# k-sheridan/mantis

Measured on AMD Instinct MI355X. Metric: poses/sec + p50 per-frame latency, 1280x720 4-cam batch, higher is better.
Workload: dtype f64; 1 GPU; config3: 4-cam 1280x720 rig, shared map, full mantis3 path per camera + joint rig Gauss-Newton; cams_per_rig=4, contexts_per_gpu=6, landmarks=720, parallelism=rig-data-parallel x1

## Files before the change

### mantis_amd/csrc/api.hip

```cpp
#include <hip/hip_runtime.h>
#ifndef MK_FC_THREADS
#define MK_FC_THREADS 256
#endif

#include <algorithm>
#include <atomic>
#include <cfloat>
#include <chrono>
#include <cmath>
#include <cstdio>
#include <cstdlib>
#include <cstring>
#include <mutex>
#include <sstream>
#include <string>
#include <thread>
#include <vector>

#include <rccl/rccl.h>

#include "kernels.hip"

using namespace mk;

namespace {

struct ZigTables {
  uint32_t kn[128];
  float wn[128], fn[128];
  ZigTables() {
    const double m1 = 2147483648.0;
    double dn = 3.442619855899, tn = dn, vn = 9.91256303526217e-3;
    double q = vn / std::exp(-.5 * dn * dn);
    kn[0] = (uint32_t)((dn / q) * m1);
    kn[1] = 0;
    wn[0] = (float)(q / m1);
    wn[127] = (float)(dn / m1);
    fn[0] = 1.f;
    fn[127] = (float)std::exp(-.5 * dn * dn);
    for (int i = 126; i >= 1; i--) {
      dn = std::sqrt(-2. * std::log(vn / dn + std::exp(-.5 * dn * dn)));
      kn[i + 1] = (uint32_t)((dn / tn) * m1);
      tn = dn;
      fn[i] = (float)std::exp(-.5 * dn * dn);
      wn[i] = (float)(dn / m1);
    }
  }
};
const ZigTables& zig() {
  static ZigTables t;
  return t;
}
inline uint64_t rng_step(uint64_t x) { return (uint64_t)(uint32_t)x * 4164903690ULL + (x >> 32); }
inline float rng_gauss(uint64_t& state) {
  const ZigTables& T = zig();
  const float r = 3.442620f;
  const float rng_flt = 2.3283064365386962890625e-10f;
  uint64_t temp = state;
  float x, y;
  for (;;) {
    int hz = (int)(uint32_t)temp;
    temp = rng_step(temp);
    int iz = hz & 127;
    x = hz * T.wn[iz];
    if ((unsigned)std::abs(hz) < T.kn[iz]) break;
    if (iz == 0) {
      do {
        x = (unsigned)temp * rng_flt;
        temp = rng_step(temp);
        y = (unsigned)temp * rng_flt;
        temp = rng_step(temp);
        x = (float)(-std::log(x + FLT_MIN) * 0.2904764);
        y = (float)-std::log(y + FLT_MIN);
      } while (y + y < x * x);
      x = hz > 0 ? r + x : -r - x;
      break;
    }
    y = (unsigned)temp * rng_flt;
    temp = rng_step(temp);
    if (T.fn[iz] + y * (T.fn[iz - 1] - T.fn[iz]) < std::exp(-.5 * x * x)) break;
  }
  state = temp;
  return x;
}

#define HIP_OK(expr)                                                              \
  do {                                                                            \
    hipError_t e_ = (expr);                                                       \
    if (e_ != hipSuccess) {                                                       \
      c->err = std::string(#expr) + ": " + hipGetErrorString(e_);                 \
      return MANTIS_ERR_DEVICE;                                                   \
    }                                                                             \
  } while (0)

struct Ctx {
  mantis_config cfg{};
  hipStream_t s = nullptr;
  hipStream_t s_copy = nullptr;
  hipEvent_t ev_gauss = nullptr;
  hipEvent_t ev_wait = nullptr;
  int spin_frames = 16;
  std::string err;
  uint64_t rng_state = 1;
  double* d_lm = nullptr;
  int nw = 0, nr = 0, ng = 0;
  int F = 0, Wmax = 0, Hmax = 0;
  int n_cu = 256;
  bool trace_lds_ok = false;
  size_t trace_lds_max = 0;
  int trace_lds_frames = 0;
  int fc_small_frames = 0;
  size_t plane = 0;
  int pool_cap = 0;
  uint16_t* d_lroot = nullptr;
  size_t lstride = 0;
  size_t fstride = 0;
  uint8_t *d_bgr = nullptr, *d_strong = nullptr, *d_edge = nullptr,
          *d_det = nullptr, *d_mask = nullptr;
  int32_t* d_lab = nullptr;
  uint32_t *d_eb = nullptr, *d_b1 = nullptr, *d_b2 = nullptr;
  uint32_t* d_mbits = nullptr;
  size_t bstride = 0;
  int morph_bh = 48;
  int morph_walk = 1 << 20;
  bool runs_done = false;
  int morph_walk_small = 48;
  size_t pf_mask_lds = 0;
  int hyst_epoch = 3;
  bool hyst_rec = true;
  size_t hyst_rec_lds = 0;
  bool pf_split = true;
  uint32_t* d_dbits = nullptr;
  uint32_t* d_tbits = nullptr;
  size_t tstride = 0;
  int32_t* d_rowb = nullptr;
  size_t rstride = 0;
  size_t dstride = 0;
  FrameDesc* d_frames = nullptr;
  Border* d_borders = nullptr;
  int32_t *d_bcount = nullptr, *d_boff = nullptr, *d_pool = nullptr, *d_scratch = nullptr;
  QuadRec* d_quads = nullptr;
  RppOut* d_rpp = nullptr;
  RppItem* d_items = nullptr;
  rpp::Refine* d_refine = nullptr;
  int32_t *d_jobs0 = nullptr, *d_jobs1 = nullptr;
  RppQueue* d_rq = nullptr;
  int rpp_blocks = 0;
  double* d_opool[2] = {nullptr, nullptr};
  int32_t* d_ojob[2] = {nullptr, nullptr};
  int32_t* d_octl = nullptr;
  int32_t op_cap = 0;
  int op_rounds = 6, op_spill = 32;
  int op_lanes_small = 64, op_rounds_small = 6;
  int seg_m = 64;
  int canny_strip = 2;
  int canny_small = 0;
#ifndef MK_SHIFT_SPLIT
#define MK_SHIFT_SPLIT 0
#endif
  bool shift_split = MK_SHIFT_SPLIT;
#ifndef MK_GN_FUSED_ALL
#define MK_GN_FUSED_ALL 1
#endif
  bool gn_fused_all = MK_GN_FUSED_ALL;
  bool pf_shifts = true;
  int pf_init = 1;
  bool canny_cat = true;
  bool counted = false;
  bool vec_ok = false;
  double *d_dense_c2w = nullptr, *d_dense_err = nullptr, *d_pairs = nullptr;
  int32_t* d_dense_np = nullptr;
  size_t dense_cap = 0;
  void* d_dense_jobs = nullptr;
  size_t dense_pairs_cap = 0;
  size_t dense_jobs_cap = 0;
  GnCam* d_gncam = nullptr;
  RigGnIO* d_rigio = nullptr;
  double* d_gnobs = nullptr;
  double* d_gnacc = nullptr;
  int gn_rigs = 0, gn_cpr = 0;
  int gn_last_rigs = 0, gn_last_local = 0;
  HypRec *d_gen = nullptr, *d_hyps = nullptr;
  FrameState* d_st = nullptr;
  ScoreState* d_sst = nullptr;
  FrameDebug* d_dbg = nullptr;
  mantis_cam_result* d_res = nullptr;
  float* d_gauss = nullptr;
  int32_t* d_gtotal = nullptr;
  float* h_gauss = nullptr;
  uint64_t* h_states = nullptr;
  mantis_cam_result* h_res = nullptr;
  FrameState* h_st = nullptr;
  int32_t* h_gtotal = nullptr;
  FrameDesc* h_frames = nullptr;
  bool prof = false;
  std::vector<std::string> ev_names;
  std::vector<hipEvent_t> ev;
  std::vector<float> last_ms;
  std::vector<std::string> last_names;
  std::vector<void*> user_allocs;
  void* comm = nullptr;
  int nranks = 1, rank = 0;
  double* d_gn28 = nullptr;
  int32_t *d_sh_gidx = nullptr, *d_sh_pf = nullptr, *d_sh_flags = nullptr;
  int32_t* h_sh_flags = nullptr;
  size_t sh_cap = 0;
  uint8_t *d_sh_rec = nullptr, *h_sh_rec = nullptr;
  size_t sh_rec_bytes = 0;
  int gauss_cap = 0;
  RigWJob* d_rwjobs = nullptr;
  double* d_rwout = nullptr;
  size_t rw_cap = 0;
  int rw_rigs = 0, rw_C = 0;
  std::vector<double> rw_weights, rw_c2w, rw_sums;
  std::vector<int32_t> rw_chosen;
  bool has_prior = false;
  double prior_Twb[16];
  double* d_markov = nullptr;
  MarkovOp* d_mops = nullptr;
  int markov_n = 0;
  int32_t* d_agree = nullptr;
  bool agreed_fail = false;
  struct CallGraph {
    int n = 0, W = 0, H = 0, live = 0, nw = 0, nr = 0, ng = 0;
    bool vec = false;
    const void* lm = nullptr;
    const void* gauss = nullptr;
    hipGraphExec_t pre = nullptr, post = nullptr;
  };
  std::vector<CallGraph> graphs;
  bool use_graphs = false;
  bool screen_off = false;
  std::vector<std::pair<Cam, ScreenCam>> scam_cache;
  struct Track {
    void* d_in = nullptr;
    void* h_in = nullptr;
    size_t in_cap = 0;
    void* d_state = nullptr;
    void* d_res = nullptr;
    void* h_res = nullptr;
    int rig_cap = 0;
    void *d_Twb = nullptr, *d_c2w = nullptr, *d_pf = nullptr;
    long long* d_sums = nullptr;
    int32_t* d_cnt = nullptr;
    size_t pose_cap = 0, task_cap = 0;
    int rigs = 0, C = 0, P = 0, I = 0, record = 0;
  } trk;
  struct Mcl {
    bool live = false;
    mantis_mcl_params p{};
    int N = 0, cap = 0, cur = 0;
    void* d_T[2] = {nullptr, nullptr};
    double *d_L = nullptr, *d_Lprev = nullptr;
    unsigned long long *d_q = nullptr, *d_cum = nullptr;
    int32_t* d_anc = nullptr;
    void *d_in = nullptr, *h_in = nullptr;
    void *d_c2w = nullptr, *d_pf = nullptr;
    long long* d_sums = nullptr;
    int32_t* d_cnt = nullptr;
    void *d_res = nullptr, *h_res = nullptr;
    bool has_record = false;
    int rec_C = 0, rec_pred = 0;
    void *d_modes = nullptr, *h_modes = nullptr;
    bool has_modes = false;
    struct mantis_mcl_modes modes;
    double modes_g = 0;
    mantis_mcl_color_params color{};
    long long* d_csums = nullptr;
    int32_t* d_ccnt = nullptr;
    double *d_Ec = nullptr, *d_charge = nullptr;
    int color_cap = 0;
    int rec_color = 0, rec_color_min = 0;
  } mcl;
};

mantis_status agree(Ctx* c, mantis_status local, int32_t count = -1) {
  c->agreed_fail = false;
  if (!c->comm || !c->d_agree) return local;
  int32_t v[3] = {local != MANTIS_OK ? 1 : 0, count, -count};
  if (hipMemcpyAsync(c->d_agree, v, sizeof(v), hipMemcpyHostToDevice, c->s) != hipSuccess ||
      ncclAllReduce(c->d_agree, c->d_agree, 3, ncclInt32, ncclMax, (ncclComm_t)c->comm, c->s) != ncclSuccess ||
      hipMemcpyAsync(v, c->d_agree, sizeof(v), hipMemcpyDeviceToHost, c->s) != hipSuccess ||
      hipStreamSynchronize(c->s) != hipSuccess) {
    c->err = "agreement all-reduce failed";
    return MANTIS_ERR_COMM;
  }
  const bool mismatch = v[1] != -v[2];
  c->agreed_fail = v[0] != 0 || mismatch;
  if (local != MANTIS_OK) return local;
  if (v[0]) {
    c->err = "another rank of the communicator failed before this exchange (see its mantis_last_error)";
    return MANTIS_ERR_COMM;
  }
  if (mismatch) {
    c->err = "ranks passed different frame counts to a batched exchange (every rank must pass the same n_frames)";
    return MANTIS_ERR_ARG;
  }
  return MANTIS_OK;
}

inline Landmarks lmk_of(const Ctx* c) {
  return Landmarks{c->d_lm, c->nw, c->nr, c->ng, c->d_lm ? (const float4*)(c->d_lm + kLmfOffset) : nullptr};
}

void mark(Ctx* c, const char* name) {
  if (!c->prof) return;
  if (c->ev.size() <= c->ev_names.size()) {
    hipEvent_t e;
    (void)hipEventCreate(&e);
    c->ev.push_back(e);
  }
  (void)hipEventRecord(c->ev[c->ev_names.size()], c->s);
  c->ev_names.push_back(name);
}

struct Ctx;
hipError_t wait_stream(Ctx* c, int frames);

inline void bind_device(const Ctx* c) {
  int d = -1;
  if (hipGetDevice(&d) != hipSuccess || d != c->cfg.device) (void)hipSetDevice(c->cfg.device);
}

inline size_t morph_lds(int W, int bh) { return (size_t)3 * (bh + 2 * MB_HALO) * ((W + 31) / 32) * sizeof(uint32_t); }

inline int blocks_for(size_t n, int per = 256, int cap = 4096) {
  size_t b = (n + per - 1) / per;
  return (int)std::min<size_t>(std::max<size_t>(b, 1), (size_t)cap);
}

Cam cam_from(const mantis_image& im) {
  Cam m;
  m.fx = (double)(float)im.K[0];
  m.fy = (double)(float)im.K[4];
  m.cx = (double)(float)im.K[2];
  m.cy = (double)(float)im.K[5];
  for (int k = 0; k < 4; k++) m.k[k] = im.D[k];
  return m;
}

ScreenCam screen_cam_cached(Ctx* c, const Cam& cm) {
  for (const auto& e : c->scam_cache)
    if (std::memcmp(&e.first, &cm, sizeof(Cam)) == 0) return e.second;
  ScreenCam sc = screen_cam_from(cm);
  if (c->screen_off) sc.sens = INFINITY;
  if (c->scam_cache.size() >= 64) c->scam_cache.erase(c->scam_cache.begin());
  c->scam_cache.emplace_back(cm, sc);
  return sc;
}

template <class T>
mantis_status dalloc(Ctx* c, T** p, size_t count);

mantis_status stage_frames(Ctx* c, const mantis_image* cams, int n, int& W, int& H) {
  if (n <= 0 || n > c->F) { c->err = "frame count exceeds max_cams"; return MANTIS_ERR_ARG; }
  W = cams[0].width;
  H = cams[0].height;
  if (W <= 2 || H <= 2 || W > c->Wmax || H > c->Hmax) { c->err = "image size outside [3, max]"; return MANTIS_ERR_ARG; }
  const size_t fb = (size_t)W * H * 3;
  for (int i = 0; i < n; i++) {
    const mantis_image& im = cams[i];
    if (im.width != W || im.height != H) { c->err = "all cameras of a batch must share one size"; return MANTIS_ERR_ARG; }
    if (!im.bgr || im.step_bytes < 3 * W) { c->err = "bgr8 image with step >= 3*width required"; return MANTIS_ERR_ARG; }
    FrameDesc& fd = c->h_frames[i];
    fd.w = W;
    fd.h = H;
    fd.cam = cam_from(im);
    fd.scam = screen_cam_cached(c, fd.cam);
    if (im.mem_kind == 1 && im.step_bytes == 3 * W) {
      fd.bgr = im.bgr;
    } else {
      if (!c->d_bgr) {
        if (dalloc(c, &c->d_bgr, (size_t)c->F * c->Wmax * c->Hmax * 3) != MANTIS_OK) {
          c->d_bgr = nullptr;
          c->err = "hipMalloc of the frame staging buffer failed";
          return MANTIS_ERR_OOM;
        }
      }
      uint8_t* dst = c->d_bgr + (size_t)i * fb;
      HIP_OK(hipMemcpy2DAsync(dst, 3 * W, im.bgr, im.step_bytes, 3 * W, H,
                              im.mem_kind == 1 ? hipMemcpyDeviceToDevice : hipMemcpyHostToDevice, c->s));
      fd.bgr = dst;
    }
  }
  c->vec_ok = (W % 4) == 0;
  for (int i = 0; i < n; i++) c->vec_ok = c->vec_ok && ((uintptr_t)c->h_frames[i].bgr & 3) == 0;
// ... 198 lines not shown
  k_rpp_s1b<<<(unsigned)std::min<size_t>((expected_items + 63) / 64, (size_t)c->n_cu * MK_S1B_WPC), 64, 0, c->s>>>(
      items, jobs0, jobs1, q, pr);
  mark(c, "rpp_2nd");
  run_objpose_rounds<1>(c, blocks_for(expected_items * 2), items, rf, jobs1, q, st, 0, lanes, rounds);
  mark(c, "rpp_cand");
  k_rpp_merge<<<(unsigned)((ni + 255) / 256), 256, 0, c->s>>>(items, ni, rf, out, quads,
                                                               quads ? c->cfg.quad_gn_iterations : 0);
  mark(c, "rpp_merge");
}

mantis_status run_pose(Ctx* c, int n) {
  HIP_OK(hipMemsetAsync(c->d_rq, 0, sizeof(RppQueue), c->s));
  dim3 gr((kMaxQuads * 2 + 255) / 256, n);
  k_rpp_prep<<<gr, 256, 0, c->s>>>(c->d_quads, c->d_st, c->d_items, c->d_jobs0, c->d_rq, c->cfg.grid_spacing / 2);
  const size_t ni = (size_t)n * kMaxQuads * 2;
  mark(c, "rpp_prep");
  launch_rpp_queues(c, c->d_items, c->d_refine, c->d_jobs0, c->d_jobs1, c->d_rq, c->d_rpp, c->d_st, ni, (size_t)n * 160,
                    c->d_quads, true, n <= c->fc_small_frames);
  k_frame_hyps<<<n, 256, 0, c->s>>>(c->d_rpp, c->d_st, c->d_gen, c->d_hyps, c->d_dbg, 0.5, 0.2);
  mark(c, "hyps_cluster");
  HIP_OK(hipGetLastError());
  return MANTIS_OK;
}

struct Shard {
  int n_global;
  int slots;
  const int32_t* gidx;
};

mantis_status gauss_offsets(Ctx* c, int n, const Shard* sh) {
  const int per = c->cfg.particles * c->cfg.iterations * 6;
  if (!sh) {
    k_gauss_offsets<<<1, kGaussOffThreads, 0, c->s>>>(c->d_st, n, per, c->d_gtotal);
    HIP_OK(hipGetLastError());
    return MANTIS_OK;
  }
  HIP_OK(hipMemcpyAsync(c->d_sh_gidx, sh->gidx, sizeof(int32_t) * n, hipMemcpyHostToDevice, c->s));
  int32_t* send = c->d_sh_pf;
  int32_t* recv = c->d_sh_pf + 2 * (size_t)sh->slots;
  k_shard_pf_pack<<<(sh->slots + 255) / 256, 256, 0, c->s>>>(c->d_st, c->d_sh_gidx, n, sh->slots, send);
  ncclResult_t r = ncclAllGather(send, recv, 2 * (size_t)sh->slots, ncclInt32, (ncclComm_t)c->comm, c->s);
  if (r != ncclSuccess) { c->err = std::string("ncclAllGather (PF flags): ") + ncclGetErrorString(r); return MANTIS_ERR_COMM; }
  k_gauss_offsets_global<<<1, 1024, 0, c->s>>>(recv, sh->slots * c->nranks, c->d_sh_flags, sh->n_global, c->d_st,
                                               c->d_sh_gidx, n, per, c->d_gtotal);
  mark(c, "pf_exchange");
  HIP_OK(hipGetLastError());
  return MANTIS_OK;
}

void gen_gauss(Ctx* c, int n) {
  const int per = c->cfg.particles * c->cfg.iterations * 6;
  uint64_t s = c->rng_state;
  c->h_states[0] = s;
  for (int f = 0; f < n; f++) {
    float* g = c->h_gauss + (size_t)f * per;
    for (int k = 0; k < per; k++) g[k] = rng_gauss(s);
    c->h_states[f + 1] = s;
  }
}

mantis_status run_score(Ctx* c, int n, int n_gauss, bool copy_gauss = true) {
  const int per = c->cfg.particles * c->cfg.iterations * 6;
  if (copy_gauss) {
    HIP_OK(hipMemcpyAsync(c->d_gauss, c->h_gauss, sizeof(float) * per * n_gauss, hipMemcpyHostToDevice, c->s_copy));
    HIP_OK(hipEventRecord(c->ev_gauss, c->s_copy));
    HIP_OK(hipStreamWaitEvent(c->s, c->ev_gauss, 0));
  }
  mark(c, "gauss_h2d");
  Landmarks L = lmk_of(c);
  const bool split = c->pf_split && n <= c->fc_small_frames && c->cfg.particles <= kPfMaxParticles &&
                     c->cfg.iterations > 0;
  const bool pf_shifts = !split && c->pf_shifts;
  const int pf_init = split ? 0 : c->pf_init;
  if (!pf_init) {
    k_score_init<kScoreInit><<<n, kScoreInit, 0, c->s>>>(c->d_frames, c->d_mbits, c->bstride, L, c->d_st, c->d_hyps,
                                                        c->d_res, c->d_dbg, c->d_sst);
    mark(c, "score_pf_yaw/k_score_init");
  }
  const size_t ml = c->pf_mask_lds;
  constexpr int ppb = std::max(1, kPfThreads / 64 / kPfSplit);
  if (split) {
    const int nblk = (c->cfg.particles + ppb - 1) / ppb;
    for (int it = 0; it < c->cfg.iterations; it++)
      k_score_pf_part<kPfThreads, kPfSplit><<<dim3(nblk, n), kPfThreads, 0, c->s>>>(
          c->d_frames, c->d_mbits, c->bstride, L, c->d_st, c->d_gauss, c->d_res, c->d_dbg, c->d_sst, c->cfg.particles,
          c->cfg.iterations, it, ppb, nblk);
  } else if (ml)
    k_score_pf<kPfThreads, kPfSplit, true><<<n, kPfThreads, ml, c->s>>>(
        c->d_frames, c->d_mbits, c->bstride, L, c->d_st, c->d_gauss, c->d_res, c->d_dbg, c->d_sst, c->cfg.particles,
        c->cfg.iterations, pf_shifts ? 1 : 0, c->cfg.grid_spacing, 9, pf_init, c->d_hyps,
        (unsigned char*)c->d_gen);
  else
    k_score_pf<kPfThreads, kPfSplit, false><<<n, kPfThreads, 0, c->s>>>(
        c->d_frames, c->d_mbits, c->bstride, L, c->d_st, c->d_gauss, c->d_res, c->d_dbg, c->d_sst, c->cfg.particles,
        c->cfg.iterations, pf_shifts ? 1 : 0, c->cfg.grid_spacing, 9, pf_init, c->d_hyps,
        (unsigned char*)c->d_gen);
  mark(c, "score_pf_yaw/k_score_pf");
  const bool shifts_apart = !pf_shifts && (split || c->shift_split);
  if (shifts_apart) {
    constexpr int spb = kScoreTail / 128;
    k_score_shift_part<kScoreTail><<<dim3((81 + spb - 1) / spb, n), kScoreTail, 0, c->s>>>(
        c->d_frames, c->d_mbits, c->bstride, L, c->d_st, c->d_sst, c->cfg.grid_spacing, 9, spb);
    mark(c, "score_pf_yaw/k_score_shift_part");
  }
  k_score_final<kScoreTail><<<n, kScoreTail, 0, c->s>>>(c->d_frames, c->d_mbits, c->bstride, L, c->d_st, c->d_res, c->d_dbg,
                                               c->d_sst, c->cfg.grid_spacing, 9, shifts_apart || pf_shifts);
  mark(c, "score_pf_yaw/k_score_final");
  HIP_OK(hipGetLastError());
  return MANTIS_OK;
}

void finish_profile(Ctx* c, bool append = false) {
  if (!c->prof || c->ev_names.empty()) return;
  (void)hipEventSynchronize(c->ev[c->ev_names.size() - 1]);
  if (!append) {
    c->last_names.clear();
    c->last_ms.clear();
  }
  for (size_t i = 1; i < c->ev_names.size(); i++) {
    float ms = 0;
    (void)hipEventElapsedTime(&ms, c->ev[i - 1], c->ev[i]);
    c->last_names.push_back(c->ev_names[i]);
    c->last_ms.push_back(ms);
  }
  c->ev_names.clear();
}

hipError_t wait_stream(Ctx* c, int frames) {
  if (frames <= c->spin_frames || !c->ev_wait) return hipStreamSynchronize(c->s);
  hipError_t e = hipEventRecord(c->ev_wait, c->s);
  if (e != hipSuccess) return e;
  return hipEventSynchronize(c->ev_wait);
}

using mk::shard::fuse_rig;
using mk::shard::mat4_inv_rigid;
using mk::shard::mat4_mul;
using mk::shard::quat_to_mat4;

template <class T>
mantis_status dalloc(Ctx* c, T** p, size_t count);
template <class T>
mantis_status halloc(Ctx* c, T** p, size_t count);

mantis_status ensure_gauss(Ctx* c, int n) {
  if (n <= c->gauss_cap) return MANTIS_OK;
  const int per = c->cfg.particles * c->cfg.iterations * 6;
  HIP_OK(hipStreamSynchronize(c->s));
  (void)hipFree(c->d_gauss);
  (void)hipHostFree(c->h_gauss);
  (void)hipHostFree(c->h_states);
  c->d_gauss = nullptr;
  c->h_gauss = nullptr;
  c->h_states = nullptr;
  c->gauss_cap = 0;
  if (dalloc(c, &c->d_gauss, (size_t)n * per) || halloc(c, &c->h_gauss, (size_t)n * per) ||
      halloc(c, &c->h_states, (size_t)n + 1))
    return MANTIS_ERR_OOM;
  c->gauss_cap = n;
  return MANTIS_OK;
}

template <class F>
mantis_status capture_graph(Ctx* c, hipGraphExec_t* out, F&& body) {
  HIP_OK(hipStreamBeginCapture(c->s, hipStreamCaptureModeThreadLocal));
  const mantis_status st = body();
  hipGraph_t gr = nullptr;
  const hipError_t e = hipStreamEndCapture(c->s, &gr);
  if (st != MANTIS_OK || e != hipSuccess) {
    if (gr) (void)hipGraphDestroy(gr);
    if (st != MANTIS_OK) return st;
    c->err = std::string("hipStreamEndCapture: ") + hipGetErrorString(e);
    return MANTIS_ERR_DEVICE;
  }
  const hipError_t ei = hipGraphInstantiate(out, gr, nullptr, nullptr, 0);
  (void)hipGraphDestroy(gr);
  if (ei != hipSuccess) {
    *out = nullptr;
    c->err = std::string("hipGraphInstantiate: ") + hipGetErrorString(ei);
    return MANTIS_ERR_DEVICE;
  }
  return MANTIS_OK;
}

Ctx::CallGraph* call_graph(Ctx* c, int n, int W, int H, const Shard* sh) {
  if (!c->use_graphs || sh || c->prof || n > c->fc_small_frames) return nullptr;
  const size_t hr_lds = (size_t)((H + HR_ROWS - 1) / HR_ROWS) * HR_ROWS * bits::words(W) * sizeof(uint32_t);
  if (!(c->hyst_rec && bits::words(W) <= 63 && H <= HR_ROWS * HR_MAXW && hr_lds <= c->hyst_rec_lds)) return nullptr;
  const int live = std::max(1, g_live_ctx[c->cfg.device & 63].load());
  for (auto& g : c->graphs)
    if (g.n == n && g.W == W && g.H == H && g.vec == c->vec_ok && g.live == live && g.lm == c->d_lm &&
        g.nw == c->nw && g.nr == c->nr && g.ng == c->ng && g.gauss == c->d_gauss)
      return &g;
  if (c->graphs.size() >= 8) {
    if (c->graphs.front().pre) (void)hipGraphExecDestroy(c->graphs.front().pre);
    if (c->graphs.front().post) (void)hipGraphExecDestroy(c->graphs.front().post);
    c->graphs.erase(c->graphs.begin());
  }
  Ctx::CallGraph g;
  g.n = n; g.W = W; g.H = H; g.vec = c->vec_ok; g.live = live;
  g.lm = c->d_lm; g.nw = c->nw; g.nr = c->nr; g.ng = c->ng; g.gauss = c->d_gauss;
  c->graphs.push_back(g);
  return &c->graphs.back();
}

mantis_status process_frames(Ctx* c, const mantis_image* cams, int n, const Shard* sh = nullptr) {
  if (!c->d_lm) { c->err = "map not set (mantis_set_map)"; return MANTIS_ERR_STATE; }
  if (n <= 0 || n > c->F) { c->err = "frame count exceeds max_cams"; return MANTIS_ERR_ARG; }
  const int ng = sh ? sh->n_global : n;
  if ((int64_t)c->cfg.particles * c->cfg.iterations * 6 * ng > INT32_MAX) {
    c->err = "particles x iterations x 6 x frames (all rig cameras when sharded) exceeds 2^31 gaussians per call";
    return MANTIS_ERR_ARG;
  }
  if (mantis_status e = ensure_gauss(c, ng)) return e;
  struct Joiner {
    std::thread t;
    ~Joiner() { if (t.joinable()) t.join(); }
  } gauss;
  gauss.t = std::thread([c, ng] { gen_gauss(c, ng); });
  int W, H;
  mantis_status st = stage_frames(c, cams, n, W, H);
  const auto results_d2h = [&]() -> mantis_status {
    HIP_OK(hipMemcpyAsync(c->h_res, c->d_res, sizeof(mantis_cam_result) * n, hipMemcpyDeviceToHost, c->s));
    HIP_OK(hipMemcpyAsync(c->h_st, c->d_st, sizeof(FrameState) * n, hipMemcpyDeviceToHost, c->s));
    HIP_OK(hipMemcpyAsync(c->h_gtotal, c->d_gtotal, sizeof(int32_t), hipMemcpyDeviceToHost, c->s));
    return MANTIS_OK;
  };
  Ctx::CallGraph* g = st == MANTIS_OK ? call_graph(c, n, W, H, sh) : nullptr;
  if (g) {
    if (!g->pre)
      st = capture_graph(c, &g->pre, [&]() -> mantis_status {
        mantis_status s2 = run_image_stages(c, n, W, H);
        if (s2 == MANTIS_OK) s2 = run_contours(c, n, W, H);
        if (s2 == MANTIS_OK) s2 = run_pose(c, n);
        if (s2 == MANTIS_OK) s2 = gauss_offsets(c, n, nullptr);
        return s2;
      });
    if (st != MANTIS_OK) return st;
    HIP_OK(hipGraphLaunch(g->pre, c->s));
    gauss.t.join();
    const int per = c->cfg.particles * c->cfg.iterations * 6;
    HIP_OK(hipMemcpyAsync(c->d_gauss, c->h_gauss, sizeof(float) * per * ng, hipMemcpyHostToDevice, c->s));
    if (!g->post)
      st = capture_graph(c, &g->post, [&]() -> mantis_status {
        mantis_status s2 = run_score(c, n, ng, false);
        if (s2 == MANTIS_OK) s2 = results_d2h();
        return s2;
      });
    if (st != MANTIS_OK) return st;
    HIP_OK(hipGraphLaunch(g->post, c->s));
  } else {
    if (st == MANTIS_OK) st = run_image_stages(c, n, W, H);
    if (st == MANTIS_OK) st = run_contours(c, n, W, H);
    if (st == MANTIS_OK) st = run_pose(c, n);
    if (sh) st = agree(c, st);
    if (st != MANTIS_OK) return st;
    if ((st = gauss_offsets(c, n, sh)) != MANTIS_OK) return st;
    gauss.t.join();
    if ((st = run_score(c, n, ng)) != MANTIS_OK) return st;
    if ((st = results_d2h()) != MANTIS_OK) return st;
  }
  if (sh) HIP_OK(hipMemcpyAsync(c->h_sh_flags, c->d_sh_flags, sizeof(int32_t) * ng, hipMemcpyDeviceToHost, c->s));
  HIP_OK(wait_stream(c, n));
  finish_profile(c);
  const int per = c->cfg.particles * c->cfg.iterations * 6;
  int used = 0;
  if (sh)
    for (int f = 0; f < ng; f++) used += c->h_sh_flags[f] ? 1 : 0;
  for (int f = 0; f < n; f++) {
    if (!sh && c->h_st[f].reaches_pf) used++;
    if (c->h_st[f].overflow) {
      std::ostringstream os;
      os << "frame " << f << ": workspace capacity exceeded (flags " << c->h_st[f].overflow << ", borders "
         << c->h_st[f].n_borders << ", points " << c->h_st[f].n_points << ", raw quads " << c->h_st[f].n_raw_quads
         << ")";
      c->err = os.str();
      c->h_res[f].status = MANTIS_ERR_CAPACITY;
    }
  }
  if (const char* fs = getenv("MANTIS_FRAME_STATS")) {
    if (FILE* fp = fopen(fs, "a")) {
      for (int f = 0; f < n; f++)
        fprintf(fp, "%d %d %d %d %d %d %d\n", c->h_st[f].n_runs, c->h_st[f].n_borders, c->h_st[f].n_points,
                c->h_st[f].trace_steps_max, c->h_st[f].trace_steps_sum, c->h_st[f].n_chunks, c->h_st[f].trace_ticks);
// ... 84 lines not shown
      g_create_err = "mantis_config.struct_size mismatch";
      return MANTIS_ERR_ARG;
    }
    cfg = *cfg_in;
  }
  if (cfg.max_quads == 0) cfg.max_quads = kMaxQuads;
  if ((int64_t)cfg.particles * cfg.iterations * 6 * (cfg.max_cams > 0 ? cfg.max_cams : 1) > INT32_MAX) {
    g_create_err = "particles x iterations x 6 x max_cams exceeds 2^31 gaussians per batch";
    return MANTIS_ERR_ARG;
  }
  if (cfg.particles < 1 || cfg.particles > 96 || cfg.iterations < 0 || cfg.iterations > 1000 || cfg.max_cams < 1 ||
      cfg.max_width < 3 || cfg.max_height < 3 || cfg.gn_iterations < 0 || cfg.gn_iterations > 10 ||
      cfg.quad_gn_iterations < 0 || cfg.quad_gn_iterations > 20 || cfg.rig_weighting < 0 || cfg.rig_weighting > 1) {
    g_create_err = "invalid config (particles 1..96, iterations 0..1000, gn_iterations 0..10, "
                   "quad_gn_iterations 0..20, max_cams >= 1, image >= 3x3)";
    return MANTIS_ERR_ARG;
  }
  if (cfg.max_width > 8190) {
    g_create_err = "max_width: at most 8190 (the hysteresis bands hold a row's worst-case runs in LDS)";
    return MANTIS_ERR_ARG;
  }
  if (cfg.max_height > 65533) {
    g_create_err = "max_height: at most 65533 (border walks and contour points pack y + 1 in 16 bits)";
    return MANTIS_ERR_ARG;
  }
  if ((int64_t)((cfg.max_height + HB_ROWS - 1) / HB_ROWS) * HB_ROWS * ((cfg.max_width + 1) / 2) >= (1 << 24)) {
    g_create_err = "max_width x max_height: at most 2^25 pixels (hysteresis run ids and their band row share a word)";
    return MANTIS_ERR_ARG;
  }
  if (cfg.max_quads != kMaxQuads) {
    g_create_err = "max_quads: the per-frame quad capacity is fixed at 256 in this build";
    return MANTIS_ERR_ARG;
  }
  int ndev = 0;
  if (hipGetDeviceCount(&ndev) != hipSuccess || ndev <= cfg.device) {
    g_create_err = "no HIP device available (libmantis_amd requires an MI355X / gfx950 GPU)";
    return MANTIS_ERR_DEVICE;
  }
  Ctx* c = new Ctx();
  c->cfg = cfg;
  c->rng_state = cfg.rng_seed ? cfg.rng_seed : 0xffffffffULL;
  if (hipSetDevice(cfg.device) != hipSuccess || hipStreamCreateWithFlags(&c->s, hipStreamNonBlocking) != hipSuccess ||
      hipStreamCreateWithFlags(&c->s_copy, hipStreamNonBlocking) != hipSuccess ||
      hipEventCreateWithFlags(&c->ev_gauss, hipEventDisableTiming) != hipSuccess ||
      hipEventCreateWithFlags(&c->ev_wait, hipEventDisableTiming | hipEventBlockingSync) != hipSuccess) {
    g_create_err = "hipSetDevice/hipStreamCreate failed";
    if (c->s) (void)hipStreamDestroy(c->s);
    if (c->s_copy) (void)hipStreamDestroy(c->s_copy);
    delete c;
    return MANTIS_ERR_DEVICE;
  }
  if (hipDeviceGetAttribute(&c->n_cu, hipDeviceAttributeMultiprocessorCount, cfg.device) != hipSuccess || c->n_cu < 1)
    c->n_cu = 256;
  if (const char* e = std::getenv("MANTIS_RPP_BLOCKS")) c->rpp_blocks = std::atoi(e);
  if (const char* e = std::getenv("MANTIS_OP_ROUNDS")) c->op_rounds = std::max(1, std::min(kOpMaxRounds, std::atoi(e)));
  if (const char* e = std::getenv("MANTIS_OP_SPILL")) c->op_spill = std::max(0, std::min(64, std::atoi(e)));
  if (const char* e = std::getenv("MANTIS_OP_LANES_SMALL")) c->op_lanes_small = std::max(1, std::min(64, std::atoi(e)));
  if (const char* e = std::getenv("MANTIS_OP_ROUNDS_SMALL")) c->op_rounds_small = std::max(1, std::min(kOpMaxRounds, std::atoi(e)));
  if (const char* e = std::getenv("MANTIS_SEG_M")) c->seg_m = std::max(0, std::min(4096, std::atoi(e)));
  if (const char* e = std::getenv("MANTIS_CANNY_STRIP")) c->canny_strip = c->canny_small = std::atoi(e);
  if (const char* e = std::getenv("MANTIS_CANNY_CAT")) c->canny_cat = e[0] != '0';
  if (const char* e = std::getenv("MANTIS_SHIFT_SPLIT")) c->shift_split = e[0] != '0';
  if (const char* e = std::getenv("MANTIS_PF_SHIFTS")) c->pf_shifts = e[0] != '0';
  if (const char* e = std::getenv("MANTIS_GN_FUSED")) c->gn_fused_all = e[0] != '0';
  if (const char* e = std::getenv("MANTIS_PF_INIT")) c->pf_init = std::max(0, std::min(2, std::atoi(e)));
  if (const char* e = std::getenv("MANTIS_HYST_REC")) c->hyst_rec = e[0] != '0';
  {
    const char* pc = std::getenv("DEBUG_CLR_GRAPH_PACKET_CAPTURE");
    c->use_graphs = pc && pc[0] == '0';
    if (const char* e = std::getenv("MANTIS_GRAPHS")) c->use_graphs = c->use_graphs && e[0] != '0';
  }
  if (const char* e = std::getenv("MANTIS_HYST_EPOCH0")) c->hyst_epoch = std::max(3, std::min(255, std::atoi(e)));
  c->F = cfg.max_cams;
  c->Wmax = cfg.max_width;
  c->Hmax = cfg.max_height;
  c->plane = (size_t)(c->Wmax + 2) * (c->Hmax + 2);
  c->bstride = bits::tiled_words(c->Wmax, c->Hmax);
  c->dstride = (size_t)dbits_wpw(c->Wmax + 2) * (c->Hmax + 2);
  c->pool_cap = cfg.max_contour_points;
  {
    c->trace_lds_max = 160 * 1024 - 512 * 8 - 64;
    c->trace_lds_ok = hipFuncSetAttribute((const void*)k_trace_borders_lds, hipFuncAttributeMaxDynamicSharedMemorySize,
                                          (int)c->trace_lds_max) == hipSuccess;
    const char* so = getenv("MANTIS_SCREEN");
    c->screen_off = so && so[0] == '0';
    const char* e = getenv("MANTIS_TRACE_LDS_FRAMES");
    c->trace_lds_frames = e ? atoi(e) : c->n_cu / 4;
    const char* e2 = getenv("MANTIS_FC_SMALL_FRAMES");
    c->fc_small_frames = e2 ? atoi(e2) : c->n_cu / 4;
    const char* e3 = getenv("MANTIS_PF_SPLIT");
    c->pf_split = !(e3 && e3[0] == '0');
  }
  {
    const size_t ml = bits::tiled_words(c->Wmax, c->Hmax) * 4;
    hipFuncAttributes a1;
    c->pf_mask_lds = 0;
    if (!getenv("MANTIS_PF_MASK_GLOBAL") &&
        hipFuncGetAttributes(&a1, (const void*)k_score_pf<kPfThreads, kPfSplit, true>) == hipSuccess &&
        a1.sharedSizeBytes + ml <= 160 * 1024 &&
        hipFuncSetAttribute((const void*)k_score_pf<kPfThreads, kPfSplit, true>,
                            hipFuncAttributeMaxDynamicSharedMemorySize, (int)ml) == hipSuccess)
      c->pf_mask_lds = ml;
  }
  {
    hipFuncAttributes a;
    if (hipFuncGetAttributes(&a, (const void*)k_hyst_rec) == hipSuccess) {
      const size_t budget = 160 * 1024 - a.sharedSizeBytes;
      if (hipFuncSetAttribute((const void*)k_hyst_rec, hipFuncAttributeMaxDynamicSharedMemorySize, (int)budget) ==
          hipSuccess)
        c->hyst_rec_lds = budget;
    }
  }
  if (hipFuncSetAttribute((const void*)k_hyst_band, hipFuncAttributeMaxDynamicSharedMemorySize,
                          (int)(3 * sizeof(uint32_t) * HB_ROWS * bits::words(c->Wmax))) != hipSuccess) {
    g_create_err = "max_width too large for the hysteresis band kernel";
    (void)hipStreamDestroy(c->s);
    delete c;
    return MANTIS_ERR_ARG;
  }
  c->morph_bh = morph_lds(c->Wmax, MB_BH) <= 160 * 1024 ? MB_BH : MB_BH_NARROW;
  if (const char* e = getenv("MANTIS_MORPH_WALK")) {
    c->morph_walk = std::max(0, atoi(e));
    c->morph_walk_small = std::max(1, c->morph_walk);
  }
  if (const char* e = getenv("MANTIS_MORPH_WALK_SMALL")) c->morph_walk_small = std::max(1, atoi(e));
  if (morph_lds(c->Wmax, c->morph_bh) > 160 * 1024 ||
      hipFuncSetAttribute((const void*)k_morph, hipFuncAttributeMaxDynamicSharedMemorySize,
                          (int)morph_lds(c->Wmax, c->morph_bh)) !=
          hipSuccess) {
    g_create_err = "max_width too large for the morphology band kernel";
    (void)hipStreamDestroy(c->s);
    delete c;
    return MANTIS_ERR_ARG;
  }
  const int F = c->F;
  const int per = cfg.particles * cfg.iterations * 6;
  mantis_status st = MANTIS_OK;
  auto chk = [&](mantis_status s) { if (st == MANTIS_OK) st = s; };
  c->fstride = (c->plane + 3) & ~(size_t)3;
  chk(dalloc(c, &c->d_strong, (size_t)F * c->fstride));
  c->lstride = (c->plane + 1) & ~(size_t)1;
  chk(dalloc(c, &c->d_lroot, (size_t)F * c->lstride));
  chk(dalloc(c, &c->d_edge, c->plane));
  chk(dalloc(c, &c->d_det, c->plane));
  chk(dalloc(c, &c->d_eb, (size_t)F * c->bstride));
  chk(dalloc(c, &c->d_b1, (size_t)F * c->bstride));
  chk(dalloc(c, &c->d_b2, (size_t)F * c->bstride));
  chk(dalloc(c, &c->d_dbits, (size_t)F * c->dstride));
  c->tstride = tbits_words(c->Wmax + 2, c->Hmax + 2);
  chk(dalloc(c, &c->d_tbits, (size_t)F * c->tstride));
  c->rstride = (size_t)c->Hmax + 3 + (c->Hmax + HB_ROWS - 1) / HB_ROWS;
  chk(dalloc(c, &c->d_rowb, (size_t)F * c->rstride));
  chk(dalloc(c, &c->d_mask, c->plane));
  chk(dalloc(c, &c->d_mbits, (size_t)F * c->bstride));
  chk(dalloc(c, &c->d_lab, (size_t)F * c->plane));
  chk(dalloc(c, &c->d_frames, (size_t)F));
  chk(dalloc(c, &c->d_borders, (size_t)F * kMaxBorders));
  chk(dalloc(c, &c->d_bcount, (size_t)F * kMaxBorders));
  chk(dalloc(c, &c->d_boff, (size_t)F * kMaxBorders));
  chk(dalloc(c, &c->d_pool, (size_t)F * 2 * c->pool_cap));
  chk(dalloc(c, &c->d_scratch, (size_t)F * 4 * c->pool_cap));
  chk(dalloc(c, &c->d_quads, (size_t)F * kMaxQuads));
  chk(dalloc(c, &c->d_rpp, (size_t)F * kMaxQuads * 2));
  chk(dalloc(c, &c->d_items, (size_t)F * kMaxQuads * 2));
  chk(dalloc(c, &c->d_refine, (size_t)F * kMaxQuads * 2 * rpp::kCand));
  chk(dalloc(c, &c->d_jobs0, (size_t)F * kMaxQuads * 2));
  chk(dalloc(c, &c->d_jobs1, (size_t)F * kMaxQuads * 2 * rpp::kCand));
  chk(dalloc(c, &c->d_rq, 1));
  {
    const size_t blocks = c->rpp_blocks > 0 ? (size_t)c->rpp_blocks : (size_t)std::max(64, 3 * c->n_cu / 2);
    c->op_cap = (int32_t)(blocks * 256);
    for (int k = 0; k < 2; k++) {
      chk(dalloc(c, &c->d_opool[k], (size_t)kOpFields * c->op_cap));
      chk(dalloc(c, &c->d_ojob[k], (size_t)c->op_cap));
    }
    chk(dalloc(c, &c->d_octl, 2 * 2 * kOpMaxRounds));
  }
  chk(dalloc(c, &c->d_gen, (size_t)F * kMaxHyps));
  chk(dalloc(c, &c->d_hyps, (size_t)F * kMaxHyps));
  chk(dalloc(c, &c->d_st, (size_t)F));
  chk(dalloc(c, &c->d_sst, (size_t)F));
  chk(dalloc(c, &c->d_dbg, (size_t)F));
  chk(dalloc(c, &c->d_res, (size_t)F));
  chk(dalloc(c, &c->d_gauss, (size_t)F * per));
// ... 4 lines not shown
  chk(halloc(c, &c->h_res, (size_t)F));
  chk(halloc(c, &c->h_st, (size_t)F));
  chk(halloc(c, &c->h_gtotal, 1));
  chk(halloc(c, &c->h_frames, (size_t)F));
  if (st != MANTIS_OK) {
    g_create_err = c->err;
    mantis_destroy(c);
    return st;
  }
  (void)hipGetLastError();
  if (hipMemset(c->d_dbg, 0, sizeof(FrameDebug) * F) != hipSuccess ||
      hipMemset(c->d_strong, 0, c->fstride * (size_t)F) != hipSuccess) {
    g_create_err = "hipMemset failed";
    mantis_destroy(c);
    return MANTIS_ERR_DEVICE;
  }
  g_live_ctx[cfg.device & 63].fetch_add(1);
  c->counted = true;
  *out_ctx = c;
  return MANTIS_OK;
}

mantis_status mantis_destroy(void* ctx) {
  Ctx* c = (Ctx*)ctx;
  if (c) bind_device(c);
  if (!c) return MANTIS_ERR_ARG;
  if (c->counted) g_live_ctx[c->cfg.device & 63].fetch_sub(1);
  if (c->s) (void)hipStreamSynchronize(c->s);
  if (c->comm) (void)ncclCommDestroy((ncclComm_t)c->comm);
  for (auto& g : c->graphs) {
    if (g.pre) (void)hipGraphExecDestroy(g.pre);
    if (g.post) (void)hipGraphExecDestroy(g.post);
  }
  if (c->d_rwjobs) (void)hipFree(c->d_rwjobs);
  if (c->d_markov) (void)hipFree(c->d_markov);
  if (c->d_mops) (void)hipFree(c->d_mops);
  if (c->d_rwout) (void)hipFree(c->d_rwout);
  void* dptrs[] = {c->d_opool[0], c->d_opool[1], c->d_ojob[0], c->d_ojob[1], c->d_octl, c->d_dense_jobs, c->d_agree, c->d_gn28, c->d_bgr, c->d_lroot, c->d_strong, c->d_edge, c->d_det, c->d_mask, c->d_lab, c->d_eb, c->d_b1, c->d_b2, c->d_mbits, c->d_dbits, c->d_tbits, c->d_rowb,
                   c->d_frames, c->d_borders, c->d_bcount, c->d_boff, c->d_pool, c->d_scratch, c->d_quads, c->d_rpp, c->d_items, c->d_refine, c->d_jobs0, c->d_jobs1, c->d_rq,
                   c->d_dense_c2w, c->d_dense_err, c->d_dense_np, c->d_pairs, c->d_gncam, c->d_rigio, c->d_gnobs, c->d_gnacc, c->d_sh_gidx, c->d_sh_pf, c->d_sh_flags, c->d_sh_rec, c->d_gen, c->d_hyps, c->d_st, c->d_sst, c->d_dbg, c->d_res, c->d_gauss, c->d_gtotal, c->d_lm};
  for (void* p : dptrs)
    if (p) (void)hipFree(p);
  void* tptrs[] = {c->trk.d_in, c->trk.d_state, c->trk.d_res, c->trk.d_Twb, c->trk.d_c2w, c->trk.d_pf, c->trk.d_sums, c->trk.d_cnt};
  for (void* p : tptrs)
    if (p) (void)hipFree(p);
  void* mptrs[] = {c->mcl.d_T[0], c->mcl.d_T[1], c->mcl.d_L, c->mcl.d_Lprev, c->mcl.d_q, c->mcl.d_cum, c->mcl.d_anc,
                   c->mcl.d_in, c->mcl.d_c2w, c->mcl.d_pf, c->mcl.d_sums, c->mcl.d_cnt, c->mcl.d_res, c->mcl.d_modes,
                   c->mcl.d_csums, c->mcl.d_ccnt, c->mcl.d_Ec, c->mcl.d_charge};
  for (void* p : mptrs)
    if (p) (void)hipFree(p);
  for (void* p : c->user_allocs) (void)hipFree(p);
  void* hptrs[] = {c->h_gauss, c->h_states, c->h_res, c->h_st, c->h_gtotal, c->h_frames, c->h_sh_flags, c->h_sh_rec,
                   c->trk.h_in, c->trk.h_res, c->mcl.h_in, c->mcl.h_res, c->mcl.h_modes};
  for (void* p : hptrs)
    if (p) (void)hipHostFree(p);
  for (hipEvent_t e : c->ev) (void)hipEventDestroy(e);
  if (c->ev_gauss) (void)hipEventDestroy(c->ev_gauss);
  if (c->ev_wait) (void)hipEventDestroy(c->ev_wait);
  if (c->s_copy) (void)hipStreamDestroy(c->s_copy);
  if (c->s) (void)hipStreamDestroy(c->s);
  delete c;
  return MANTIS_OK;
}

const char* mantis_last_error(void* ctx) {
  if (!ctx) return g_create_err.c_str();
  return ((Ctx*)ctx)->err.c_str();
}

mantis_status mantis_set_map(void* ctx, const double* white, int32_t nw, const double* red, int32_t nr,
                             const double* green, int32_t ng) {
  Ctx* c = (Ctx*)ctx;
  if (c) bind_device(c);
  if (!c || nw < 0 || nr < 0 || ng < 0 || nw + nr + ng > 768 || ng > 64 || (nw && !white) || (nr && !red) ||
      (ng && !green)) {
    if (c) c->err = "map: need nw+nr+ng <= 768 and ng <= 64";
    return MANTIS_ERR_ARG;
  }
  std::vector<double> all;
  all.insert(all.end(), white, white + 3 * nw);
  all.insert(all.end(), red, red + 3 * nr);
  all.insert(all.end(), green, green + 3 * ng);
  const size_t nl = (size_t)nw + nr + ng;
  std::vector<double> buf(kLmfOffset + 2 * 768, 0.0);
  std::copy(all.begin(), all.end(), buf.begin());
  float* lf = (float*)(buf.data() + kLmfOffset);
  for (size_t i = 0; i < nl; i++) screen_landmark(all.data() + 3 * i, lf + 4 * i);
  if (c->d_lm) (void)hipFree(c->d_lm);
  c->d_lm = nullptr;
  if (dalloc(c, &c->d_lm, buf.size()) != MANTIS_OK) return MANTIS_ERR_OOM;
  HIP_OK(hipMemcpy(c->d_lm, buf.data(), sizeof(double) * buf.size(), hipMemcpyHostToDevice));
  c->nw = nw;
  c->nr = nr;
  c->ng = ng;
  return MANTIS_OK;
}

int32_t mantis_parse_coordinates(const char* s, double* xyz, int32_t max_pts) {
  if (!s) return 0;
  std::vector<std::string> rows;
  std::stringstream ts(s);
  std::string tmp;
  while (std::getline(ts, tmp, ';')) {
    tmp.erase(std::remove(tmp.begin(), tmp.end(), '\n'), tmp.end());
    tmp.erase(std::remove(tmp.begin(), tmp.end(), ' '), tmp.end());
    rows.push_back(tmp);
  }
  int n = 0;
  for (auto& e : rows) {
    std::stringstream rs(e);
    std::string rt;
    double v[3] = {0, 0, 0};
    for (int k = 0; k < 3; k++) {
      std::getline(rs, rt, ',');
      v[k] = std::atof(rt.data());
    }
    if (xyz && n < max_pts) { xyz[3 * n] = v[0]; xyz[3 * n + 1] = v[1]; xyz[3 * n + 2] = v[2]; }
    n++;
  }
  return n;
}

mantis_status mantis_rng_get(void* ctx, uint64_t* state) {
  if (!ctx || !state) return MANTIS_ERR_ARG;
  *state = ((Ctx*)ctx)->rng_state;
  return MANTIS_OK;
}
mantis_status mantis_rng_set(void* ctx, uint64_t state) {
  if (!ctx) return MANTIS_ERR_ARG;
  ((Ctx*)ctx)->rng_state = state ? state : 0xffffffffULL;
  return MANTIS_OK;
}

namespace {
mantis_status run_rig_gn(Ctx* c, const double* Tbc, int n_rigs, int cams_local, mantis_result* out,
                         bool use_comm);
}

namespace {
mantis_status weight_rigs(Ctx* c, int n_rigs, int C, const mantis_cam_result* all, const double* Tall,
                          const int32_t* gidx, int n_local, bool use_comm, mantis_result* out,
                          const double* pred_Twb = nullptr) {
  const int K = C + 1;
  const size_t nslot = (size_t)n_rigs * K * C;
  std::vector<double> Twb((size_t)n_rigs * K * 16);
  std::vector<char> cand((size_t)n_rigs * K, 0);
  for (int r = 0; r < n_rigs; r++) {
    for (int k = 0; k < C; k++) {
      const mantis_cam_result& cr = all[(size_t)r * C + k];
      if (!cr.publish) continue;
      double Twc[16], Tinv[16];
      quat_to_mat4(cr.orientation_xyzw, cr.position, Twc);
      mat4_inv_rigid(Tall + 16 * ((size_t)r * C + k), Tinv);
      mat4_mul(Twc, Tinv, &Twb[16 * ((size_t)r * K + k)]);
      cand[(size_t)r * K + k] = 1;
    }
    if (pred_Twb) {
      std::memcpy(&Twb[16 * ((size_t)r * K + C)], pred_Twb + 16 * (size_t)r, sizeof(double) * 16);
      cand[(size_t)r * K + C] = 1;
    }
  }
  c->rw_c2w.assign(nslot * 12, 0.0);
  std::vector<RigWJob> jobs;
  std::vector<size_t> slot_of;
  for (int i = 0; i < n_local; i++) {
    const int g = gidx ? gidx[i] : i;
    const int r = g / C, cam = g % C;
    for (int k = 0; k < K; k++) {
      if (!cand[(size_t)r * K + k]) continue;
      double Twc[16], Tcw[16];
      mat4_mul(&Twb[16 * ((size_t)r * K + k)], Tall + 16 * (size_t)g, Twc);
      mat4_inv_rigid(Twc, Tcw);
      RigWJob J;
      std::memset(&J, 0, sizeof(J));
      for (int a = 0; a < 3; a++) {
        for (int b = 0; b < 3; b++) J.c2w[3 * a + b] = Tcw[4 * a + b];
        J.c2w[9 + a] = Tcw[4 * a + 3];
// ... 397 lines not shown
  if (c) bind_device(c);
  if (!c || !cls || !edges_out) return MANTIS_ERR_ARG;
  const int W = width, H = height;
  if (W <= 2 || H <= 2 || W > c->Wmax || H > c->Hmax) { c->err = "image size outside [3, max]"; return MANTIS_ERR_ARG; }
  for (size_t i = 0; i < (size_t)W * H; i++)
    if (cls[i] > 2) { c->err = "class plane: bytes must be 0 (none), 1 (weak) or 2 (strong)"; return MANTIS_ERR_ARG; }
  HIP_OK(hipMemcpyAsync(c->d_edge, cls, (size_t)W * H, hipMemcpyHostToDevice, c->s));
  k_cls_to_bits<<<blocks_for((size_t)bits::words(W) * H), 256, 0, c->s>>>(c->d_edge, c->d_b1, c->d_b2, W, H);
  if (mantis_status st = run_hysteresis(c, 1, W, H, true); st != MANTIS_OK) return st;
  HIP_OK(hipMemcpyAsync(edges_out, c->d_edge, (size_t)W * H, hipMemcpyDeviceToHost, c->s));
  HIP_OK(hipStreamSynchronize(c->s));
  for (size_t i = 0; i < (size_t)W * H; i++) edges_out[i] = edges_out[i] ? 255 : 0;
  return MANTIS_OK;
}

mantis_status mantis_masks(void* ctx, const mantis_image* img, uint8_t* det_out, uint8_t* mask_out) {
  Ctx* c = (Ctx*)ctx;
  if (c) bind_device(c);
  if (!c || !img) return MANTIS_ERR_ARG;
  int W, H;
  mantis_status st = stage_frames(c, img, 1, W, H);
  if (st != MANTIS_OK) return st;
  if ((st = run_image_stages(c, 1, W, H, false, det_out != nullptr)) != MANTIS_OK) return st;
  if (det_out) {
    HIP_OK(hipMemcpy2DAsync(det_out, W, c->d_det + (W + 2) + 1, W + 2, W, H, hipMemcpyDeviceToHost, c->s));
  }
  if (mask_out) {
    k_bits_to_bytes<<<blocks_for((size_t)W * H), 256, 0, c->s>>>(c->d_mbits, c->d_mask, W, H, -1);
    HIP_OK(hipMemcpyAsync(mask_out, c->d_mask, (size_t)W * H, hipMemcpyDeviceToHost, c->s));
  }
  HIP_OK(hipStreamSynchronize(c->s));
  for (size_t i = 0; det_out && i < (size_t)W * H; i++) det_out[i] = det_out[i] ? 255 : 0;
  for (size_t i = 0; mask_out && i < (size_t)W * H; i++) mask_out[i] = mask_out[i] ? 255 : 0;
  return MANTIS_OK;
}

mantis_status mantis_detect_quads(void* ctx, const mantis_image* img, int32_t* corners, int32_t max_quads,
                                  int32_t* n_quads) {
  Ctx* c = (Ctx*)ctx;
  if (c) bind_device(c);
  if (!c || !img || !n_quads) return MANTIS_ERR_ARG;
  int W, H;
  mantis_status st = stage_frames(c, img, 1, W, H);
  if (st != MANTIS_OK) return st;
  if ((st = run_image_stages(c, 1, W, H)) != MANTIS_OK) return st;
  if ((st = run_contours(c, 1, W, H)) != MANTIS_OK) return st;
  HIP_OK(hipMemcpyAsync(c->h_st, c->d_st, sizeof(FrameState), hipMemcpyDeviceToHost, c->s));
  HIP_OK(hipStreamSynchronize(c->s));
  if (c->h_st[0].overflow) { c->err = "detect_quads: workspace capacity exceeded"; return MANTIS_ERR_CAPACITY; }
  int nq = c->h_st[0].n_quads;
  *n_quads = nq;
  if (corners && max_quads > 0) {
    std::vector<QuadRec> q(nq);
    HIP_OK(hipMemcpy(q.data(), c->d_quads, sizeof(QuadRec) * nq, hipMemcpyDeviceToHost));
    for (int i = 0; i < nq && i < max_quads; i++)
      for (int k = 0; k < 8; k++) corners[8 * i + k] = q[i].c[k];
  }
  return MANTIS_OK;
}

mantis_status mantis_score_hypotheses(void* ctx, const mantis_image* img, const uint8_t* mask, const double* c2w,
                                      int32_t n, int32_t fast, double* err, int32_t* nproj) {
  Ctx* c = (Ctx*)ctx;
  if (c) bind_device(c);
  if (!c || !img || !c2w || n <= 0 || !err || !nproj) return MANTIS_ERR_ARG;
  if (!c->d_lm) { c->err = "map not set"; return MANTIS_ERR_STATE; }
  int W, H;
  mantis_status st = stage_frames(c, img, 1, W, H);
  if (st != MANTIS_OK) return st;
  double* d_c2w = nullptr;
  double* d_err = nullptr;
  int32_t* d_np = nullptr;
  if (dalloc(c, &d_c2w, (size_t)12 * n) != MANTIS_OK || dalloc(c, &d_err, (size_t)n) != MANTIS_OK ||
      dalloc(c, &d_np, (size_t)n) != MANTIS_OK)
    return MANTIS_ERR_OOM;
  const uint8_t* d_mask = nullptr;
  if (mask) {
    HIP_OK(hipMemcpyAsync(c->d_mask, mask, (size_t)W * H, hipMemcpyHostToDevice, c->s));
    d_mask = c->d_mask;
  }
  HIP_OK(hipMemcpyAsync(d_c2w, c2w, sizeof(double) * 12 * n, hipMemcpyHostToDevice, c->s));
  Landmarks L = lmk_of(c);
  mark(c, "start");
  k_score_api<<<(n + kApiHyps - 1) / kApiHyps, 64 * kApiHyps, 0, c->s>>>(c->d_frames, d_mask, L, d_c2w, n, fast, d_err, d_np);
  mark(c, "score_api");
  HIP_OK(hipGetLastError());
  HIP_OK(hipMemcpyAsync(err, d_err, sizeof(double) * n, hipMemcpyDeviceToHost, c->s));
  HIP_OK(hipMemcpyAsync(nproj, d_np, sizeof(int32_t) * n, hipMemcpyDeviceToHost, c->s));
  HIP_OK(hipStreamSynchronize(c->s));
  finish_profile(c);
  (void)hipFree(d_c2w);
  (void)hipFree(d_err);
  (void)hipFree(d_np);
  return MANTIS_OK;
}

mantis_status mantis_quad_gn(void* ctx, const double* img_pts, const double* obj_pts, int32_t n, double* R,
                             double* t, int32_t iterations, int32_t* steps, double* costs) {
  Ctx* c = (Ctx*)ctx;
  if (c) bind_device(c);
  if (!c || !img_pts || !obj_pts || n <= 0 || !R || !t || iterations < 0 || iterations > 100) return MANTIS_ERR_ARG;
  double *d_ip, *d_op, *d_R, *d_t, *d_c;
  int32_t* d_s;
  if (dalloc(c, &d_ip, (size_t)8 * n) || dalloc(c, &d_op, (size_t)12 * n) || dalloc(c, &d_R, (size_t)9 * n) ||
      dalloc(c, &d_t, (size_t)3 * n) || dalloc(c, &d_c, (size_t)2 * n) || dalloc(c, &d_s, (size_t)n))
    return MANTIS_ERR_OOM;
  HIP_OK(hipMemcpyAsync(d_ip, img_pts, sizeof(double) * 8 * n, hipMemcpyHostToDevice, c->s));
  HIP_OK(hipMemcpyAsync(d_op, obj_pts, sizeof(double) * 12 * n, hipMemcpyHostToDevice, c->s));
  HIP_OK(hipMemcpyAsync(d_R, R, sizeof(double) * 9 * n, hipMemcpyHostToDevice, c->s));
  HIP_OK(hipMemcpyAsync(d_t, t, sizeof(double) * 3 * n, hipMemcpyHostToDevice, c->s));
  k_quad_gn<<<(n + 255) / 256, 256, 0, c->s>>>(d_ip, d_op, n, d_R, d_t, iterations, d_s, d_c);
  HIP_OK(hipGetLastError());
  HIP_OK(hipMemcpyAsync(R, d_R, sizeof(double) * 9 * n, hipMemcpyDeviceToHost, c->s));
  HIP_OK(hipMemcpyAsync(t, d_t, sizeof(double) * 3 * n, hipMemcpyDeviceToHost, c->s));
  if (steps) HIP_OK(hipMemcpyAsync(steps, d_s, sizeof(int32_t) * n, hipMemcpyDeviceToHost, c->s));
  if (costs) HIP_OK(hipMemcpyAsync(costs, d_c, sizeof(double) * 2 * n, hipMemcpyDeviceToHost, c->s));
  HIP_OK(hipStreamSynchronize(c->s));
  void* ps[] = {d_ip, d_op, d_R, d_t, d_c, d_s};
  for (void* p : ps) (void)hipFree(p);
  return MANTIS_OK;
}

mantis_status mantis_rpp_batch(void* ctx, const double* img_pts, const double* obj_pts, int32_t n, double* R,
                               double* t, double* errs, int32_t* rpp_status) {
  Ctx* c = (Ctx*)ctx;
  if (c) bind_device(c);
  if (!c || !img_pts || !obj_pts || n <= 0 || !R || !t || !errs || !rpp_status) return MANTIS_ERR_ARG;
  double *d_ip, *d_op;
  RppItem* d_it;
  rpp::Refine* d_rf;
  RppOut* d_out;
  int32_t *d_j0, *d_j1;
  RppQueue* d_q;
  if (dalloc(c, &d_ip, (size_t)8 * n) || dalloc(c, &d_op, (size_t)12 * n) || dalloc(c, &d_it, (size_t)n) ||
      dalloc(c, &d_rf, (size_t)n * rpp::kCand) || dalloc(c, &d_out, (size_t)n) || dalloc(c, &d_j0, (size_t)n) ||
      dalloc(c, &d_j1, (size_t)n * rpp::kCand) || dalloc(c, &d_q, 1))
    return MANTIS_ERR_OOM;
  HIP_OK(hipMemcpyAsync(d_ip, img_pts, sizeof(double) * 8 * n, hipMemcpyHostToDevice, c->s));
  HIP_OK(hipMemcpyAsync(d_op, obj_pts, sizeof(double) * 12 * n, hipMemcpyHostToDevice, c->s));
  HIP_OK(hipMemsetAsync(d_q, 0, sizeof(RppQueue), c->s));
  mark(c, "start");
  k_rpp_prep_api<<<(n + 255) / 256, 256, 0, c->s>>>(d_ip, d_op, n, d_it, d_j0, d_q);
  mark(c, "rpp_prep");
  launch_rpp_queues(c, d_it, d_rf, d_j0, d_j1, d_q, d_out, nullptr, (size_t)n, (size_t)n, nullptr, false);
  HIP_OK(hipGetLastError());
  std::vector<RppOut> h(n);
  HIP_OK(hipMemcpyAsync(h.data(), d_out, sizeof(RppOut) * n, hipMemcpyDeviceToHost, c->s));
  HIP_OK(hipStreamSynchronize(c->s));
  finish_profile(c);
  for (int i = 0; i < n; i++) {
    for (int k = 0; k < 9; k++) R[9 * i + k] = h[i].R[k];
    for (int k = 0; k < 3; k++) t[3 * i + k] = h[i].t[k];
    errs[2 * i] = h[i].obj_err;
    errs[2 * i + 1] = h[i].img_err;
    rpp_status[i] = h[i].error == 1 ? -1 : h[i].status;
  }
  void* ps[] = {d_ip, d_op, d_it, d_rf, d_out, d_j0, d_j1, d_q};
  for (void* p : ps) (void)hipFree(p);
  return MANTIS_OK;
}

mantis_status mantis_rpp_solve(void* ctx, const double* img_pts, const double* obj_pts, int32_t n_points,
                               int32_t n, double* R, double* t, double* errs, int32_t* rpp_status,
                               int32_t* iterations) {
  Ctx* c = (Ctx*)ctx;
  if (c) bind_device(c);
  if (!c || !img_pts || !obj_pts || n <= 0 || !R || !t || !errs || !rpp_status) return MANTIS_ERR_ARG;
// ... 130 lines not shown
```

### mantis_amd/csrc/dense_impl.hip

```cpp

namespace mk {

__global__ __launch_bounds__(1024) void k_argmin(const double* __restrict__ err, int n, int64_t base,
                                                 double* __restrict__ out2) {
  __shared__ double se[1024];
  __shared__ int si[1024];
  const int t = threadIdx.x;
  double be = DBL_MAX;
  int bi = 0x7fffffff;
  for (int i = t; i < n; i += 1024) {
    const double e = err[i];
    if (e < be) { be = e; bi = i; }
  }
  se[t] = be;
  si[t] = bi;
  __syncthreads();
  for (int s = 512; s > 0; s >>= 1) {
    if (t < s) {
      const double e2 = se[t + s];
      const int i2 = si[t + s];
      if (e2 < se[t] || (e2 == se[t] && i2 < si[t])) { se[t] = e2; si[t] = i2; }
    }
    __syncthreads();
  }
  if (t == 0) {
    out2[0] = se[0];
    out2[1] = si[0] == 0x7fffffff ? -1.0 : (double)(base + si[0]);
  }
}

struct DenseJob {
  const uint8_t* mask;
  const double* c2w;
  int32_t n, err_off;
  int64_t index_base;
};
__global__ __launch_bounds__(64 * kApiHyps) void k_score_api_batch(const FrameDesc* __restrict__ frames,
                                                                   const DenseJob* __restrict__ jobs, Landmarks lmk,
                                                                   double* __restrict__ err, int32_t* __restrict__ nproj) {
  const int f = blockIdx.y;
  const DenseJob J = jobs[f];
  if ((int)blockIdx.x * kDenseHyps >= J.n) return;
  const FrameDesc fd = frames[f];
  if (J.mask)
    score_api_fast<kDenseHyps>(fd, &frames[f].cam, MaskBytes{J.mask}, lmk, J.c2w, J.n, err + J.err_off,
                               nproj + J.err_off);
  else
    score_api_fast<kDenseHyps>(fd, &frames[f].cam, MaskNone{}, lmk, J.c2w, J.n, err + J.err_off, nproj + J.err_off);
}
__global__ __launch_bounds__(1024) void k_argmin_batch(const DenseJob* __restrict__ jobs, const double* __restrict__ err,
                                                       double* __restrict__ out2) {
  const DenseJob J = jobs[blockIdx.x];
  __shared__ double se[1024];
  __shared__ int si[1024];
  const int t = threadIdx.x;
  double be = DBL_MAX;
  int bi = 0x7fffffff;
  for (int i = t; i < J.n; i += 1024) {
    const double e = err[J.err_off + i];
    if (e < be) { be = e; bi = i; }
  }
  se[t] = be;
  si[t] = bi;
  __syncthreads();
  for (int s = 512; s > 0; s >>= 1) {
    if (t < s) {
      const double e2 = se[t + s];
      const int i2 = si[t + s];
      if (e2 < se[t] || (e2 == se[t] && i2 < si[t])) { se[t] = e2; si[t] = i2; }
    }
    __syncthreads();
  }
  if (t == 0) {
    out2[2 * blockIdx.x] = se[0];
    out2[2 * blockIdx.x + 1] = si[0] == 0x7fffffff ? -1.0 : (double)(J.index_base + si[0]);
  }
}

}

extern "C" {

mantis_status mantis_argmin_pick(const double* pairs, int32_t nranks, double* best_err, int64_t* best_idx) {
  if (!pairs || nranks <= 0 || !best_err || !best_idx) return MANTIS_ERR_ARG;
  double be = DBL_MAX;
  int64_t bi = -1;
  for (int r = 0; r < nranks; r++) {
    const double e = pairs[2 * r];
    const int64_t i = (int64_t)pairs[2 * r + 1];
    if (i < 0) continue;
    if (bi < 0 || e < be || (e == be && i < bi)) { be = e; bi = i; }
  }
  *best_err = be;
  *best_idx = bi;
  return MANTIS_OK;
}

}

namespace {
mantis_status score_argmin_impl(void* ctx, const mantis_image* img, const uint8_t* mask, const double* c2w,
                                int32_t n, int64_t index_base, int32_t use_comm, double* best_err,
                                int64_t* best_idx, bool dev) {
  Ctx* c = (Ctx*)ctx;
  if (c) bind_device(c);
  if (!c || !img || !c2w || n < 0 || !best_err || !best_idx) return MANTIS_ERR_ARG;
  if (use_comm && !c->comm) { c->err = "comm not initialised (mantis_comm_init)"; return MANTIS_ERR_STATE; }
  const auto prepare = [&]() -> mantis_status {
    if (!c->d_lm) { c->err = "map not set"; return MANTIS_ERR_STATE; }
    if (use_comm && (c->nranks < 1 || c->nranks > 63)) { c->err = "argmin exchange supports 1..63 ranks"; return MANTIS_ERR_ARG; }
    int W, H;
    mantis_status st = stage_frames(c, img, 1, W, H);
    if (st != MANTIS_OK) return st;
    const size_t cap = (size_t)(n > 0 ? n : 1);
    if (cap > c->dense_cap) {
      (void)hipFree(c->d_dense_c2w);
      (void)hipFree(c->d_dense_err);
      (void)hipFree(c->d_dense_np);
      c->d_dense_c2w = nullptr;
      c->d_dense_err = nullptr;
      c->d_dense_np = nullptr;
      c->dense_cap = 0;
      if (dalloc(c, &c->d_dense_c2w, 12 * cap) != MANTIS_OK || dalloc(c, &c->d_dense_err, cap) != MANTIS_OK ||
          dalloc(c, &c->d_dense_np, cap) != MANTIS_OK)
        return MANTIS_ERR_OOM;
      c->dense_cap = cap;
    }
    if (!c->d_pairs) {
      if (dalloc(c, &c->d_pairs, (size_t)2 * 64) != MANTIS_OK) return MANTIS_ERR_OOM;
      c->dense_pairs_cap = 128;
    }
    return MANTIS_OK;
  };
  mantis_status st = prepare();
  if (use_comm) st = agree(c, st, 1);
  if (st != MANTIS_OK) return st;
  const int W = img->width, H = img->height;
  const uint8_t* d_mask = nullptr;
  const double* d_c2w = c->d_dense_c2w;
  if (dev) {
    d_mask = mask;
    d_c2w = c2w;
  } else {
    if (mask) {
      HIP_OK(hipMemcpyAsync(c->d_mask, mask, (size_t)W * H, hipMemcpyHostToDevice, c->s));
      d_mask = c->d_mask;
    }
    if (n > 0) HIP_OK(hipMemcpyAsync(c->d_dense_c2w, c2w, sizeof(double) * 12 * n, hipMemcpyHostToDevice, c->s));
  }
  Landmarks L = lmk_of(c);
  mark(c, "start");
  if (n > 0) {
    k_score_api<<<(n + kApiHyps - 1) / kApiHyps, 64 * kApiHyps, 0, c->s>>>(c->d_frames, d_mask, L, d_c2w, n, 1, c->d_dense_err,
                                               c->d_dense_np);
    mark(c, "score_dense");
  }
  k_argmin<<<1, 1024, 0, c->s>>>(c->d_dense_err, n, index_base, c->d_pairs);
  mark(c, "argmin");
  HIP_OK(hipGetLastError());
  int nr = 1;
  if (use_comm) {
    nr = c->nranks;
    ncclResult_t r = ncclAllGather(c->d_pairs, c->d_pairs + 2, 2, ncclFloat64, (ncclComm_t)c->comm, c->s);
    if (r != ncclSuccess) { c->err = std::string("ncclAllGather: ") + ncclGetErrorString(r); return MANTIS_ERR_COMM; }
    mark(c, "allgather");
  }
  double h[2 * 64];
  HIP_OK(hipMemcpyAsync(h, c->d_pairs + (use_comm ? 2 : 0), sizeof(double) * 2 * nr, hipMemcpyDeviceToHost, c->s));
  HIP_OK(hipStreamSynchronize(c->s));
  finish_profile(c);
  return mantis_argmin_pick(h, nr, best_err, best_idx);
}
}

extern "C" {

mantis_status mantis_score_argmin_batch(void* ctx, const mantis_image* imgs, int32_t n_frames,
                                        const uint8_t* const* masks_dev, const double* const* c2w_dev,
                                        const int32_t* n_hyps, const int64_t* index_base, int32_t use_comm,
                                        double* best_err, int64_t* best_idx) {
  Ctx* c = (Ctx*)ctx;
  if (c) bind_device(c);
  if (!c || !imgs || n_frames <= 0 || !c2w_dev || !n_hyps || !index_base || !best_err || !best_idx)
    return MANTIS_ERR_ARG;
  if (use_comm && !c->comm) { c->err = "comm not initialised (mantis_comm_init)"; return MANTIS_ERR_STATE; }
  std::vector<DenseJob> jobs(n_frames);
  int maxn = 0;
  const auto prepare = [&]() -> mantis_status {
    if (!c->d_lm) { c->err = "map not set"; return MANTIS_ERR_STATE; }
    if (use_comm && (c->nranks < 1 || c->nranks > 63)) { c->err = "argmin exchange supports 1..63 ranks"; return MANTIS_ERR_ARG; }
    int W, H;
    mantis_status st = stage_frames(c, imgs, n_frames, W, H);
    if (st != MANTIS_OK) return st;
    size_t tot = 0;
    for (int f = 0; f < n_frames; f++) {
      if (n_hyps[f] < 0 || (n_hyps[f] > 0 && !c2w_dev[f])) { c->err = "bad hypothesis block"; return MANTIS_ERR_ARG; }
      jobs[f] = DenseJob{masks_dev ? masks_dev[f] : nullptr, c2w_dev[f], n_hyps[f], (int32_t)tot, index_base[f]};
      tot += (size_t)n_hyps[f];
      maxn = std::max(maxn, n_hyps[f]);
    }
    if (tot > (size_t)INT32_MAX) { c->err = "too many hypotheses in one batch"; return MANTIS_ERR_ARG; }
    const size_t cap = std::max<size_t>(tot, 1);
    if (cap > c->dense_cap) {
      (void)hipFree(c->d_dense_err);
      (void)hipFree(c->d_dense_np);
      (void)hipFree(c->d_dense_c2w);
      c->d_dense_err = c->d_dense_c2w = nullptr;
      c->d_dense_np = nullptr;
      c->dense_cap = 0;
      if (dalloc(c, &c->d_dense_c2w, 12 * cap) != MANTIS_OK || dalloc(c, &c->d_dense_err, cap) != MANTIS_OK ||
          dalloc(c, &c->d_dense_np, cap) != MANTIS_OK)
        return MANTIS_ERR_OOM;
      c->dense_cap = cap;
    }
    const size_t pair_cap = std::max<size_t>((size_t)2 * n_frames * (use_comm ? c->nranks + 1 : 1), 128);
    if (pair_cap > c->dense_pairs_cap) {
      (void)hipFree(c->d_pairs);
      c->d_pairs = nullptr;
      c->dense_pairs_cap = 0;
      if (dalloc(c, &c->d_pairs, pair_cap) != MANTIS_OK) return MANTIS_ERR_OOM;
      c->dense_pairs_cap = pair_cap;
    }
    if ((size_t)n_frames > c->dense_jobs_cap) {
      (void)hipFree(c->d_dense_jobs);
      c->d_dense_jobs = nullptr;
      c->dense_jobs_cap = 0;
      if (dalloc(c, (DenseJob**)&c->d_dense_jobs, (size_t)n_frames) != MANTIS_OK) return MANTIS_ERR_OOM;
      c->dense_jobs_cap = (size_t)n_frames;
    }
    return MANTIS_OK;
  };
  mantis_status st = prepare();
  if (use_comm) st = agree(c, st, n_frames);
  if (st != MANTIS_OK) return st;
  DenseJob* d_jobs = (DenseJob*)c->d_dense_jobs;
  HIP_OK(hipMemcpyAsync(d_jobs, jobs.data(), sizeof(DenseJob) * n_frames, hipMemcpyHostToDevice, c->s));
  Landmarks L = lmk_of(c);
  mark(c, "start");
  if (maxn > 0)
    k_score_api_batch<<<dim3((maxn + kDenseHyps - 1) / kDenseHyps, n_frames), 64 * kApiHyps, 0, c->s>>>(
        c->d_frames, d_jobs, L, c->d_dense_err, c->d_dense_np);
  mark(c, "score_dense");
  k_argmin_batch<<<n_frames, 1024, 0, c->s>>>(d_jobs, c->d_dense_err, c->d_pairs);
  mark(c, "argmin");
  HIP_OK(hipGetLastError());
  int nr = 1;
  if (use_comm) {
    nr = c->nranks;
    ncclResult_t r = ncclAllGather(c->d_pairs, c->d_pairs + 2 * n_frames, 2 * (size_t)n_frames, ncclFloat64,
                                   (ncclComm_t)c->comm, c->s);
    if (r != ncclSuccess) { c->err = std::string("ncclAllGather: ") + ncclGetErrorString(r); return MANTIS_ERR_COMM; }
    mark(c, "allgather");
  }
  std::vector<double> h((size_t)2 * n_frames * nr);
  HIP_OK(hipMemcpyAsync(h.data(), c->d_pairs + (use_comm ? 2 * n_frames : 0), sizeof(double) * h.size(),
                        hipMemcpyDeviceToHost, c->s));
  HIP_OK(hipStreamSynchronize(c->s));
  finish_profile(c);
  std::vector<double> pr((size_t)2 * nr);
  for (int f = 0; f < n_frames; f++) {
    for (int r = 0; r < nr; r++) {
      pr[2 * r] = h[(size_t)r * 2 * n_frames + 2 * f];
      pr[2 * r + 1] = h[(size_t)r * 2 * n_frames + 2 * f + 1];
    }
    mantis_argmin_pick(pr.data(), nr, &best_err[f], &best_idx[f]);
  }
  return MANTIS_OK;
}

mantis_status mantis_score_argmin(void* ctx, const mantis_image* img, const uint8_t* mask, const double* c2w,
                                  int32_t n, int64_t index_base, int32_t use_comm, double* best_err,
                                  int64_t* best_idx) {
  return score_argmin_impl(ctx, img, mask, c2w, n, index_base, use_comm, best_err, best_idx, false);
}

mantis_status mantis_score_argmin_dev(void* ctx, const mantis_image* img, const uint8_t* mask_dev,
                                      const double* c2w_dev, int32_t n, int64_t index_base, int32_t use_comm,
                                      double* best_err, int64_t* best_idx) {
  return score_argmin_impl(ctx, img, mask_dev, c2w_dev, n, index_base, use_comm, best_err, best_idx, true);
}

}
```

### mantis_amd/csrc/hostcheck.cpp

```cpp
#include <algorithm>
#include <cstdint>
#include <cstring>
#include <vector>

static int g_jacobi_ff = 1;
#define MK_JACOBI_FF g_jacobi_ff
#include "mk_bits.h"
#include "mk_contour.h"
#include "mk_gn.h"
#include "mk_math.h"
#include "mk_mcl.h"
#include "mk_mcl_color.h"
#include "mk_mcl_modes.h"
#include "mk_rpp.h"
#include "mk_screen.h"
#include "mk_shard.h"
#include "mk_sort.h"
#include "mk_track.h"

extern "C" {

void hc_set_jacobi_ff(int on) { g_jacobi_ff = on; }

int hc_rpp(const double* model, const double* iprts, double* R, double* t, double* errs, int* err_code) {
  mk::rpp::Result r = mk::rpp::solve(model, iprts);
  std::memcpy(R, r.R, sizeof(r.R));
  std::memcpy(t, r.t, sizeof(r.t));
  errs[0] = r.obj_err;
  errs[1] = r.img_err;
  errs[2] = r.iterations;
  *err_code = r.error;
  return r.status;
}

int hc_rpp_n(const double* model, const double* iprts, int n, double* R, double* t, double* errs, int* err_code) {
  mk::rpp::Result r;
  switch (n) {
    case 4: r = mk::rpp::solve(model, iprts); break;
#define MK_HC_RPP(k) \
    case k: r = mk::rpp::n##k::solve(model, iprts); break;
    MK_RPP_INSTANCES(MK_HC_RPP)
#undef MK_HC_RPP
    default: return -100;
  }
  std::memcpy(R, r.R, sizeof(r.R));
  std::memcpy(t, r.t, sizeof(r.t));
  errs[0] = r.obj_err;
  errs[1] = r.img_err;
  errs[2] = r.iterations;
  *err_code = r.error;
  return r.status;
}

void hc_first_objpose(const double* model, const double* iprts, double* R, double* t, double* errs, int32_t* it,
                      double* Qout) {
  mk::rpp::Stage1 s;
  mk::rpp::stage1a(model, iprts, s);
  std::memcpy(R, s.R, sizeof(s.R));
  std::memcpy(t, s.t, sizeof(s.t));
  errs[0] = s.obj_err;
  errs[1] = s.img_err;
  *it = s.iterations;
  std::memcpy(Qout, s.Q, sizeof(s.Q));
}

int hc_stage1_cands(const double* model, const double* iprts, double* sR, double* R, double* t, double* errs,
                    int32_t* its, int32_t* error) {
  mk::rpp::Stage1 s;
  mk::rpp::stage1(model, iprts, s);
  *error = s.error;
  std::memcpy(sR, s.sR, sizeof(s.sR));
  for (int j = 0; j < mk::rpp::kCand; j++) {
    its[j] = -1;
    if (s.error != 1 && ((s.keep_mask >> j) & 1)) {
      mk::rpp::Refine r;
      mk::rpp::refine(model, s.Q, s.sR[j], r);
      std::memcpy(R + 9 * j, r.R, sizeof(r.R));
      std::memcpy(t + 3 * j, r.t, sizeof(r.t));
      errs[2 * j] = r.obj_err;
      errs[2 * j + 1] = r.img_err;
      its[j] = r.iterations;
    }
  }
  return s.keep_mask;
}

void hc_rpp_iters(const double* model, const double* iprts, int32_t* it) {
  mk::rpp::Stage1 s;
  mk::rpp::stage1(model, iprts, s);
  it[0] = s.iterations;
  for (int j = 0; j < mk::rpp::kCand; j++) {
    it[1 + j] = -1;
// ... 310 lines not shown
        const int j = r0 + w * 64 + l;
        if (j < N) cum[j] += pre;
      }
      pre += wt[w];
    }
    carry = pre;
  }
}
void hc_mcl_ancestors(const uint64_t* cum, const uint64_t* q, int N, uint32_t U, int32_t* anc) {
  int last = 0;
  for (int j = 0; j < N; j++)
    if (q[j] > 0) last = j;
  for (int i = 0; i < N; i++) anc[i] = mk::mcl::ancestor(cum, N, U, i, last);
}
int hc_mcl_past(uint64_t c, int N, uint32_t U, int i, uint64_t S) { return mk::mcl::past(c, N, U, i, S) ? 1 : 0; }
uint64_t hc_mcl_rng_next(uint64_t s) { return mk::mcl::rng_next(s); }

void hc_mcl_step(const int64_t* sums, const int32_t* counts, int N, int C, double* T, double* L, double tau,
                 double resample_frac, int32_t min_projections, uint32_t U, uint64_t* q, uint64_t* cum, int32_t* anc,
                 int32_t* flags4, uint64_t* S, double* ess_err2, double* T_mean16, double* cov36, double* E,
                 double* Lnew) {
  std::vector<mk::Xf> X(N);
  std::vector<long long> s((size_t)N * C);
  for (size_t k = 0; k < s.size(); k++) s[k] = sums[k];
  for (int j = 0; j < N; j++) X[j] = mk::track::xf_from_mat4(T + 16 * (size_t)j);
  const mk::mcl::Outcome o = mk::mcl::step_seq(s.data(), counts, N, C, X.data(), L, tau, resample_frac, min_projections,
                                               U, q, cum, anc, E, Lnew);
  for (int j = 0; j < N; j++) mk::track::xf_to_mat4(X[j], T + 16 * (size_t)j);
  flags4[0] = o.lost; flags4[1] = o.resampled; flags4[2] = o.n_valid; flags4[3] = o.best;
  *S = o.S;
  ess_err2[0] = o.ess;
  ess_err2[1] = o.best_error;
  if (o.lost) {
    std::memset(T_mean16, 0, sizeof(double) * 16);
    std::memset(cov36, 0, sizeof(double) * 36);
  } else {
    mk::track::xf_to_mat4(o.mean, T_mean16);
    std::memcpy(cov36, o.cov, sizeof(double) * 36);
  }
}

void hc_mcl_cell_key(const double* T, const double* A, double g, int32_t* key4) {
  key4[3] = mk::mcl::cell_key(mk::track::xf_from_mat4(T), mk::track::xf_from_mat4(A), g, key4, key4 + 1, key4 + 2);
}
void hc_mcl_lattice_site(int s, int cx, int cy, int32_t* ixy2) { mk::mcl::lattice_site(s, cx, cy, ixy2, ixy2 + 1); }
void hc_mcl_modes(const double* T, const uint64_t* q, const int64_t* sums, const int32_t* counts, int N, int C, int best,
                  double g, int max_modes, void* out) {
  std::vector<mk::Xf> X(N);
  std::vector<long long> s((size_t)N * C);
  for (size_t k = 0; k < s.size(); k++) s[k] = sums[k];
  for (int j = 0; j < N; j++) X[j] = mk::track::xf_from_mat4(T + 16 * (size_t)j);
  mk::mcl::modes_seq(X.data(), q, s.data(), counts, N, C, best, g, max_modes, (mk::mcl::Modes*)out);
}

int32_t hc_mcl_color_window(const uint8_t* bgr, int W, int H, double u, double v) {
  return mk::mcl::color_window_sum(bgr, W, H, u, v);
}
void hc_mcl_color_sums(const double* c2w, int n, const double* green, int ng, const double* K, const double* D,
                       const uint8_t* bgr, int W, int H, int64_t* csum, int32_t* cn) {
  mk::Cam cm{(double)(float)K[0], (double)(float)K[4], (double)(float)K[2], (double)(float)K[5], {D[0], D[1], D[2], D[3]}};
  for (int i = 0; i < n; i++) {
    mk::Xf T;
    for (int k = 0; k < 12; k++) (k < 9 ? T.R[k] : T.t[k - 9]) = c2w[12 * i + k];
    long long s;
    mk::mcl::color_sums(T, green, ng, cm, bgr, W, H, &s, &cn[i]);
    csum[i] = s;
  }
}
void hc_mcl_color_charge(const int64_t* csums, const int32_t* cns, int N, int C, int32_t min_color_projections,
                         double color_miss, double color_tau, double* Ec, int32_t* n_out, double* charge) {
  std::vector<long long> s(C > 0 ? C : 1);
  for (int j = 0; j < N; j++) {
    for (int c = 0; c < C; c++) s[c] = csums[(size_t)j * C + c];
    Ec[j] = mk::mcl::color_pool(s.data(), cns + (size_t)j * C, C, min_color_projections, &n_out[j]);
    charge[j] = mk::mcl::color_charge(Ec[j], color_miss, color_tau);
  }
}
void hc_mcl_color_fold(const double* L, const double* E, const int32_t* n_proj, const double* charge, int N, double tau,
                       int32_t min_projections, double* L_out) {
  for (int j = 0; j < N; j++)
    L_out[j] = mk::mcl::log_weight_color(L[j], E[j], n_proj[j], min_projections, tau, charge[j]);
}

}
```

### mantis_amd/csrc/kernels.hip

```cpp
#include <hip/hip_runtime.h>

#include <cfloat>
#include <cstdint>

#include "mk_bits.h"
#include "mk_contour.h"
#include "mk_gn.h"
#include "mk_math.h"
#include "mk_rpp.h"
#include "mk_shard.h"
#include "mk_sort.h"
#include "mk_types.h"
#include "synth.h"

namespace mk {

#ifndef MK_DPP_SCAN
#define MK_DPP_SCAN 1
#endif
__device__ inline int wave_incl_scan(int v, int lane) {
#if MK_DPP_SCAN
  (void)lane;
  v += __builtin_amdgcn_update_dpp(0, v, 0x111, 0xf, 0xf, true);
  v += __builtin_amdgcn_update_dpp(0, v, 0x112, 0xf, 0xf, true);
  v += __builtin_amdgcn_update_dpp(0, v, 0x114, 0xf, 0xf, true);
  v += __builtin_amdgcn_update_dpp(0, v, 0x118, 0xf, 0xf, true);
  v += __builtin_amdgcn_update_dpp(0, v, 0x142, 0xa, 0xf, false);
  v += __builtin_amdgcn_update_dpp(0, v, 0x143, 0xc, 0xf, false);
#else
  for (int o = 1; o < 64; o <<= 1) {
    const int u = __shfl_up(v, o);
    if (lane >= o) v += u;
  }
#endif
  return v;
}
__device__ inline int wave_sum(int v) {
#if MK_DPP_SCAN
  return __builtin_amdgcn_readlane(wave_incl_scan(v, 0), 63);
#else
  for (int o = 32; o > 0; o >>= 1) v += __shfl_xor(v, o);
  return v;
#endif
}

typedef __attribute__((address_space(1))) const uint8_t gu8;
typedef __attribute__((address_space(1))) const uint32_t gu32;
__device__ inline gu8* gbytes(const uint8_t* p) { return (gu8*)p; }
__device__ inline gu32* gwords(const void* p) { return (gu32*)p; }

__device__ inline int uf_find_c(int32_t* lab, int x) {
  while (true) {
    int p = lab[x];
    if (p == x) return x;
    int g = lab[p];
    if (g == p) return p;
    lab[x] = g;
    x = g;
  }
}
__device__ inline void uf_union_c(int32_t* lab, int a, int b) {
  while (true) {
    a = uf_find_c(lab, a);
    b = uf_find_c(lab, b);
    if (a == b) return;
    if (a < b) { int t = a; a = b; b = t; }
    int old = atomicCAS(&lab[a], a, b);
    if (old == a) return;
    a = old;
  }
}
__device__ inline int lds_find(const int* L, int x) {
  int p;
  while ((p = L[x]) != x) x = p;
  return x;
}
__device__ inline void lds_union(int* L, int a, int b) {
  while (true) {
    a = lds_find(L, a);
    b = lds_find(L, b);
    if (a == b) return;
    if (a < b) { int t = a; a = b; b = t; }
    int old = atomicCAS(&L[a], a, b);
    if (old == a) return;
    a = old;
  }
}

#ifndef MK_FTH
#define MK_FTH 16
// ... 3376 lines not shown
  HypRec* Hh = hyps + (size_t)f * kMaxHyps;
  for (int j = tid; j < n; j += blockDim.x)
    if (flag[j] >= 0) Hh[flag[j]] = G[j];
}

constexpr int kGaussOffThreads = 256;
__global__ __launch_bounds__(kGaussOffThreads) void k_gauss_offsets(FrameState* st, int nf, int per_frame, int32_t* total) {
  constexpr int NT = kGaussOffThreads;
  __shared__ int wsum[NT / 64];
  const int t = threadIdx.x, lane = t & 63, wave = t >> 6;
  const int chunk = (nf + NT - 1) / NT;
  const int f0 = min(nf, t * chunk), f1 = min(nf, f0 + chunk);
  int mine = 0;
  for (int f = f0; f < f1; f++) mine += st[f].reaches_pf ? per_frame : 0;
  int incl = mine;
  for (int o = 1; o < 64; o <<= 1) {
    const int v = __shfl_up(incl, o);
    if (lane >= o) incl += v;
  }
  if (lane == 63) wsum[wave] = incl;
  __syncthreads();
  int base = 0;
  for (int w = 0; w < wave; w++) base += wsum[w];
  int acc = base + incl - mine;
  for (int f = f0; f < f1; f++) {
    st[f].gauss_offset = acc;
    if (st[f].reaches_pf) acc += per_frame;
  }
  if (t == NT - 1) *total = base + incl;
}

__global__ __launch_bounds__(256) void k_shard_pf_pack(const FrameState* __restrict__ st,
                                                       const int32_t* __restrict__ gidx, int n_local, int slots,
                                                       int32_t* __restrict__ pairs) {
  const int s = blockIdx.x * 256 + threadIdx.x;
  if (s >= slots) return;
  pairs[2 * s] = s < n_local ? gidx[s] : -1;
  pairs[2 * s + 1] = s < n_local ? (st[s].reaches_pf ? 1 : 0) : 0;
}

__global__ __launch_bounds__(1024) void k_gauss_offsets_global(const int32_t* __restrict__ pairs, int npairs,
                                                               int32_t* flags, int ng, FrameState* st,
                                                               const int32_t* __restrict__ gidx, int n_local,
                                                               int per_frame, int32_t* total) {
  __shared__ int wsum[16];
  __shared__ int bad;
  const int t = threadIdx.x, lane = t & 63, wave = t >> 6;
  if (t == 0) bad = 0;
  for (int i = t; i < ng; i += 1024) flags[i] = 0;
  __syncthreads();
  for (int i = t; i < npairs; i += 1024) {
    const int g = pairs[2 * i];
    if (g >= ng) bad = 1;
    else if (g >= 0) flags[g] = pairs[2 * i + 1];
  }
  __syncthreads();
  const int chunk = (ng + 1023) / 1024;
  const int f0 = min(ng, t * chunk), f1 = min(ng, f0 + chunk);
  int mine = 0;
  for (int f = f0; f < f1; f++) mine += flags[f] ? per_frame : 0;
  int incl = mine;
  for (int o = 1; o < 64; o <<= 1) {
    const int v = __shfl_up(incl, o);
    if (lane >= o) incl += v;
  }
  if (lane == 63) wsum[wave] = incl;
  __syncthreads();
  int base = 0;
  for (int w = 0; w < wave; w++) base += wsum[w];
  int acc = base + incl - mine;
  for (int f = f0; f < f1; f++) {
    flags[ng + f] = acc;
    if (flags[f]) acc += per_frame;
  }
  if (t == 1023) *total = bad ? -1 : base + incl;
  __syncthreads();
  for (int f = t; f < n_local; f += 1024) st[f].gauss_offset = flags[ng + gidx[f]];
}

struct Landmarks {
  const double* xyz;
  int32_t nw, nr, ng;
  const float4* xyzf;
};
constexpr int kLmfOffset = 3 * 768;

struct MaskNone {
  __device__ uint32_t word(int, int, int) const { return 1u; }
  __device__ bool test(uint32_t, int) const { return true; }
};
struct MaskBytes {
  const uint8_t* m;
  __device__ uint32_t word(int lin, int, int) const { return m[lin]; }
  __device__ bool test(uint32_t w, int) const { return w != 0; }
};
typedef __attribute__((address_space(3))) const uint32_t lds_cu32;
struct MaskLds {
  lds_cu32* m;
  int Hp;
  __device__ uint32_t word(int, int x, int y) const { return m[__umul24((uint32_t)(x >> 5), (uint32_t)Hp) + y]; }
  __device__ bool test(uint32_t w, int x) const { return (w >> (x & 31)) & 1u; }
};
struct MaskBits {
  const uint32_t* m;
  int Hp, W;
  __device__ uint32_t word(int, int x, int y) const { return m[__umul24((uint32_t)(x >> 5), (uint32_t)Hp) + y]; }
  __device__ bool test(uint32_t w, int x) const { return (w >> (x & 31)) & 1u; }
};
__device__ inline uint32_t load_bgr(const uint8_t* bgr, int lin, int npx) {
  const bool last = lin == npx - 1;
  typedef __attribute__((address_space(1), aligned(1))) const uint32_t gu32u;
  const uint32_t v = *(gu32u*)(bgr + (3 * lin - (last ? 1 : 0)));
  return last ? (v >> 8) : v;
}

struct ColorLds {
  double u[64], v[64];
  int32_t acc[64], ok[64];
  int32_t x0[64], run[64];
};
typedef unsigned int cu32x4 __attribute__((ext_vector_type(4)));
__device__ inline int color_row_words(cu32x4 q0, cu32x4 q1, uint32_t d8, uint32_t m) {
  const uint32_t d[9] = {q0.x, q0.y, q0.z, q0.w, q1.x, q1.y, q1.z, q1.w, d8};
  uint32_t w[8];
#pragma unroll
  for (int j = 0; j < 8; j++) w[j] = __builtin_amdgcn_alignbyte(d[j + 1], d[j], m);
  w[7] &= 0xffffu;
  constexpr uint32_t T0 = 50u | 255u << 8 | 85u << 16 | 50u << 24;
  constexpr uint32_t T1 = 255u | 85u << 8 | 50u << 16 | 255u << 24;
  constexpr uint32_t T2 = 85u | 50u << 8 | 255u << 16 | 85u << 24;
  uint32_t sq = 0, ct = 0;
#pragma unroll
  for (int j = 0; j < 8; j++) {
    sq = __builtin_amdgcn_udot4(w[j], w[j], sq, false);
    ct = __builtin_amdgcn_udot4(w[j], j % 3 == 0 ? T0 : (j % 3 == 1 ? T1 : T2), ct, false);
  }
  return (int)sq - 2 * (int)ct + 10 * (50 * 50 + 255 * 255 + 85 * 85);
}
__device__ inline int color_row_run(const uint8_t* bgr, long lin0) {
  const long b = 3 * lin0;
  const uint32_t m = (uint32_t)(b & 3);
  typedef __attribute__((address_space(1), aligned(4))) const cu32x4 gu4a;
  const uint8_t* a = bgr + (b - m);
  uint32_t d8 = 0u;
  if (m == 3u) d8 = *(gu32*)(a + 32);
  return color_row_words(*(gu4a*)a, *(gu4a*)(a + 16), d8, m);
}
__device__ inline void wave_score_color(const Xf& c2w, const double* green, int ngr, const Cam& cm,
                                        const uint8_t* bgr, int W, int H, ColorLds* cl, double* err_out,
                                        int* n_out) {
  const int lane = threadIdx.x & 63;
  const long npx = (long)W * H;
  double total = 0;
  int n = 0;
  for (int base = 0; base < ngr; base += 64) {
    const int nb = min(64, ngr - base);
    {
      const int l = base + lane;
      int ok = 0;
      double u = 0, v = 0;
      if (lane < nb) {
        double rp[3];
        xf_apply(c2w, green + 3 * l, rp);
        distort(cm, rp[0], rp[1], rp[2], &u, &v);
        ok = rp[2] > 0 && in_frame(u, v, H, W);
      }
      const int x0 = cv_round(u + (-5.0 + 0.0));
      int run = 1;
// ... 130 lines not shown
      } else if ((yf & 6) == 6) {
        int rs = 0;
        for (int ox = 0; ox < 10; ox++) {
          const long lin = lin0 + ox;
          int b = 0, g = 0, rr = 0;
          if (lin >= 0 && lin < npx) {
            const uint32_t pv = load_bgr(bgr, lin, npx);
            b = (int)(pv & 0xffu);
            g = (int)((pv >> 8) & 0xffu);
            rr = (int)((pv >> 16) & 0xffu);
          }
          const int e0 = b - 50, e1 = g - 255, e2 = rr - 85;
          rs += e0 * e0 + e1 * e1 + e2 * e2;
        }
        rsum[k] = rs;
      } else {
        const int h = i / ngr;
        rsum[k] = color_row_exact(pose_of(h), green + 3 * (i - h * ngr), cm, bgr, W, H, r);
      }
    }
#pragma unroll
    for (int k = 0; k < kU; k++)
      if (slot[k] >= 0) atomicAdd(&cp->acc[slot[k]], rsum[k]);
  }
  __syncthreads();
  MK_CTICK(1);
  for (int h = tid; h < nh; h += NT) {
    double total = 0;
    int n = 0;
    for (int l = 0; l < ngr; l++) {
      const int i = h * ngr + l;
      if (cp->yf[i] & 1) {
        total += (double)cp->acc[i] / (double)(10 * 10);
        n++;
      }
    }
    err[h] = n <= 0 ? DBL_MAX : total / ((double)n * 1.1);
  }
  __syncthreads();
}

#ifndef MK_SCR_UNROLL
#define MK_SCR_UNROLL 6
#endif
constexpr int kScrUnroll = MK_SCR_UNROLL;
struct UQueue {
  uint32_t* e;
  int32_t* n;
  int cap;
};
template <class MK>
__device__ __attribute__((noinline)) bool exact_term(const Xf& T, const double* X, const Cam& cm, int W, int H, const uint8_t* bgr,
                                  const MK& mask, int& e) {
  double rp[3], u, v;
  xf_apply(T, X, rp);
  distort(cm, rp[0], rp[1], rp[2], &u, &v);
  if (!(rp[2] > 0 && in_frame(u, v, H, W))) return false;
  const int npx = W * H;
  int x = cv_round(u), y = cv_round(v);
  const int li = y * W + x;
  const bool ok = li >= 0 && li < npx;
  if (x >= W) { x -= W; y += 1; }
  e = 3 * 255 * 255;
  if (ok && mask.test(mask.word(li, x, y), x)) {
    const uint32_t pv = load_bgr(bgr, li, npx);
    const int b = (int)(pv & 0xffu) - 255, g = (int)((pv >> 8) & 0xffu) - 255, r = (int)((pv >> 16) & 0xffu) - 255;
    e = b * b + g * g + r * r;
  }
  return true;
}
__device__ inline float rfl(float v) {
  return __builtin_bit_cast(float, __builtin_amdgcn_readfirstlane(__builtin_bit_cast(int, v)));
}
__device__ inline PoseF rfl(const PoseF& P) {
  PoseF u;
#pragma unroll
  for (int k = 0; k < 9; k++) u.R[k] = rfl(P.R[k]);
#pragma unroll
  for (int k = 0; k < 3; k++) u.t[k] = rfl(P.t[k]);
  u.tn = rfl(P.tn);
  u.pad[0] = u.pad[1] = u.pad[2] = 0.f;
  return u;
}
template <int U, class MK, class LM>
__device__ inline void wave_sums_screen_t(const PoseF& P, const LM& lm_at, int lb, int le, const ScreenCam& sc, int W,
                                          int H, const uint8_t* bgr, const MK& mask, UQueue q, int tag, const Xf* Tx,
                                          const double* lmd, const Cam* cmp, long long& s_out, int& n_out) {
  const int lane = threadIdx.x & 63;
  int s = 0, n = 0;
  for (int b0 = lb; b0 < le; b0 += 64 * U) {
    int st[U], lin[U], px[U], py[U];
#pragma unroll
    for (int k = 0; k < U; k++) {
      const int l = b0 + lane + 64 * k;
      const float4 L = lm_at(k, l < le ? l : le - 1);
      int x, y;
      const int t = screen_project(P, L.x, L.y, L.z, L.w, sc, W, H, &x, &y);
      st[k] = l < le ? t : SCR_OUT;
      const bool in = st[k] == SCR_IN;
      px[k] = in ? x : 0;
      py[k] = in ? y : 0;
      lin[k] = in ? (int)__umul24((uint32_t)y, (uint32_t)W) + x : 0;
    }
    uint32_t mw[U];
#pragma unroll
    for (int k = 0; k < U; k++) mw[k] = mask.word(lin[k], px[k], py[k]);
    uint32_t pv[U];
    int hm[U];
#pragma unroll
    for (int k = 0; k < U; k++) {
      const bool hit = st[k] == SCR_IN && mask.test(mw[k], px[k]);
      hm[k] = hit ? -1 : 0;
      uint32_t l3;
      asm("v_lshl_add_u32 %0, %1, 1, %1" : "=v"(l3) : "v"(lin[k]));
      const uint32_t off = hit ? l3 - 1u : 0u;
      typedef __attribute__((address_space(1), aligned(1))) const uint32_t gu32u;
      pv[k] = *(gu32u*)(gbytes(bgr) + off);
    }
#pragma unroll
    for (int k = 0; k < U; k++) asm volatile("" : "+v"(pv[k]));
    int cu = 0;
#pragma unroll
    for (int k = 0; k < U; k++) {
      cu += st[k] == SCR_UNSURE;
      const uint32_t d = ~(pv[k] >> 8) & 0xffffffu;
      const int term = (int)__builtin_amdgcn_udot4(d, d, 0u, false);
      constexpr int kBlack = 3 * 255 * 255;
      const int e = kBlack ^ ((term ^ kBlack) & hm[k]);
      const int im = st[k] == SCR_IN ? -1 : 0;
      n -= im;
      s += e & im;
    }
    if (__ballot(cu > 0)) {
      const int incl = wave_incl_scan(cu, lane);
      int base = 0;
      if (lane == 63) base = atomicAdd(q.n, incl);
      base = __builtin_amdgcn_readlane(base, 63);
      int idx = base + incl - cu;
#pragma unroll
      for (int k = 0; k < U; k++) {
        if (st[k] != SCR_UNSURE) continue;
        const int l = b0 + lane + 64 * k;
        if (idx < q.cap) {
          q.e[idx] = ((uint32_t)tag << 16) | (uint32_t)l;
        } else {
          int e;
          if (exact_term(*Tx, lmd + 3 * l, *cmp, W, H, bgr, mask, e)) { n++; s += e; }
        }
        idx++;
      }
    }
  }
  s_out = wave_sum(s);
  n_out = wave_sum(n);
}
template <int U, class MK>
__device__ inline void wave_sums_screen(const PoseF& P, const float4* lmf, int lb, int le, const ScreenCam& sc, int W,
                                        int H, const uint8_t* bgr, const MK& mask, UQueue q, int tag, const Xf* Tx,
                                        const double* lmd, const Cam* cmp, long long& s_out, int& n_out) {
  wave_sums_screen_t<U>(P, [&](int, int l) { return lmf[l]; }, lb, le, sc, W, H, bgr, mask, q, tag, Tx, lmd, cmp,
                        s_out, n_out);
}
template <int U>
struct WaveLms {
  float4 L[U];
  int lb, le;
  __device__ void load(const float4* lmf, int lb_, int le_) {
    lb = lb_;
    le = le_;
    const int lane = threadIdx.x & 63;
#pragma unroll
    for (int k = 0; k < U; k++) {
      const int l = lb + lane + 64 * k;
      L[k] = lmf[l < le ? l : le - 1];
    }
  }
  template <class MK>
  __device__ void sums(const PoseF& P, const ScreenCam& sc, int W, int H, const uint8_t* bgr, const MK& mask, UQueue q,
                       int tag, const Xf* Tx, const double* lmd, const Cam* cmp, long long& s_out, int& n_out) const {
    wave_sums_screen_t<U>(P, [&](int k, int) { return L[k]; }, lb, le, sc, W, H, bgr, mask, q, tag, Tx, lmd, cmp, s_out,
                          n_out);
  }
};
template <class MK, class PoseOf, class Add>
__device__ inline void block_drain(UQueue q, const double* lmd, const Cam* cmp, int W, int H, const uint8_t* bgr,
                                   const MK& mask, const PoseOf& pose_of, const Add& add) {
  const int n = min(*q.n, q.cap);
  for (int i = threadIdx.x; i < n; i += blockDim.x) {
    const uint32_t en = q.e[i];
    const int tag = (int)(en >> 16), l = (int)(en & 0xffffu);
    int e;
    if (exact_term(pose_of(tag), lmd + 3 * l, *cmp, W, H, bgr, mask, e)) add(tag, e);
  }
}

#ifndef MK_PF_THREADS
#define MK_PF_THREADS 1024
#endif
constexpr int kPfThreads = MK_PF_THREADS;
#ifndef MK_PF_SPLIT
#define MK_PF_SPLIT 2
#endif
constexpr int kPfSplit = MK_PF_SPLIT;
#ifndef MK_SCORE_TAIL_THREADS
#define MK_SCORE_TAIL_THREADS 1024
#endif
constexpr int kScoreTail = MK_SCORE_TAIL_THREADS;
#ifndef MK_SCORE_INIT_THREADS
#define MK_SCORE_INIT_THREADS 1024
#endif
constexpr int kScoreInit = MK_SCORE_INIT_THREADS;
constexpr int kInitQueue = 1024, kPfQueue = 1024, kTailQueue = 512;
static_assert(kScoreTail >= 128 && kScoreTail % 64 == 0, "score tail block");

struct PoseLds {
  Xf c2w, w2c;
  Quat q;
  double err;
};
constexpr int kPfMaxParticles = 96;
struct ScoreState {
  PoseLds cur;
  int32_t nsc, ctr;
  long long psum[kPfMaxParticles];
  int32_t pcnt[kPfMaxParticles];
};

__device__ inline double rfl(double v) {
  const unsigned long long b = (unsigned long long)__double_as_longlong(v);
  const unsigned lo = (unsigned)__builtin_amdgcn_readfirstlane((int)(unsigned)b);
  const unsigned hi = (unsigned)__builtin_amdgcn_readfirstlane((int)(unsigned)(b >> 32));
  return __longlong_as_double((long long)(((unsigned long long)hi << 32) | lo));
}
__device__ inline Xf rfl(const Xf& T) {
  Xf u;
#pragma unroll
  for (int k = 0; k < 9; k++) u.R[k] = rfl(T.R[k]);
#pragma unroll
  for (int k = 0; k < 3; k++) u.t[k] = rfl(T.t[k]);
  return u;
}

__device__ inline void score_early_result(const FrameState& s, mantis_cam_result& R, FrameDebug& D) {
  R.status = 0;
  R.reason = s.n_quads == 0 ? MANTIS_NO_QUADS : MANTIS_NO_HYPS;
  R.publish = 0;
  R.n_quads = s.n_quads;
  R.n_hyps = s.n_hyps;
  R.n_scored = 0;
  D.reason = R.reason;
  D.publish = 0;
}

template <int NT, class MK>
__device__ inline void block_score_init(const FrameDesc& fd, const Cam* cmp, const MK& mask, const Landmarks& lmk,
                                        const WaveLms<kScrUnroll>& wl, HypRec* Hh, int C, FrameDebug& D, ErrIdx* ei,
                                        unsigned long long* hs, int32_t* hn, PoseF* pfi, int npfi, UQueue q,
                                        int32_t* uqn, PoseLds& cur, int32_t& nsc, int32_t& uniq_bi, ScoreState& S) {
  const int tid = threadIdx.x, wave = tid >> 6, lane = tid & 63;
  const int W = fd.w, H = fd.h;
  if (tid == 0) *uqn = 0;
  for (int h = tid; h < C; h += NT) {
    hs[h] = 0;
    hn[h] = 0;
    if (h < npfi) pfi[h] = posef_from(Hh[h].c2w);
  }
  __syncthreads();
  for (int t = __builtin_amdgcn_readfirstlane(wave); t < 2 * C; t += (NT / 64)) {
    const int h = t >> 1;
    long long s;
    int n;
    const PoseF P = h < npfi ? pfi[h] : posef_from(Hh[h].c2w);
    wl.sums(P, fd.scam, W, H, fd.bgr, mask, q, h, &Hh[h].c2w, lmk.xyz, cmp, s, n);
    if (lane == 0) {
      atomicAdd(&hs[h], (unsigned long long)s);
      atomicAdd(&hn[h], n);
    }
  }
  __syncthreads();
  block_drain(q, lmk.xyz, cmp, W, H, fd.bgr, mask, [&](int t) -> const Xf& { return Hh[t].c2w; },
              [&](int t, int e) {
                atomicAdd(&hs[t], (unsigned long long)e);
                atomicAdd(&hn[t], 1);
              });
  __syncthreads();
  for (int h = tid; h < C; h += NT) {
    const int n = hn[h];
    const double e = n <= 0 ? DBL_MAX : (double)(long long)hs[h] / ((double)n * 1.1);
    Hh[h].error = e;
    Hh[h].nproj = n;
    ei[h].e = e;
    ei[h].i = h;
    for (int k = 0; k < 9; k++) D.hyp_c2w[h][k] = Hh[h].c2w.R[k];
    for (int k = 0; k < 3; k++) D.hyp_c2w[h][9 + k] = Hh[h].c2w.t[k];
    D.hyp_err[h] = e;
    D.hyp_n[h] = n;
  }
  __syncthreads();
  if (wave == 0) {
    double be = DBL_MAX;
    int bj = 0x7fffffff, cnt = 0;
    for (int h = lane; h < C; h += 64) {
      const double e = ei[h].e;
      if (e < be || bj == 0x7fffffff) { be = e; bj = h; cnt = 1; }
      else if (e == be) cnt++;
    }
    for (int o = 32; o > 0; o >>= 1) {
      const double oe = __shfl_xor(be, o);
      const int oj = __shfl_xor(bj, o), oc = __shfl_xor(cnt, o);
      if (oe < be) { be = oe; bj = oj; cnt = oc; }
      else if (oe == be) { cnt += oc; if (oj < bj) bj = oj; }
    }
    if (lane == 0) uniq_bi = cnt == 1 ? bj : -1;
  }
  __syncthreads();
  if (tid == 0) {
    int bi = 0;
    if (C > 1) {
      if (uniq_bi >= 0) {
        bi = uniq_bi;
      } else {
        std_sort_desc(ei, ei + C);
        bi = ei[C - 1].i;
      }
    }
    cur.c2w = Hh[bi].c2w; cur.w2c = Hh[bi].w2c; cur.q = Hh[bi].q; cur.err = Hh[bi].error;
    for (int k = 0; k < 9; k++) D.best1_c2w[k] = cur.c2w.R[k];
    for (int k = 0; k < 3; k++) D.best1_c2w[9 + k] = cur.c2w.t[k];
    D.best1_err = cur.err;
    D.pf_iter_err[0] = cur.err;
    nsc = C + 1;
    S.cur = cur;
    S.nsc = nsc;
    S.ctr = 0;
  }
  __syncthreads();
}

template <int NT>
__global__ __launch_bounds__(NT) void k_score_init(
    const FrameDesc* __restrict__ frames, const uint32_t* __restrict__ mbits, size_t bstride, Landmarks lmk,
    FrameState* st, HypRec* __restrict__ hyps, mantis_cam_result* __restrict__ res, FrameDebug* dbg,
    ScoreState* __restrict__ sst) {
  const int f = blockIdx.x;
  const int tid = threadIdx.x, wave = tid >> 6;
  const FrameDesc fd = frames[f];
  const MaskBits mask{mbits + (size_t)f * bstride, bits::tiled_rows(fd.h), fd.w};
  FrameDebug& D = dbg[f];
  const int nl = lmk.nw + lmk.nr + lmk.ng;
  __shared__ float4 lmf[768];
  __shared__ ErrIdx ei[kMaxHyps];
  __shared__ unsigned long long hs[kMaxHyps];
  __shared__ int32_t hn[kMaxHyps];
  __shared__ uint32_t uqe[kInitQueue];
  __shared__ int32_t uqn;
  __shared__ PoseLds cur;
  __shared__ int32_t nsc, uniq_bi;
  constexpr int kInitPoses = 128;
  __shared__ PoseF pfi[kInitPoses];
  if (!st[f].reaches_pf) {
    if (tid == 0) score_early_result(st[f], res[f], D);
    return;
  }
  for (int i = tid; i < nl; i += blockDim.x) lmf[i] = lmk.xyzf[i];
  __syncthreads();
  static_assert((NT / 64) % 2 == 0 && 64 * kScrUnroll * 2 >= 768, "one register trip per half");
  WaveLms<kScrUnroll> wl;
  wl.load(lmf, nl * (wave & 1) / 2, nl * ((wave & 1) + 1) / 2);
  block_score_init<NT>(fd, &frames[f].cam, mask, lmk, wl, hyps + (size_t)f * kMaxHyps, st[f].n_hyps, D, ei, hs, hn,
                       pfi, kInitPoses, UQueue{uqe, &uqn, kInitQueue}, &uqn, cur, nsc, uniq_bi, sst[f]);
}

__device__ inline void shift_values(int grid_size, double grid_spacing, double* shv) {
  double x = -((double)grid_size / 2.0) * grid_spacing + ((double)grid_spacing / 2.0);
  int k = 0;
  for (; x < ((double)grid_size / 2.0) * grid_spacing && k < 9; x += grid_spacing) shv[k++] = x;
}
__device__ inline void shift_pose(const Xf& w2c, const double* shv, int j, PoseLds& o) {
  Xf nw = w2c;
  nw.t[0] += shv[j / 9];
  nw.t[1] += shv[j % 9];
  nw.t[2] += 0.0;
  Hyp h;
  hyp_set_w2c(h, nw);
  o.c2w = h.c2w; o.w2c = h.w2c; o.q = h.q;
}

__device__ inline void pf_particle(const Xf& cur_w2c, const float* g6, Xf& w2c, Xf& c2w) {
  double yaw = (double)g6[0] * 0.03, pitch = (double)g6[1] * 0.03, roll = (double)g6[2] * 0.03;
  double tz = (double)g6[3] * 0.01, ty = (double)g6[4] * 0.01, tx = (double)g6[5] * 0.01;
  Xf rnd;
  basis_from_rpy_small(roll, pitch, yaw, rnd.R);
  rnd.t[0] = tx; rnd.t[1] = ty; rnd.t[2] = tz;
  w2c = xf_mul(cur_w2c, rnd);
  c2w = xf_inverse(w2c);
}

template <int NT, int SPLIT, bool LM>
__global__ __launch_bounds__(NT) void k_score_pf(
    const FrameDesc* __restrict__ frames, const uint32_t* __restrict__ mbits, size_t bstride, Landmarks lmk,
    const FrameState* __restrict__ st, const float* __restrict__ gauss, mantis_cam_result* __restrict__ res,
    FrameDebug* dbg, ScoreState* __restrict__ sst, int particles, int iterations, int shifts, double grid_spacing,
    int grid_size, int init, HypRec* __restrict__ hyps, unsigned char* __restrict__ init_scratch) {
  const int f = blockIdx.x;
  const int tid = threadIdx.x, wave = tid >> 6, lane = tid & 63;
  if (!st[f].reaches_pf) {
    if (init && tid == 0) score_early_result(st[f], res[f], dbg[f]);
    return;
  }
  const FrameDesc fd = frames[f];
  const int W = fd.w, H = fd.h;
  const uint32_t* fm = mbits + (size_t)f * bstride;
  extern __shared__ __align__(16) uint32_t pf_mask[];
  if (LM) {
    typedef unsigned int u32x4 __attribute__((ext_vector_type(4)));
    const int n4 = (int)(bits::tiled_words(W, H) / 4);
    const u32x4* src = (const u32x4*)fm;
    u32x4* dst = (u32x4*)pf_mask;
    for (int i = tid; i < n4; i += NT) dst[i] = src[i];
  }
  FrameDebug& D = dbg[f];
  const int nl = lmk.nw + lmk.nr + lmk.ng;
  __shared__ float4 lmf[768];
  constexpr int kPfBuf = 96 * (2 * (int)sizeof(Xf) + (int)sizeof(PoseF) + 8 + SPLIT * 12);
  __shared__ __align__(16) unsigned char pbuf[kPfBuf];
  Xf* Pc = (Xf*)pbuf;
  Xf* Pw = Pc + 96;
  PoseF* Pf = (PoseF*)(Pw + 96);
  double* Pe = (double*)(Pf + 96);
  unsigned long long* Ps = (unsigned long long*)(Pe + 96);
  int32_t* Pn = (int32_t*)(Ps + 96 * SPLIT);
  __shared__ uint32_t uqe[kPfQueue];
  __shared__ int32_t uqn;
  constexpr int kW = NT / 64;
  __shared__ Xf cur_c2w, cur_w2c;
  __shared__ double cur_err;
  for (int i = tid; i < nl; i += blockDim.x) lmf[i] = lmk.xyzf[i];
  if (tid == 0 && !init) {
    cur_c2w = sst[f].cur.c2w;
    cur_w2c = sst[f].cur.w2c;
    cur_err = sst[f].cur.err;
  }
  __syncthreads();
#if defined(MK_SCORE_TICKS) && MK_SCORE_TICKS == 2
  uint64_t tkp = wall_clock64();
  int32_t tka[6] = {0, 0, 0, 0, 0, 0};
#define MK_PTICK(k)                                \
  if (tid == 0) {                                  \
    const uint64_t nw = wall_clock64();            \
    tka[k] += (int32_t)(nw - tkp);                 \
    tkp = nw;                                      \
  }
#else
#define MK_PTICK(k)
#endif
  MK_PTICK(0);
  const float* gs = gauss + st[f].gauss_offset;
  const UQueue q{uqe, &uqn, kPfQueue};
  const MaskLds mlds{(lds_cu32*)pf_mask, bits::tiled_rows(H)};
  const MaskBits mglb{fm, bits::tiled_rows(H), W};
  static_assert(kW % SPLIT == 0 && 64 * kScrUnroll * SPLIT >= 768, "one register trip per slice");
  WaveLms<kScrUnroll> wl;
  {
    const int h = wave % SPLIT;
    wl.load(lmf, nl * h / SPLIT, nl * (h + 1) / SPLIT);
  }
  if (init) {
    static_assert(SPLIT == 2, "the init tasks use landmark halves");
    __shared__ PoseLds icur;
    __shared__ int32_t insc, iuniq;
    const int C = st[f].n_hyps;
    HypRec* Hh = hyps + (size_t)f * kMaxHyps;
    constexpr int kPer = (int)(sizeof(ErrIdx) + sizeof(unsigned long long) + sizeof(int32_t));
    const auto run = [&](unsigned char* buf) {
      ErrIdx* ei = (ErrIdx*)buf;
      unsigned long long* hs = (unsigned long long*)(ei + C);
      int32_t* hn = (int32_t*)(hs + C);
      const UQueue qi{uqe, &uqn, kPfQueue};
      if (LM) block_score_init<NT>(fd, &frames[f].cam, mlds, lmk, wl, Hh, C, D, ei, hs, hn, nullptr, 0, qi, &uqn,
                                   icur, insc, iuniq, sst[f]);
      else block_score_init<NT>(fd, &frames[f].cam, mglb, lmk, wl, Hh, C, D, ei, hs, hn, nullptr, 0, qi, &uqn, icur,
                                insc, iuniq, sst[f]);
    };
    if (C * kPer <= kPfBuf && init != 2) run(pbuf);
    else run(init_scratch + (size_t)f * kMaxHyps * kPer);
    if (tid == 0) {
      cur_c2w = icur.c2w;
      cur_w2c = icur.w2c;
      cur_err = icur.err;
    }
    __syncthreads();
  }
  const int ngs = particles * iterations * 6;
  const bool gl = ngs <= (int)(sizeof(lmf) / sizeof(float));
  float* glds = (float*)lmf;
  __syncthreads();
  if (gl)
    for (int i = tid; i < ngs; i += NT) glds[i] = gs[i];
  const float* gsrc = gl ? (const float*)glds : gs;
  const auto particle = [&](int it, int j, const Xf& w2c_cur) {
    Xf w2c, c2w;
    pf_particle(w2c_cur, gsrc + (size_t)(it * particles + j) * 6, w2c, c2w);
    Pw[j] = w2c;
    Pc[j] = c2w;
    Pf[j] = posef_from(c2w);
  };
  __syncthreads();
  if (iterations > 0)
    for (int j = tid; j < particles; j += NT) particle(0, j, cur_w2c);
  if (tid == 0) uqn = 0;
  __syncthreads();
  MK_PTICK(1);
  for (int it = 0; it < iterations; it++) {
    for (int task = __builtin_amdgcn_readfirstlane(wave); task < particles * SPLIT; task += kW) {
      const int j = task / SPLIT;
      long long sum;
      int cnt;
      if (LM) wl.sums(Pf[j], fd.scam, W, H, fd.bgr, mlds, q, j, &Pc[j], lmk.xyz, &frames[f].cam, sum, cnt);
      else wl.sums(Pf[j], fd.scam, W, H, fd.bgr, mglb, q, j, &Pc[j], lmk.xyz, &frames[f].cam, sum, cnt);
      if (lane == 0) {
        Ps[task] = (unsigned long long)sum;
        Pn[task] = cnt;
      }
    }
    __syncthreads();
    MK_PTICK(2);
    const auto pose_of = [&](int t) -> const Xf& { return Pc[t]; };
    const auto add = [&](int t, int e) {
      atomicAdd(&Ps[t * SPLIT], (unsigned long long)e);
      atomicAdd(&Pn[t * SPLIT], 1);
    };
    if (LM) block_drain(q, lmk.xyz, &frames[f].cam, W, H, fd.bgr, mlds, pose_of, add);
    else block_drain(q, lmk.xyz, &frames[f].cam, W, H, fd.bgr, mglb, pose_of, add);
    __syncthreads();
    MK_PTICK(3);
    if (wave == 0) {
      double be = DBL_MAX;
      int bj = 0x7fffffff;
      for (int j = lane; j < particles; j += 64) {
        long long sum = 0;
        int cnt = 0;
        for (int h = 0; h < SPLIT; h++) {
          sum += (long long)Ps[j * SPLIT + h];
          cnt += Pn[j * SPLIT + h];
        }
        const double e = cnt <= 0 ? DBL_MAX : (double)sum / ((double)cnt * 1.1);
        if (e < be || bj == 0x7fffffff) { be = e; bj = j; }
      }
      for (int o = 32; o > 0; o >>= 1) {
        const double oe = __shfl_xor(be, o);
        const int oj = __shfl_xor(bj, o);
        if (oe < be || (oe == be && oj < bj)) { be = oe; bj = oj; }
      }
      MK_PTICK(4);
      const bool upd = bj < particles && be < cur_err;
      const Xf nw = upd ? Pw[bj] : cur_w2c;
      if (lane == 0) {
        if (upd) {
          cur_err = be;
          cur_c2w = Pc[bj];
          cur_w2c = nw;
        }
        if (it + 1 < (int)(sizeof(D.pf_iter_err) / sizeof(double))) D.pf_iter_err[it + 1] = upd ? be : cur_err;
        uqn = 0;
      }
      if (it + 1 < iterations)
        for (int j = lane; j < particles; j += 64) particle(it + 1, j, nw);
    }
    __syncthreads();
    MK_PTICK(5);
  }
#if defined(MK_SCORE_TICKS) && MK_SCORE_TICKS == 2
  if (tid == 0)
    for (int k = 0; k < 6; k++) const_cast<FrameState*>(st)[f].ticks[k] = tka[k];
#endif
#undef MK_PTICK
  if (tid == 0) {
    ScoreState& S = sst[f];
    S.cur.c2w = cur_c2w;
    S.cur.w2c = cur_w2c;
    S.cur.q = basis_to_quat(cur_w2c.R);
    S.cur.err = cur_err;
    S.nsc += iterations * particles;
    for (int k = 0; k < 9; k++) D.pf_c2w[k] = cur_c2w.R[k];
    for (int k = 0; k < 3; k++) D.pf_c2w[9 + k] = cur_c2w.t[k];
    D.pf_err = cur_err;
    res[f].pf_error = cur_err;
  }
  if (!shifts) return;
  constexpr int NS = 81;
  static_assert(NS <= 96, "shift poses in the particle arrays");
  __shared__ double shv[9];
  if (tid == 0) {
    uqn = 0;
    shift_values(grid_size, grid_spacing, shv);
  }
  __syncthreads();
  if (tid < NS) {
    PoseLds o;
    shift_pose(cur_w2c, shv, tid, o);
    Pc[tid] = o.c2w;
    Pf[tid] = posef_from(o.c2w);
  }
  for (int i = tid; i < NS * SPLIT; i += NT) {
    Ps[i] = 0;
    Pn[i] = 0;
  }
  __syncthreads();
  for (int task = __builtin_amdgcn_readfirstlane(wave); task < NS * SPLIT; task += kW) {
    const int j = task / SPLIT;
    long long sum;
    int cnt;
    if (LM) wl.sums(Pf[j], fd.scam, W, H, fd.bgr, mlds, q, j, &Pc[j], lmk.xyz, &frames[f].cam, sum, cnt);
    else wl.sums(Pf[j], fd.scam, W, H, fd.bgr, mglb, q, j, &Pc[j], lmk.xyz, &frames[f].cam, sum, cnt);
    if (lane == 0) {
      Ps[task] = (unsigned long long)sum;
      Pn[task] = cnt;
    }
  }
  __syncthreads();
  {
    const auto pose_of = [&](int t) -> const Xf& { return Pc[t]; };
    const auto add = [&](int t, int e) {
      atomicAdd(&Ps[t * SPLIT], (unsigned long long)e);
      atomicAdd(&Pn[t * SPLIT], 1);
    };
    if (LM) block_drain(q, lmk.xyz, &frames[f].cam, W, H, fd.bgr, mlds, pose_of, add);
    else block_drain(q, lmk.xyz, &frames[f].cam, W, H, fd.bgr, mglb, pose_of, add);
  }
  __syncthreads();
  if (tid < NS) {
    long long sum = 0;
    int cnt = 0;
    for (int h = 0; h < SPLIT; h++) {
      sum += (long long)Ps[tid * SPLIT + h];
      cnt += Pn[tid * SPLIT + h];
    }
    sst[f].psum[tid] = sum;
    sst[f].pcnt[tid] = cnt;
  }
}

template <int NT, int SPLIT>
__global__ __launch_bounds__(NT) void k_score_pf_part(
    const FrameDesc* __restrict__ frames, const uint32_t* __restrict__ mbits, size_t bstride, Landmarks lmk,
    const FrameState* __restrict__ st, const float* __restrict__ gauss, mantis_cam_result* __restrict__ res,
    FrameDebug* dbg, ScoreState* __restrict__ sst, int particles, int iterations, int it, int ppb, int nblk) {
  const int f = blockIdx.y, b = blockIdx.x;
  const int tid = threadIdx.x, wave = tid >> 6, lane = tid & 63;
  if (!st[f].reaches_pf) return;
  const FrameDesc fd = frames[f];
  const int W = fd.w, H = fd.h;
  const int nl = lmk.nw + lmk.nr + lmk.ng;
  constexpr int kW = NT / 64, kPP = kW / SPLIT > 0 ? kW / SPLIT : 1;
  __shared__ float4 lmf[768];
  __shared__ Xf Pc[kPP];
  __shared__ PoseF Pf[kPP];
  __shared__ unsigned long long Ps[kPP];
  __shared__ int32_t Pn[kPP];
  __shared__ uint32_t uqe[kPfQueue];
  __shared__ int32_t uqn, last;
  ScoreState& S = sst[f];
  const int p0 = b * ppb, np = max(0, min(ppb, particles - p0));
  const float* gs = gauss + st[f].gauss_offset + (size_t)it * particles * 6;
  for (int i = tid; i < nl; i += NT) lmf[i] = lmk.xyzf[i];
  if (tid < np) {
    Xf w2c, c2w;
    pf_particle(S.cur.w2c, gs + (size_t)(p0 + tid) * 6, w2c, c2w);
    Pc[tid] = c2w;
    Pf[tid] = posef_from(c2w);
    Ps[tid] = 0;
    Pn[tid] = 0;
  }
  if (tid == 0) uqn = 0;
  __syncthreads();
  const UQueue q{uqe, &uqn, kPfQueue};
  const MaskBits mglb{mbits + (size_t)f * bstride, bits::tiled_rows(H), W};
  static_assert(kW % SPLIT == 0 && 64 * kScrUnroll * SPLIT >= 768, "one register trip per slice");
  WaveLms<kScrUnroll> wl;
  {
    const int h = wave % SPLIT;
    wl.load(lmf, nl * h / SPLIT, nl * (h + 1) / SPLIT);
  }
  for (int task = __builtin_amdgcn_readfirstlane(wave); task < np * SPLIT; task += kW) {
    const int j = task / SPLIT;
    long long sum;
    int cnt;
    wl.sums(Pf[j], fd.scam, W, H, fd.bgr, mglb, q, j, &Pc[j], lmk.xyz, &frames[f].cam, sum, cnt);
    if (lane == 0) {
      atomicAdd(&Ps[j], (unsigned long long)sum);
      atomicAdd(&Pn[j], cnt);
    }
  }
  __syncthreads();
  block_drain(q, lmk.xyz, &frames[f].cam, W, H, fd.bgr, mglb, [&](int t) -> const Xf& { return Pc[t]; },
              [&](int t, int e) {
                atomicAdd(&Ps[t], (unsigned long long)e);
                atomicAdd(&Pn[t], 1);
              });
  __syncthreads();
  if (tid < np) {
    S.psum[p0 + tid] = (long long)Ps[tid];
    S.pcnt[p0 + tid] = Pn[tid];
  }
  __threadfence();
  __syncthreads();
  if (tid == 0) last = atomicAdd(&S.ctr, 1) == nblk - 1;
  __syncthreads();
  if (!last || wave != 0) return;
  __threadfence();
  const volatile long long* vs = S.psum;
  const volatile int32_t* vc = S.pcnt;
  double be = DBL_MAX;
  int bj = 0x7fffffff;
  for (int j = lane; j < particles; j += 64) {
    const int cnt = vc[j];
    const double e = cnt <= 0 ? DBL_MAX : (double)vs[j] / ((double)cnt * 1.1);
    if (e < be || bj == 0x7fffffff) { be = e; bj = j; }
  }
  for (int o = 32; o > 0; o >>= 1) {
    const double oe = __shfl_xor(be, o);
    const int oj = __shfl_xor(bj, o);
    if (oe < be || (oe == be && oj < bj)) { be = oe; bj = oj; }
  }
  if (lane == 0) {
    FrameDebug& D = dbg[f];
    if (bj < particles && be < S.cur.err) {
      Xf w2c, c2w;
      pf_particle(S.cur.w2c, gs + (size_t)bj * 6, w2c, c2w);
      S.cur.c2w = c2w;
      S.cur.w2c = w2c;
      S.cur.err = be;
    }
    if (it + 1 < (int)(sizeof(D.pf_iter_err) / sizeof(double))) D.pf_iter_err[it + 1] = S.cur.err;
    S.ctr = 0;
    if (it == iterations - 1) {
      S.cur.q = basis_to_quat(S.cur.w2c.R);
      S.nsc += iterations * particles;
      for (int k = 0; k < 9; k++) D.pf_c2w[k] = S.cur.c2w.R[k];
      for (int k = 0; k < 3; k++) D.pf_c2w[9 + k] = S.cur.c2w.t[k];
      D.pf_err = S.cur.err;
      res[f].pf_error = S.cur.err;
    }
  }
}

template <int NT>
__global__ __launch_bounds__(NT) void k_score_shift_part(
    const FrameDesc* __restrict__ frames, const uint32_t* __restrict__ mbits, size_t bstride, Landmarks lmk,
    const FrameState* __restrict__ st, ScoreState* __restrict__ sst, double grid_spacing, int grid_size, int spb) {
  const int f = blockIdx.y, b = blockIdx.x;
  const int tid = threadIdx.x, wave = tid >> 6, lane = tid & 63;
  if (!st[f].reaches_pf) return;
  const FrameDesc fd = frames[f];
  const int W = fd.w, H = fd.h;
  const MaskBits mask{mbits + (size_t)f * bstride, bits::tiled_rows(H), W};
  const int nl = lmk.nw + lmk.nr + lmk.ng;
  constexpr int NS = 81, kMaxSpb = NT / 128 > 0 ? NT / 128 : 1;
  __shared__ float4 lmf[768];
  __shared__ PoseLds P[kMaxSpb];
  __shared__ double shv[9];
  __shared__ unsigned long long hs[kMaxSpb];
  __shared__ int32_t hn[kMaxSpb];
  __shared__ uint32_t uqe[kTailQueue];
  __shared__ int32_t uqn;
  const int j0 = b * spb, ns = max(0, min(min(spb, kMaxSpb), NS - j0));
  for (int i = tid; i < nl; i += NT) lmf[i] = lmk.xyzf[i];
  if (tid == 0) {
    uqn = 0;
    shift_values(grid_size, grid_spacing, shv);
  }
  __syncthreads();
  if (tid < ns) {
    shift_pose(sst[f].cur.w2c, shv, j0 + tid, P[tid]);
    hs[tid] = 0;
    hn[tid] = 0;
  }
  __syncthreads();
  const UQueue q{uqe, &uqn, kTailQueue};
  static_assert((NT / 64) % 2 == 0 && 64 * kScrUnroll * 2 >= 768, "one register trip per half");
  WaveLms<kScrUnroll> wl;
  wl.load(lmf, nl * (wave & 1) / 2, nl * ((wave & 1) + 1) / 2);
  for (int t = __builtin_amdgcn_readfirstlane(wave); t < 2 * ns; t += NT / 64) {
    const int j = t >> 1;
    long long sum;
    int n;
    wl.sums(posef_from(P[j].c2w), fd.scam, W, H, fd.bgr, mask, q, j, &P[j].c2w, lmk.xyz, &frames[f].cam, sum, n);
    if (lane == 0) {
      atomicAdd(&hs[j], (unsigned long long)sum);
      atomicAdd(&hn[j], n);
    }
  }
  __syncthreads();
  block_drain(q, lmk.xyz, &frames[f].cam, W, H, fd.bgr, mask, [&](int t) -> const Xf& { return P[t].c2w; },
              [&](int t, int e) {
                atomicAdd(&hs[t], (unsigned long long)e);
                atomicAdd(&hn[t], 1);
              });
  __syncthreads();
  if (tid < ns) {
    sst[f].psum[j0 + tid] = (long long)hs[tid];
    sst[f].pcnt[j0 + tid] = hn[tid];
  }
}

template <int NT>
__global__ __launch_bounds__(NT) void k_score_final(
    const FrameDesc* __restrict__ frames, const uint32_t* __restrict__ mbits, size_t bstride, Landmarks lmk,
    const FrameState* __restrict__ st, mantis_cam_result* __restrict__ res, FrameDebug* dbg,
    const ScoreState* __restrict__ sst, double grid_spacing, int grid_size, bool pre) {
  const int f = blockIdx.x;
  const int tid = threadIdx.x, wave = tid >> 6, lane = tid & 63;
  if (!st[f].reaches_pf) return;
  const FrameDesc fd = frames[f];
  const int W = fd.w, H = fd.h;
  const MaskBits mask{mbits + (size_t)f * bstride, bits::tiled_rows(H), W};
  mantis_cam_result& R = res[f];
  FrameDebug& D = dbg[f];
  const int nl = lmk.nw + lmk.nr + lmk.ng;
  __shared__ float4 lmf[768];
  __shared__ PoseLds P[96];
  __shared__ ErrIdx ei[96];
  static_assert(sizeof(ColorPairs) >= sizeof(ColorLds) * (NT / 64), "color scratch");
  __shared__ ColorPairs cpairs;
  __shared__ PoseLds cur;
  __shared__ double shv[9];
  __shared__ double yerr[4];
  __shared__ int32_t nsc;
  __shared__ unsigned long long hs[96];
  __shared__ int32_t hn[96];
  __shared__ uint32_t uqe[kTailQueue];
  __shared__ int32_t uqn;
#if defined(MK_SCORE_TICKS) && MK_SCORE_TICKS != 2
  const uint64_t tk0 = wall_clock64();
  int32_t* tk = const_cast<FrameState*>(st)[f].ticks;
#define MK_STICK(k) \
  if (tid == 0 && (MK_SCORE_TICKS != 3 || ((k) != 1 && (k) != 2))) tk[k] = (int32_t)(wall_clock64() - tk0);
#else
#define MK_STICK(k)
#endif
  for (int i = tid; i < nl; i += blockDim.x) lmf[i] = lmk.xyzf[i];
  if (tid == 0) {
    uqn = 0;
    cur = sst[f].cur;
    nsc = sst[f].nsc;
    shift_values(grid_size, grid_spacing, shv);
  }
  __syncthreads();
  const int NS = 81;
  if (tid < NS) shift_pose(cur.w2c, shv, tid, P[tid]);
  __syncthreads();
  const UQueue q{uqe, &uqn, kTailQueue};
  if (tid < NS) {
    hs[tid] = pre ? (unsigned long long)sst[f].psum[tid] : 0ull;
    hn[tid] = pre ? sst[f].pcnt[tid] : 0;
  }
  __syncthreads();
  if (!pre) {
  static_assert((NT / 64) % 2 == 0 && 64 * kScrUnroll * 2 >= 768, "one register trip per half");
  WaveLms<kScrUnroll> wl;
  wl.load(lmf, nl * (wave & 1) / 2, nl * ((wave & 1) + 1) / 2);
  for (int t = __builtin_amdgcn_readfirstlane(wave); t < 2 * NS; t += (NT / 64)) {
    const int j = t >> 1;
    long long sum;
    int n;
    wl.sums(posef_from(P[j].c2w), fd.scam, W, H, fd.bgr, mask, q, j, &P[j].c2w, lmk.xyz, &frames[f].cam, sum, n);
    if (lane == 0) {
      atomicAdd(&hs[j], (unsigned long long)sum);
      atomicAdd(&hn[j], n);
    }
  }
  __syncthreads();
  MK_STICK(0);
  block_drain(q, lmk.xyz, &frames[f].cam, W, H, fd.bgr, mask, [&](int t) -> const Xf& { return P[t].c2w; },
              [&](int t, int e) {
                atomicAdd(&hs[t], (unsigned long long)e);
                atomicAdd(&hn[t], 1);
              });
  __syncthreads();
  }
  if (tid < NS) {
    const int n = hn[tid];
    const double e = n <= 0 ? DBL_MAX : (double)(long long)hs[tid] / ((double)n * 1.1);
    P[tid].err = e;
    ei[tid].e = e;
    ei[tid].i = tid;
    D.shift_err[tid] = e;
  }
  __syncthreads();
  MK_STICK(1);
  __shared__ int32_t top[20];
  __shared__ int32_t tie20;
  if (tid == 0) tie20 = 0;
  __syncthreads();
  if (tid < NS) {
    const double e = ei[tid].e;
    int lt = 0, eq = 0;
    for (int j = 0; j < NS; j++) {
      const double o = ei[j].e;
      lt += o < e;
      eq += o == e;
    }
    if (lt < 20) {
      if (eq != 1) tie20 = 1;
      else top[19 - lt] = tid;
    }
  }
  __syncthreads();
  if (tid == 0) {
    if (tie20) {
      std_sort_desc(ei, ei + NS);
      for (int k = 0; k < 20; k++) top[k] = ei[NS - 20 + k].i;
    }
    for (int k = 0; k < 20; k++) D.top20_err[k] = P[top[k]].err;
    nsc += NS;
  }
  __syncthreads();
  MK_STICK(2);
  static_assert(sizeof(ColorPairs) >= 20 * sizeof(PoseLds), "top-20 staging");
  PoseLds* Y = (PoseLds*)&cpairs;
  if (tid < 20) {
    const PoseLds& s = P[top[tid]];
    Y[tid] = s;
  }
  __syncthreads();
  const Xf rz = make_rot_z90();
  if (tid < 20) {
    P[tid] = Y[tid];
    for (int k = 1; k < 4; k++) {
      Hyp h;
      hyp_set_w2c(h, xf_mul(rz, P[20 * (k - 1) + tid].w2c));
      PoseLds& d = P[20 * k + tid];
      d.c2w = h.c2w; d.w2c = h.w2c; d.q = h.q;
    }
  }
  __syncthreads();
  MK_STICK(3);
  const double* green = lmk.xyz + 3 * (lmk.nw + lmk.nr);
  __shared__ double yset_err[80];
  if (80 * lmk.ng <= kColorPairs) {
    block_score_color<NT>([&](int h) -> const Xf& { return P[h].c2w; }, 80, green, lmk.ng, fd.cam, fd.bgr, W, H,
                          &cpairs, yset_err
#if defined(MK_SCORE_TICKS) && MK_SCORE_TICKS == 3
                          , tk, tk0
#endif
                          );
  } else {
    ColorLds* cls = (ColorLds*)&cpairs;
    for (int j = wave; j < 80; j += (NT / 64)) {
      double e;
      int n;
      wave_score_color(P[j].c2w, green, lmk.ng, fd.cam, fd.bgr, W, H, &cls[wave], &e, &n);
      if (lane == 0) yset_err[j] = e;
    }
    __syncthreads();
  }
  MK_STICK(4);
  if (tid == 0) {
    double best_error = DBL_MAX;
    int best_k = -1;
// ... 36 lines not shown
    } else {
      for (int k = 0; k < 3; k++) { R.position[k] = pb.w2c.t[k]; D.position[k] = pb.w2c.t[k]; }
      R.orientation_xyzw[0] = pb.q.x; R.orientation_xyzw[1] = pb.q.y;
      R.orientation_xyzw[2] = pb.q.z; R.orientation_xyzw[3] = pb.q.w;
      for (int k = 0; k < 4; k++) D.orientation_xyzw[k] = R.orientation_xyzw[k];
      for (int k = 0; k < 9; k++) { R.c2w[k] = pb.c2w.R[k]; D.pub_c2w[k] = pb.c2w.R[k]; }
      for (int k = 0; k < 3; k++) { R.c2w[9 + k] = pb.c2w.t[k]; D.pub_c2w[9 + k] = pb.c2w.t[k]; }
      R.error = pb.err;
      D.pub_error = pb.err;
      if (min2 > 4000) {
        double var = pb.err * (1.0 / 600.0);
        for (int i = 0; i < 6; i++) R.covariance[i * 6 + i] = var;
        R.publish = 1;
        R.reason = MANTIS_PUBLISHED;
      } else {
        R.publish = 0;
        R.reason = MANTIS_YAW_AMBIGUOUS;
      }
      for (int i = 0; i < 36; i++) D.covariance[i] = R.covariance[i];
      D.reason = R.reason;
      D.publish = R.publish;
    }
  }
  MK_STICK(5);
#undef MK_STICK
}

struct RigWJob {
  double c2w[12];
  int32_t frame, pad;
};
struct RigWColors {
  int32_t c[9];
};
__global__ __launch_bounds__(256) void k_rig_weight(const FrameDesc* __restrict__ frames, Landmarks lmk,
                                                    const RigWJob* __restrict__ jobs, int n, RigWColors col,
                                                    double* __restrict__ out2) {
  const int lane = threadIdx.x & 63;
  const int j = blockIdx.x * 4 + (threadIdx.x >> 6);
  if (j >= n) return;
  const RigWJob& J = jobs[j];
  const FrameDesc fd = frames[J.frame];
  Xf T;
  for (int k = 0; k < 9; k++) T.R[k] = J.c2w[k];
  for (int k = 0; k < 3; k++) T.t[k] = J.c2w[9 + k];
  const int nl = lmk.nw + lmk.nr + lmk.ng;
  const long npx = (long)fd.w * fd.h;
  long long s = 0;
  int cnt = 0;
  for (int l = lane; l < nl; l += 64) {
    double rp[3], u, v;
    xf_apply(T, lmk.xyz + 3 * l, rp);
    distort(fd.cam, rp[0], rp[1], rp[2], &u, &v);
    const float fu = (float)u, fv = (float)v;
    if (!(fu > 0 && fu < (float)fd.w && fv > 0 && fv < (float)fd.h)) continue;
    cnt++;
    const int x = (int)rintf(fu), y = (int)rintf(fv);
    const long lin = (long)y * fd.w + x;
    const int set = l < lmk.nw ? 0 : (l < lmk.nw + lmk.nr ? 1 : 2);
    int b = 0, g = 0, r = 0;
    if (lin >= 0 && lin < npx) {
      const uint32_t pv = load_bgr(fd.bgr, lin, npx);
      b = (int)(pv & 0xffu);
      g = (int)((pv >> 8) & 0xffu);
      r = (int)((pv >> 16) & 0xffu);
    }
    const int e0 = b - col.c[3 * set], e1 = g - col.c[3 * set + 1], e2 = r - col.c[3 * set + 2];
    s += e0 * e0 + e1 * e1 + e2 * e2;
  }
  for (int o = 32; o > 0; o >>= 1) {
    s += __shfl_xor(s, o);
    cnt += __shfl_xor(cnt, o);
  }
  if (lane == 0) {
    out2[2 * j] = (double)s;
    out2[2 * j + 1] = (double)cnt;
  }
}

#ifndef MK_DENSE_HYPS
#define MK_DENSE_HYPS 64
#endif
constexpr int kApiHyps = 16, kApiQueue = 1024, kDenseHyps = MK_DENSE_HYPS;
template <int HPB, class MK>
__device__ inline void score_api_fast(const FrameDesc& fd, const Cam* cmp, const MK& mask, Landmarks lmk,
                                      const double* c2w, int n, double* err, int32_t* nproj) {
  constexpr int NW = kApiHyps;
  static_assert(NW % 2 == 0 && 64 * kScrUnroll * 2 >= 768, "one register trip per half");
  const int tid = threadIdx.x, wave = tid >> 6, lane = tid & 63;
  const int h0 = blockIdx.x * HPB, nh = min(HPB, n - h0);
  const int nl = lmk.nw + lmk.nr + lmk.ng;
  __shared__ float4 lmf[768];
  __shared__ unsigned long long hs[HPB];
  __shared__ int32_t hn[HPB];
  __shared__ uint32_t uqe[kApiQueue];
  __shared__ int32_t uqn;
  __shared__ PoseF pf[HPB];
  for (int i = tid; i < nl; i += blockDim.x) lmf[i] = lmk.xyzf[i];
  for (int i = tid; i < HPB; i += blockDim.x) {
    hs[i] = 0;
    hn[i] = 0;
    if (i < nh) pf[i] = posef_from(*(const Xf*)(c2w + 12 * (size_t)(h0 + i)));
  }
  if (tid == 0) uqn = 0;
  __syncthreads();
  const UQueue q{uqe, &uqn, kApiQueue};
  WaveLms<kScrUnroll> wl;
  wl.load(lmf, nl * (wave & 1) / 2, nl * ((wave & 1) + 1) / 2);
  for (int t = __builtin_amdgcn_readfirstlane(wave); t < 2 * nh; t += NW) {
    const int j = t >> 1;
    const Xf* T = (const Xf*)(c2w + 12 * (size_t)(h0 + j));
    long long s;
    int c;
    wl.sums(pf[j], fd.scam, fd.w, fd.h, fd.bgr, mask, q, j, T, lmk.xyz, cmp, s, c);
    if (lane == 0) {
      atomicAdd(&hs[j], (unsigned long long)s);
      atomicAdd(&hn[j], c);
    }
  }
  __syncthreads();
  block_drain(q, lmk.xyz, cmp, fd.w, fd.h, fd.bgr, mask,
              [&](int t) -> const Xf& { return *(const Xf*)(c2w + 12 * (size_t)(h0 + t)); },
              [&](int t, int e) {
                atomicAdd(&hs[t], (unsigned long long)e);
                atomicAdd(&hn[t], 1);
              });
  __syncthreads();
  for (int i = tid; i < nh; i += blockDim.x) {
    const int c = hn[i];
    err[h0 + i] = c <= 0 ? DBL_MAX : (double)(long long)hs[i] / ((double)c * 1.1);
    nproj[h0 + i] = c;
  }
}
__global__ __launch_bounds__(64 * kApiHyps) void k_score_api(const FrameDesc* __restrict__ frames, const uint8_t* mask,
                                                             Landmarks lmk, const double* __restrict__ c2w, int n,
                                                             int fast, double* __restrict__ err,
                                                             int32_t* __restrict__ nproj) {
  const FrameDesc fd = frames[0];
  if (fast) {
    if (mask) score_api_fast<kApiHyps>(fd, &frames[0].cam, MaskBytes{mask}, lmk, c2w, n, err, nproj);
    else score_api_fast<kApiHyps>(fd, &frames[0].cam, MaskNone{}, lmk, c2w, n, err, nproj);
    return;
  }
  const int wave = threadIdx.x >> 6, lane = threadIdx.x & 63;
  const int h = blockIdx.x * kApiHyps + wave;
  __shared__ ColorLds cls[kApiHyps];
  if (h >= n) return;
  Xf T;
  for (int k = 0; k < 9; k++) T.R[k] = c2w[12 * h + k];
  for (int k = 0; k < 3; k++) T.t[k] = c2w[12 * h + 9 + k];
  double e;
  int np;
  wave_score_color(T, lmk.xyz + 3 * (lmk.nw + lmk.nr), lmk.ng, fd.cam, fd.bgr, fd.w, fd.h, &cls[wave], &e, &np);
  if (lane == 0) {
    err[h] = e;
    nproj[h] = np;
  }
}

__global__ __launch_bounds__(256) void k_synth(const mantis_synth::Cam* __restrict__ cams, const uint64_t* seeds,
                                               uint8_t* out, size_t plane) {
  const int f = blockIdx.y;
  const mantis_synth::Cam c = cams[f];
  const size_t n = (size_t)c.w * c.h;
  for (size_t p = (size_t)blockIdx.x * blockDim.x + threadIdx.x; p < n; p += (size_t)gridDim.x * blockDim.x)
    mantis_synth::render_pixel(c, (int)(p % c.w), (int)(p / c.w), seeds[f], out + (size_t)f * plane + 3 * p);
}

}
```

### mantis_amd/csrc/track_impl.hip

```cpp
#include "mk_track.h"

namespace mk {

struct TrackState {
  Xf cur;
  double err;
  int32_t n, pad;
};

struct TrackArgs {
  const Xf* pred;
  const Xf* ext;
  const float* gauss;
  TrackState* st;
  mantis_track_result* res;
  Xf* Twb;
  Xf* c2w;
  PoseF* pf;
  long long* sums;
  int32_t* cnt;
  size_t pass_poses, pass_tasks;
  int32_t C, P, iterations, min_projections;
  double sigma_rot, sigma_t, max_error;
};
// ... 4 lines not shown
  TrackState& S = a.st[rig];
  mantis_track_result& R = a.res[rig];
  Xf cur;
  double cur_err = DBL_MAX;
  int32_t cur_n = 0;
  if (call == 0) {
    cur = a.pred[rig];
  } else {
    const int pass = call - 1, np = pass == 0 ? 1 : P;
    const size_t t0 = (size_t)pass * a.pass_tasks + (size_t)rig * P * C;
    double be = DBL_MAX;
    int bj = 0x7fffffff;
    int32_t bn = 0;
    for (int j = lane; j < np; j += 64) {
      int32_t n;
      const double e = track::pool(a.sums + t0 + (size_t)j * C, a.cnt + t0 + (size_t)j * C, C, &n);
      if (track::before(e, j, be, bj)) { be = e; bj = j; bn = n; }
    }
    for (int o = 32; o > 0; o >>= 1) {
      const double oe = __shfl_xor(be, o);
      const int oj = __shfl_xor(bj, o);
      const int32_t on = __shfl_xor(bn, o);
      if (track::before(oe, oj, be, bj)) { be = oe; bj = oj; bn = on; }
    }
    if (pass == 0) {
      cur = S.cur;
      cur_err = be;
      cur_n = bn;
      if (lane == 0) R.seed_error = R.iter_err[0] = be;
    } else {
      cur_err = S.err;
      cur_n = S.n;
      const bool take = bj < np && be < cur_err;
      cur = take ? a.Twb[(size_t)pass * a.pass_poses + (size_t)rig * P + bj] : S.cur;
      if (take) { cur_err = be; cur_n = bn; }
      if (lane == 0) {
        R.iter_pick[pass - 1] = take ? bj : -1;
        R.iter_err[pass] = cur_err;
      }
    }
  }
  if (call <= a.iterations) {
    const int np = call == 0 ? 1 : P;
    const float* g = a.gauss + ((size_t)rig * a.iterations + (call > 0 ? call - 1 : 0)) * P * 6;
    const size_t p0 = (size_t)call * a.pass_poses + (size_t)rig * P;
    const size_t t0 = (size_t)call * a.pass_tasks + (size_t)rig * P * C;
    for (int j = lane; j < np; j += 64) {
      const Xf T = call == 0 ? cur : track::particle(cur, g + (size_t)j * 6, a.sigma_rot, a.sigma_t);
      a.Twb[p0 + j] = T;
      for (int c = 0; c < C; c++) {
        const Xf v = track::cam_c2w(T, a.ext[(size_t)rig * C + c]);
        a.c2w[t0 + (size_t)j * C + c] = v;
        a.pf[t0 + (size_t)j * C + c] = posef_from(v);
      }
    }
  }
  if (lane == 0) {
    S.cur = cur;
    S.err = cur_err;
    S.n = cur_n;
    if (call == a.iterations + 1) {
      R.status = MANTIS_OK;
      R.n_proj = cur_n;
      R.n_scored = 1 + P * a.iterations;
      R.error = cur_err;
      R.tracked = track::gate(cur_err, cur_n, a.min_projections, a.max_error);
      track::xf_to_mat4(cur, R.T_w_b);
    }
  }
}

template <int NT, int SPLIT>
__device__ __forceinline__ void track_score_block(const FrameDesc* __restrict__ frames,
                                                  const uint32_t* __restrict__ mbits, size_t bstride,
                                                  const Landmarks& lmk, const Xf* __restrict__ c2w,
                                                  const PoseF* __restrict__ pf, long long* __restrict__ sums,
                                                  int32_t* __restrict__ cnt, size_t t0, int C, int f, int cam,
                                                  int chunk, int np) {
  const int tid = threadIdx.x, wave = tid >> 6, lane = tid & 63;
  constexpr int kW = NT / 64, kPP = kW / SPLIT;
  static_assert(kW % SPLIT == 0 && kPP >= 1 && 64 * kScrUnroll * SPLIT >= 768, "one register trip per slice");
  const FrameDesc fd = frames[f];
  const int W = fd.w, H = fd.h;
  const int nl = lmk.nw + lmk.nr + lmk.ng;
  __shared__ float4 lmf[768];
  __shared__ Xf Pc[kPP];
  __shared__ PoseF Pf[kPP];
  __shared__ unsigned long long Ps[kPP];
  __shared__ int32_t Pn[kPP];
  __shared__ uint32_t uqe[kPfQueue];
  __shared__ int32_t uqn;
  const int j0 = chunk * kPP, nj = max(0, min(kPP, np - j0));
  for (int i = tid; i < nl; i += NT) lmf[i] = lmk.xyzf[i];
  if (tid < nj) {
    const size_t t = t0 + (size_t)(j0 + tid) * C + cam;
    Pc[tid] = c2w[t];
    Pf[tid] = pf[t];
    Ps[tid] = 0;
    Pn[tid] = 0;
  }
  if (tid == 0) uqn = 0;
  __syncthreads();
  const UQueue q{uqe, &uqn, kPfQueue};
  const MaskBits mask{mbits + (size_t)f * bstride, bits::tiled_rows(H), W};
  WaveLms<kScrUnroll> wl;
  {
    const int h = wave % SPLIT;
    wl.load(lmf, nl * h / SPLIT, nl * (h + 1) / SPLIT);
  }
  for (int task = __builtin_amdgcn_readfirstlane(wave); task < nj * SPLIT; task += kW) {
    const int j = task / SPLIT;
    long long sum;
    int cnt;
    wl.sums(Pf[j], fd.scam, W, H, fd.bgr, mask, q, j, &Pc[j], lmk.xyz, &frames[f].cam, sum, cnt);
    if (lane == 0) {
      atomicAdd(&Ps[j], (unsigned long long)sum);
      atomicAdd(&Pn[j], cnt);
    }
  }
  __syncthreads();
  block_drain(q, lmk.xyz, &frames[f].cam, W, H, fd.bgr, mask, [&](int t) -> const Xf& { return Pc[t]; },
              [&](int t, int e) {
                atomicAdd(&Ps[t], (unsigned long long)e);
                atomicAdd(&Pn[t], 1);
              });
  __syncthreads();
  if (tid < nj) {
    const size_t t = t0 + (size_t)(j0 + tid) * C + cam;
    sums[t] = (long long)Ps[tid];
    cnt[t] = Pn[tid];
  }
}
template <int NT, int SPLIT>
__global__ __launch_bounds__(NT) void k_track_score(const FrameDesc* __restrict__ frames,
                                                    const uint32_t* __restrict__ mbits, size_t bstride, Landmarks lmk,
                                                    TrackArgs a, int pass, int np) {
  const int chunk = blockIdx.x, cam = blockIdx.y, rig = blockIdx.z;
  track_score_block<NT, SPLIT>(frames, mbits, bstride, lmk, a.c2w, a.pf, a.sums, a.cnt,
                               (size_t)pass * a.pass_tasks + (size_t)rig * a.P * a.C, a.C, rig * a.C + cam, cam, chunk,
                               np);
}
constexpr int kTrackPP = (kPfThreads / 64) / kPfSplit;

}

namespace {

namespace trk = mk::track;

template <class T>
mantis_status track_grow(Ctx* c, T** p, size_t count) {
  if (*p) (void)hipFree(*p);
  *p = nullptr;
  return dalloc(c, p, count);
}

mantis_status track_workspace(Ctx* c, int R, int C, int P, int I, bool record) {
  Ctx::Track& t = c->trk;
  const size_t in_bytes = sizeof(Xf) * ((size_t)R + (size_t)R * C) + sizeof(float) * (size_t)R * I * P * 6;
  const size_t passes = record ? (size_t)I + 1 : 1;
  const size_t poses = passes * R * P, tasks = poses * C;
  if (in_bytes > t.in_cap || R > t.rig_cap || poses > t.pose_cap || tasks > t.task_cap)
    HIP_OK(hipStreamSynchronize(c->s));
  if (in_bytes > t.in_cap) {
    t.in_cap = 0;
    if (t.h_in) (void)hipHostFree(t.h_in);
    t.h_in = nullptr;
    if (track_grow(c, (uint8_t**)&t.d_in, in_bytes) || halloc(c, (uint8_t**)&t.h_in, in_bytes)) return MANTIS_ERR_OOM;
    t.in_cap = in_bytes;
  }
  if (R > t.rig_cap) {
    t.rig_cap = 0;
    if (t.h_res) (void)hipHostFree(t.h_res);
    t.h_res = nullptr;
    if (track_grow(c, (TrackState**)&t.d_state, (size_t)R) || track_grow(c, (mantis_track_result**)&t.d_res, (size_t)R) ||
        halloc(c, (mantis_track_result**)&t.h_res, (size_t)R))
      return MANTIS_ERR_OOM;
    t.rig_cap = R;
  }
  if (poses > t.pose_cap) {
    t.pose_cap = 0;
    if (track_grow(c, (Xf**)&t.d_Twb, poses)) return MANTIS_ERR_OOM;
    t.pose_cap = poses;
  }
  if (tasks > t.task_cap) {
    t.task_cap = 0;
    if (track_grow(c, (Xf**)&t.d_c2w, tasks) || track_grow(c, (PoseF**)&t.d_pf, tasks) ||
        track_grow(c, &t.d_sums, tasks) || track_grow(c, &t.d_cnt, tasks))
      return MANTIS_ERR_OOM;
    t.task_cap = tasks;
  }
  return MANTIS_OK;
}

mantis_status track_fail(Ctx* c, const char* what) {
  c->err = std::string("track: ") + what;
  return MANTIS_ERR_ARG;
}

mantis_status track_impl(Ctx* c, const mantis_image* cams, int32_t n_rigs, int32_t C, const double* pred,
                         const mantis_track_params* p, mantis_track_result* out) {
  if (!cams || !pred || !p || !out) return track_fail(c, "null argument");
  if (p->struct_size != (int32_t)sizeof(mantis_track_params)) return track_fail(c, "params.struct_size mismatch");
  if (!c->d_lm || c->nw + c->nr + c->ng <= 0) return track_fail(c, "map not set (mantis_set_map)");
  if (n_rigs <= 0 || C <= 0) return track_fail(c, "n_rigs and cams_per_rig must be positive");
  if (C > trk::kMaxCams) return track_fail(c, "cams_per_rig exceeds 8");
  if ((int64_t)n_rigs * C > c->F) return track_fail(c, "n_rigs x cams_per_rig exceeds max_cams");
// ... 202 lines not shown
```

Measured before the change: 30480 rig poses/s.

## Deduplicate identical landmarks with multiplicity weights and narrow unroll when few remain

Identical landmark coordinates are merged on the host at upload into a unique set with per-landmark counts. All screen-scoring kernels (particle filter, shift, tracking, dense API) iterate over the unique set and weight errors and projection counts by multiplicity. When the unique count fits in fewer register slots, a narrower-unroll kernel variant is chosen. This reduces projection work only if the map contains duplicates, and adds a weight multiply per landmark plus more kernel instantiations.

```diff
diff --git a/mantis_amd/csrc/api.hip b/mantis_amd/csrc/api.hip
--- a/mantis_amd/csrc/api.hip
+++ b/mantis_amd/csrc/api.hip
@@ -104,6 +104,8 @@
   uint64_t rng_state = 1;
   double* d_lm = nullptr;
   int nw = 0, nr = 0, ng = 0;
+  int nd = 0;
+  bool lm_dedupe = true;
   int F = 0, Wmax = 0, Hmax = 0;
   int n_cu = 256;
   bool trace_lds_ok = false;
@@ -222,7 +224,7 @@
   int32_t* d_agree = nullptr;
   bool agreed_fail = false;
   struct CallGraph {
-    int n = 0, W = 0, H = 0, live = 0, nw = 0, nr = 0, ng = 0;
+    int n = 0, W = 0, H = 0, live = 0, nw = 0, nr = 0, ng = 0, nd = 0;
     bool vec = false;
     const void* lm = nullptr;
     const void* gauss = nullptr;
@@ -300,8 +302,11 @@
 }
 
 inline Landmarks lmk_of(const Ctx* c) {
-  return Landmarks{c->d_lm, c->nw, c->nr, c->ng, c->d_lm ? (const float4*)(c->d_lm + kLmfOffset) : nullptr};
-}
+  if (!c->d_lm) return Landmarks{nullptr, c->nw, c->nr, c->ng, nullptr, nullptr, nullptr, nullptr, 0};
+  return Landmarks{c->d_lm, c->nw, c->nr, c->ng, (const float4*)(c->d_lm + kLmfOffset), c->d_lm + kLmdOffset,
+                   (const float4*)(c->d_lm + kLmdfOffset), (const int32_t*)(c->d_lm + kLmwOffset), c->nd};
+}
+inline bool lm_narrow(const Ctx* c, int split) { return lm_trip_slots(c->nd, split, kScrUnroll) < kScrUnroll; }
 
 void mark(Ctx* c, const char* name) {
   if (!c->prof) return;
@@ -666,26 +671,30 @@
   constexpr int ppb = std::max(1, kPfThreads / 64 / kPfSplit);
   if (split) {
     const int nblk = (c->cfg.particles + ppb - 1) / ppb;
+    const auto kpart = lm_narrow(c, kPfSplit) ? k_score_pf_part<kPfThreads, kPfSplit, kScrUnroll - 1>
+                                              : k_score_pf_part<kPfThreads, kPfSplit, kScrUnroll>;
     for (int it = 0; it < c->cfg.iterations; it++)
-      k_score_pf_part<kPfThreads, kPfSplit><<<dim3(nblk, n), kPfThreads, 0, c->s>>>(
-          c->d_frames, c->d_mbits, c->bstride, L, c->d_st, c->d_gauss, c->d_res, c->d_dbg, c->d_sst, c->cfg.particles,
-          c->cfg.iterations, it, ppb, nblk);
-  } else if (ml)
-    k_score_pf<kPfThreads, kPfSplit, true><<<n, kPfThreads, ml, c->s>>>(
-        c->d_frames, c->d_mbits, c->bstride, L, c->d_st, c->d_gauss, c->d_res, c->d_dbg, c->d_sst, c->cfg.particles,
-        c->cfg.iterations, pf_shifts ? 1 : 0, c->cfg.grid_spacing, 9, pf_init, c->d_hyps,
-        (unsigned char*)c->d_gen);
-  else
-    k_score_pf<kPfThreads, kPfSplit, false><<<n, kPfThreads, 0, c->s>>>(
-        c->d_frames, c->d_mbits, c->bstride, L, c->d_st, c->d_gauss, c->d_res, c->d_dbg, c->d_sst, c->cfg.particles,
-        c->cfg.iterations, pf_shifts ? 1 : 0, c->cfg.grid_spacing, 9, pf_init, c->d_hyps,
-        (unsigned char*)c->d_gen);
+      kpart<<<dim3(nblk, n), kPfThreads, 0, c->s>>>(c->d_frames, c->d_mbits, c->bstride, L, c->d_st, c->d_gauss, c->d_res,
+                                                    c->d_dbg, c->d_sst, c->cfg.particles, c->cfg.iterations, it, ppb,
+                                                    nblk);
+  } else {
+    const bool narrow = lm_narrow(c, kPfSplit);
+    const auto kpf = ml ? (narrow ? k_score_pf<kPfThreads, kPfSplit, true, kScrUnroll - 1>
+                                  : k_score_pf<kPfThreads, kPfSplit, true, kScrUnroll>)
+                        : (narrow ? k_score_pf<kPfThreads, kPfSplit, false, kScrUnroll - 1>
+                                  : k_score_pf<kPfThreads, kPfSplit, false, kScrUnroll>);
+    kpf<<<n, kPfThreads, ml, c->s>>>(c->d_frames, c->d_mbits, c->bstride, L, c->d_st, c->d_gauss, c->d_res, c->d_dbg,
+                                     c->d_sst, c->cfg.particles, c->cfg.iterations, pf_shifts ? 1 : 0,
+                                     c->cfg.grid_spacing, 9, pf_init, c->d_hyps, (unsigned char*)c->d_gen);
+  }
   mark(c, "score_pf_yaw/k_score_pf");
   const bool shifts_apart = !pf_shifts && (split || c->shift_split);
   if (shifts_apart) {
     constexpr int spb = kScoreTail / 128;
-    k_score_shift_part<kScoreTail><<<dim3((81 + spb - 1) / spb, n), kScoreTail, 0, c->s>>>(
-        c->d_frames, c->d_mbits, c->bstride, L, c->d_st, c->d_sst, c->cfg.grid_spacing, 9, spb);
+    const auto kshift = lm_narrow(c, 2) ? k_score_shift_part<kScoreTail, kScrUnroll - 1>
+                                        : k_score_shift_part<kScoreTail, kScrUnroll>;
+    kshift<<<dim3((81 + spb - 1) / spb, n), kScoreTail, 0, c->s>>>(c->d_frames, c->d_mbits, c->bstride, L, c->d_st,
+                                                                   c->d_sst, c->cfg.grid_spacing, 9, spb);
     mark(c, "score_pf_yaw/k_score_shift_part");
   }
   k_score_final<kScoreTail><<<n, kScoreTail, 0, c->s>>>(c->d_frames, c->d_mbits, c->bstride, L, c->d_st, c->d_res, c->d_dbg,
@@ -775,7 +784,7 @@
   const int live = std::max(1, g_live_ctx[c->cfg.device & 63].load());
   for (auto& g : c->graphs)
     if (g.n == n && g.W == W && g.H == H && g.vec == c->vec_ok && g.live == live && g.lm == c->d_lm &&
-        g.nw == c->nw && g.nr == c->nr && g.ng == c->ng && g.gauss == c->d_gauss)
+        g.nw == c->nw && g.nr == c->nr && g.ng == c->ng && g.nd == c->nd && g.gauss == c->d_gauss)
       return &g;
   if (c->graphs.size() >= 8) {
     if (c->graphs.front().pre) (void)hipGraphExecDestroy(c->graphs.front().pre);
@@ -784,7 +793,7 @@
   }
   Ctx::CallGraph g;
   g.n = n; g.W = W; g.H = H; g.vec = c->vec_ok; g.live = live;
-  g.lm = c->d_lm; g.nw = c->nw; g.nr = c->nr; g.ng = c->ng; g.gauss = c->d_gauss;
+  g.lm = c->d_lm; g.nw = c->nw; g.nr = c->nr; g.ng = c->ng; g.nd = c->nd; g.gauss = c->d_gauss;
   c->graphs.push_back(g);
   return &c->graphs.back();
 }
@@ -1035,6 +1044,8 @@
     c->trace_lds_max = 160 * 1024 - 512 * 8 - 64;
     c->trace_lds_ok = hipFuncSetAttribute((const void*)k_trace_borders_lds, hipFuncAttributeMaxDynamicSharedMemorySize,
                                           (int)c->trace_lds_max) == hipSuccess;
+    const char* ld = getenv("MANTIS_LM_DEDUPE");
+    c->lm_dedupe = !(ld && ld[0] == '0');
     const char* so = getenv("MANTIS_SCREEN");
     c->screen_off = so && so[0] == '0';
     const char* e = getenv("MANTIS_TRACE_LDS_FRAMES");
@@ -1048,11 +1059,14 @@
     const size_t ml = bits::tiled_words(c->Wmax, c->Hmax) * 4;
     hipFuncAttributes a1;
     c->pf_mask_lds = 0;
-    if (!getenv("MANTIS_PF_MASK_GLOBAL") &&
-        hipFuncGetAttributes(&a1, (const void*)k_score_pf<kPfThreads, kPfSplit, true>) == hipSuccess &&
-        a1.sharedSizeBytes + ml <= 160 * 1024 &&
-        hipFuncSetAttribute((const void*)k_score_pf<kPfThreads, kPfSplit, true>,
-                            hipFuncAttributeMaxDynamicSharedMemorySize, (int)ml) == hipSuccess)
+    const void* kn = (const void*)k_score_pf<kPfThreads, kPfSplit, true, kScrUnroll - 1>;
+    const void* kw = (const void*)k_score_pf<kPfThreads, kPfSplit, true, kScrUnroll>;
+    hipFuncAttributes a2;
+    if (!getenv("MANTIS_PF_MASK_GLOBAL") && hipFuncGetAttributes(&a1, kn) == hipSuccess &&
+        hipFuncGetAttributes(&a2, kw) == hipSuccess &&
+        std::max(a1.sharedSizeBytes, a2.sharedSizeBytes) + ml <= 160 * 1024 &&
+        hipFuncSetAttribute(kn, hipFuncAttributeMaxDynamicSharedMemorySize, (int)ml) == hipSuccess &&
+        hipFuncSetAttribute(kw, hipFuncAttributeMaxDynamicSharedMemorySize, (int)ml) == hipSuccess)
       c->pf_mask_lds = ml;
   }
   {
@@ -1223,10 +1237,14 @@
   all.insert(all.end(), red, red + 3 * nr);
   all.insert(all.end(), green, green + 3 * ng);
   const size_t nl = (size_t)nw + nr + ng;
-  std::vector<double> buf(kLmfOffset + 2 * 768, 0.0);
+  std::vector<double> buf(kLmBufDoubles, 0.0);
   std::copy(all.begin(), all.end(), buf.begin());
   float* lf = (float*)(buf.data() + kLmfOffset);
   for (size_t i = 0; i < nl; i++) screen_landmark(all.data() + 3 * i, lf + 4 * i);
+  const int nd = lm_dedupe(all.data(), (int)nl, c->lm_dedupe, buf.data() + kLmdOffset,
+                           (int32_t*)(buf.data() + kLmwOffset), nullptr);
+  float* ldf = (float*)(buf.data() + kLmdfOffset);
+  for (int i = 0; i < nd; i++) screen_landmark(buf.data() + kLmdOffset + 3 * i, ldf + 4 * i);
   if (c->d_lm) (void)hipFree(c->d_lm);
   c->d_lm = nullptr;
   if (dalloc(c, &c->d_lm, buf.size()) != MANTIS_OK) return MANTIS_ERR_OOM;
@@ -1234,6 +1252,7 @@
   c->nw = nw;
   c->nr = nr;
   c->ng = ng;
+  c->nd = nd;
   return MANTIS_OK;
 }
 
@@ -1797,7 +1816,8 @@
   HIP_OK(hipMemcpyAsync(d_c2w, c2w, sizeof(double) * 12 * n, hipMemcpyHostToDevice, c->s));
   Landmarks L = lmk_of(c);
   mark(c, "start");
-  k_score_api<<<(n + kApiHyps - 1) / kApiHyps, 64 * kApiHyps, 0, c->s>>>(c->d_frames, d_mask, L, d_c2w, n, fast, d_err, d_np);
+  const auto kapi = lm_narrow(c, 2) ? k_score_api<kScrUnroll - 1> : k_score_api<kScrUnroll>;
+  kapi<<<(n + kApiHyps - 1) / kApiHyps, 64 * kApiHyps, 0, c->s>>>(c->d_frames, d_mask, L, d_c2w, n, fast, d_err, d_np);
   mark(c, "score_api");
   HIP_OK(hipGetLastError());
   HIP_OK(hipMemcpyAsync(err, d_err, sizeof(double) * n, hipMemcpyDeviceToHost, c->s));
diff --git a/mantis_amd/csrc/dense_impl.hip b/mantis_amd/csrc/dense_impl.hip
--- a/mantis_amd/csrc/dense_impl.hip
+++ b/mantis_amd/csrc/dense_impl.hip
@@ -35,6 +35,7 @@
   int32_t n, err_off;
   int64_t index_base;
 };
+template <int U>
 __global__ __launch_bounds__(64 * kApiHyps) void k_score_api_batch(const FrameDesc* __restrict__ frames,
                                                                    const DenseJob* __restrict__ jobs, Landmarks lmk,
                                                                    double* __restrict__ err, int32_t* __restrict__ nproj) {
@@ -43,10 +44,11 @@
   if ((int)blockIdx.x * kDenseHyps >= J.n) return;
   const FrameDesc fd = frames[f];
   if (J.mask)
-    score_api_fast<kDenseHyps>(fd, &frames[f].cam, MaskBytes{J.mask}, lmk, J.c2w, J.n, err + J.err_off,
-                               nproj + J.err_off);
+    score_api_fast<kDenseHyps, U>(fd, &frames[f].cam, MaskBytes{J.mask}, lmk, J.c2w, J.n, err + J.err_off,
+                                  nproj + J.err_off);
   else
-    score_api_fast<kDenseHyps>(fd, &frames[f].cam, MaskNone{}, lmk, J.c2w, J.n, err + J.err_off, nproj + J.err_off);
+    score_api_fast<kDenseHyps, U>(fd, &frames[f].cam, MaskNone{}, lmk, J.c2w, J.n, err + J.err_off,
+                                  nproj + J.err_off);
 }
 __global__ __launch_bounds__(1024) void k_argmin_batch(const DenseJob* __restrict__ jobs, const double* __restrict__ err,
                                                        double* __restrict__ out2) {
@@ -151,8 +153,9 @@
   Landmarks L = lmk_of(c);
   mark(c, "start");
   if (n > 0) {
-    k_score_api<<<(n + kApiHyps - 1) / kApiHyps, 64 * kApiHyps, 0, c->s>>>(c->d_frames, d_mask, L, d_c2w, n, 1, c->d_dense_err,
-                                               c->d_dense_np);
+    const auto kapi = lm_narrow(c, 2) ? k_score_api<kScrUnroll - 1> : k_score_api<kScrUnroll>;
+    kapi<<<(n + kApiHyps - 1) / kApiHyps, 64 * kApiHyps, 0, c->s>>>(c->d_frames, d_mask, L, d_c2w, n, 1, c->d_dense_err,
+                                                                   c->d_dense_np);
     mark(c, "score_dense");
   }
   k_argmin<<<1, 1024, 0, c->s>>>(c->d_dense_err, n, index_base, c->d_pairs);
@@ -237,9 +240,11 @@
   HIP_OK(hipMemcpyAsync(d_jobs, jobs.data(), sizeof(DenseJob) * n_frames, hipMemcpyHostToDevice, c->s));
   Landmarks L = lmk_of(c);
   mark(c, "start");
-  if (maxn > 0)
-    k_score_api_batch<<<dim3((maxn + kDenseHyps - 1) / kDenseHyps, n_frames), 64 * kApiHyps, 0, c->s>>>(
+  if (maxn > 0) {
+    const auto kbatch = lm_narrow(c, 2) ? k_score_api_batch<kScrUnroll - 1> : k_score_api_batch<kScrUnroll>;
+    kbatch<<<dim3((maxn + kDenseHyps - 1) / kDenseHyps, n_frames), 64 * kApiHyps, 0, c->s>>>(
         c->d_frames, d_jobs, L, c->d_dense_err, c->d_dense_np);
+  }
   mark(c, "score_dense");
   k_argmin_batch<<<n_frames, 1024, 0, c->s>>>(d_jobs, c->d_dense_err, c->d_pairs);
   mark(c, "argmin");
diff --git a/mantis_amd/csrc/hostcheck.cpp b/mantis_amd/csrc/hostcheck.cpp
--- a/mantis_amd/csrc/hostcheck.cpp
+++ b/mantis_amd/csrc/hostcheck.cpp
@@ -8,6 +8,7 @@
 #include "mk_bits.h"
 #include "mk_contour.h"
 #include "mk_gn.h"
+#include "mk_lmdedupe.h"
 #include "mk_math.h"
 #include "mk_mcl.h"
 #include "mk_mcl_color.h"
@@ -484,4 +485,9 @@
     L_out[j] = mk::mcl::log_weight_color(L[j], E[j], n_proj[j], min_projections, tau, charge[j]);
 }
 
-}
+int hc_lm_dedupe(const double* xyz, int n, int merge, double* out_xyz, int32_t* out_w, int32_t* out_first) {
+  return mk::lm_dedupe(xyz, n, merge != 0, out_xyz, out_w, out_first);
+}
+int hc_lm_trip_slots(int nd, int split, int wide) { return mk::lm_trip_slots(nd, split, wide); }
+
+}
diff --git a/mantis_amd/csrc/kernels.hip b/mantis_amd/csrc/kernels.hip
--- a/mantis_amd/csrc/kernels.hip
+++ b/mantis_amd/csrc/kernels.hip
@@ -6,6 +6,7 @@
 #include "mk_bits.h"
 #include "mk_contour.h"
 #include "mk_gn.h"
+#include "mk_lmdedupe.h"
 #include "mk_math.h"
 #include "mk_rpp.h"
 #include "mk_shard.h"
@@ -3548,8 +3549,13 @@
   const double* xyz;
   int32_t nw, nr, ng;
   const float4* xyzf;
+  const double* dxyz;
+  const float4* dxyzf;
+  const int32_t* dw;
+  int32_t nd;
 };
-constexpr int kLmfOffset = 3 * 768;
+constexpr int kLmfOffset = 3 * 768, kLmdOffset = kLmfOffset + 2 * 768, kLmdfOffset = kLmdOffset + 3 * 768,
+              kLmwOffset = kLmdfOffset + 2 * 768, kLmBufDoubles = kLmwOffset + 768 / 2;
 
 struct MaskNone {
   __device__ uint32_t word(int, int, int) const { return 1u; }
@@ -3846,10 +3852,11 @@
   u.pad[0] = u.pad[1] = u.pad[2] = 0.f;
   return u;
 }
-template <int U, class MK, class LM>
-__device__ inline void wave_sums_screen_t(const PoseF& P, const LM& lm_at, int lb, int le, const ScreenCam& sc, int W,
-                                          int H, const uint8_t* bgr, const MK& mask, UQueue q, int tag, const Xf* Tx,
-                                          const double* lmd, const Cam* cmp, long long& s_out, int& n_out) {
+template <int U, class MK, class LM, class WT>
+__device__ inline void wave_sums_screen_t(const PoseF& P, const LM& lm_at, const WT& wt_at, int lb, int le,
+                                          const ScreenCam& sc, int W, int H, const uint8_t* bgr, const MK& mask,
+                                          UQueue q, int tag, const Xf* Tx, const double* lmd, const Cam* cmp,
+                                          long long& s_out, int& n_out) {
   const int lane = threadIdx.x & 63;
   int s = 0, n = 0;
   for (int b0 = lb; b0 < le; b0 += 64 * U) {
@@ -3891,9 +3898,9 @@
       const int term = (int)__builtin_amdgcn_udot4(d, d, 0u, false);
       constexpr int kBlack = 3 * 255 * 255;
       const int e = kBlack ^ ((term ^ kBlack) & hm[k]);
-      const int im = st[k] == SCR_IN ? -1 : 0;
-      n -= im;
-      s += e & im;
+      const int wm = st[k] == SCR_IN ? wt_at(k) : 0;
+      n += wm;
+      s += (int)__umul24((uint32_t)e, (uint32_t)wm);
     }
     if (__ballot(cu > 0)) {
       const int incl = wave_incl_scan(cu, lane);
@@ -3909,7 +3916,10 @@
           q.e[idx] = ((uint32_t)tag << 16) | (uint32_t)l;
         } else {
           int e;
-          if (exact_term(*Tx, lmd + 3 * l, *cmp, W, H, bgr, mask, e)) { n++; s += e; }
+          if (exact_term(*Tx, lmd + 3 * l, *cmp, W, H, bgr, mask, e)) {
+            n += wt_at(k);
+            s += e * wt_at(k);
+          }
         }
         idx++;
       }
@@ -3917,44 +3927,42 @@
   }
   s_out = wave_sum(s);
   n_out = wave_sum(n);
-}
-template <int U, class MK>
-__device__ inline void wave_sums_screen(const PoseF& P, const float4* lmf, int lb, int le, const ScreenCam& sc, int W,
-                                        int H, const uint8_t* bgr, const MK& mask, UQueue q, int tag, const Xf* Tx,
-                                        const double* lmd, const Cam* cmp, long long& s_out, int& n_out) {
-  wave_sums_screen_t<U>(P, [&](int, int l) { return lmf[l]; }, lb, le, sc, W, H, bgr, mask, q, tag, Tx, lmd, cmp,
-                        s_out, n_out);
 }
 template <int U>
 struct WaveLms {
   float4 L[U];
+  int w[U];
   int lb, le;
-  __device__ void load(const float4* lmf, int lb_, int le_) {
+  __device__ void load(const float4* lmf, const int32_t* wt, int lb_, int le_) {
     lb = lb_;
     le = le_;
     const int lane = threadIdx.x & 63;
 #pragma unroll
     for (int k = 0; k < U; k++) {
       const int l = lb + lane + 64 * k;
-      L[k] = lmf[l < le ? l : le - 1];
+      L[k] = lmf[l < le ? l : max(le - 1, 0)];
+      w[k] = l < le ? wt[l] : 0;
     }
   }
   template <class MK>
   __device__ void sums(const PoseF& P, const ScreenCam& sc, int W, int H, const uint8_t* bgr, const MK& mask, UQueue q,
                        int tag, const Xf* Tx, const double* lmd, const Cam* cmp, long long& s_out, int& n_out) const {
-    wave_sums_screen_t<U>(P, [&](int k, int) { return L[k]; }, lb, le, sc, W, H, bgr, mask, q, tag, Tx, lmd, cmp, s_out,
-                          n_out);
+    wave_sums_screen_t<U>(P, [&](int k, int) { return L[k]; }, [&](int k) { return w[k]; }, lb, le, sc, W, H, bgr, mask,
+                          q, tag, Tx, lmd, cmp, s_out, n_out);
   }
 };
 template <class MK, class PoseOf, class Add>
-__device__ inline void block_drain(UQueue q, const double* lmd, const Cam* cmp, int W, int H, const uint8_t* bgr,
-                                   const MK& mask, const PoseOf& pose_of, const Add& add) {
+__device__ inline void block_drain(UQueue q, const double* lmd, const int32_t* wt, const Cam* cmp, int W, int H,
+                                   const uint8_t* bgr, const MK& mask, const PoseOf& pose_of, const Add& add) {
   const int n = min(*q.n, q.cap);
   for (int i = threadIdx.x; i < n; i += blockDim.x) {
     const uint32_t en = q.e[i];
     const int tag = (int)(en >> 16), l = (int)(en & 0xffffu);
     int e;
-    if (exact_term(pose_of(tag), lmd + 3 * l, *cmp, W, H, bgr, mask, e)) add(tag, e);
+    if (exact_term(pose_of(tag), lmd + 3 * l, *cmp, W, H, bgr, mask, e)) {
+      const int w = wt[l];
+      add(tag, e * w, w);
+    }
   }
 }
 
@@ -4016,9 +4024,9 @@
   D.publish = 0;
 }
 
-template <int NT, class MK>
+template <int NT, int U, class MK>
 __device__ inline void block_score_init(const FrameDesc& fd, const Cam* cmp, const MK& mask, const Landmarks& lmk,
-                                        const WaveLms<kScrUnroll>& wl, HypRec* Hh, int C, FrameDebug& D, ErrIdx* ei,
+                                        const WaveLms<U>& wl, HypRec* Hh, int C, FrameDebug& D, ErrIdx* ei,
                                         unsigned long long* hs, int32_t* hn, PoseF* pfi, int npfi, UQueue q,
                                         int32_t* uqn, PoseLds& cur, int32_t& nsc, int32_t& uniq_bi, ScoreState& S) {
   const int tid = threadIdx.x, wave = tid >> 6, lane = tid & 63;
@@ -4035,17 +4043,17 @@
     long long s;
     int n;
     const PoseF P = h < npfi ? pfi[h] : posef_from(Hh[h].c2w);
-    wl.sums(P, fd.scam, W, H, fd.bgr, mask, q, h, &Hh[h].c2w, lmk.xyz, cmp, s, n);
+    wl.sums(P, fd.scam, W, H, fd.bgr, mask, q, h, &Hh[h].c2w, lmk.dxyz, cmp, s, n);
     if (lane == 0) {
       atomicAdd(&hs[h], (unsigned long long)s);
       atomicAdd(&hn[h], n);
     }
   }
   __syncthreads();
-  block_drain(q, lmk.xyz, cmp, W, H, fd.bgr, mask, [&](int t) -> const Xf& { return Hh[t].c2w; },
-              [&](int t, int e) {
+  block_drain(q, lmk.dxyz, lmk.dw, cmp, W, H, fd.bgr, mask, [&](int t) -> const Xf& { return Hh[t].c2w; },
+              [&](int t, int e, int w) {
                 atomicAdd(&hs[t], (unsigned long long)e);
-                atomicAdd(&hn[t], 1);
+                atomicAdd(&hn[t], w);
               });
   __syncthreads();
   for (int h = tid; h < C; h += NT) {
@@ -4111,7 +4119,7 @@
   const FrameDesc fd = frames[f];
   const MaskBits mask{mbits + (size_t)f * bstride, bits::tiled_rows(fd.h), fd.w};
   FrameDebug& D = dbg[f];
-  const int nl = lmk.nw + lmk.nr + lmk.ng;
+  const int nl = lmk.nd;
   __shared__ float4 lmf[768];
   __shared__ ErrIdx ei[kMaxHyps];
   __shared__ unsigned long long hs[kMaxHyps];
@@ -4126,11 +4134,11 @@
     if (tid == 0) score_early_result(st[f], res[f], D);
     return;
   }
-  for (int i = tid; i < nl; i += blockDim.x) lmf[i] = lmk.xyzf[i];
+  for (int i = tid; i < nl; i += blockDim.x) lmf[i] = lmk.dxyzf[i];
   __syncthreads();
   static_assert((NT / 64) % 2 == 0 && 64 * kScrUnroll * 2 >= 768, "one register trip per half");
   WaveLms<kScrUnroll> wl;
-  wl.load(lmf, nl * (wave & 1) / 2, nl * ((wave & 1) + 1) / 2);
+  wl.load(lmf, lmk.dw, nl * (wave & 1) / 2, nl * ((wave & 1) + 1) / 2);
   block_score_init<NT>(fd, &frames[f].cam, mask, lmk, wl, hyps + (size_t)f * kMaxHyps, st[f].n_hyps, D, ei, hs, hn,
                        pfi, kInitPoses, UQueue{uqe, &uqn, kInitQueue}, &uqn, cur, nsc, uniq_bi, sst[f]);
 }
@@ -4160,7 +4168,7 @@
   c2w = xf_inverse(w2c);
 }
 
-template <int NT, int SPLIT, bool LM>
+template <int NT, int SPLIT, bool LM, int U>
 __global__ __launch_bounds__(NT) void k_score_pf(
     const FrameDesc* __restrict__ frames, const uint32_t* __restrict__ mbits, size_t bstride, Landmarks lmk,
     const FrameState* __restrict__ st, const float* __restrict__ gauss, mantis_cam_result* __restrict__ res,
@@ -4184,7 +4192,7 @@
     for (int i = tid; i < n4; i += NT) dst[i] = src[i];
   }
   FrameDebug& D = dbg[f];
-  const int nl = lmk.nw + lmk.nr + lmk.ng;
+  const int nl = lmk.nd;
   __shared__ float4 lmf[768];
   constexpr int kPfBuf = 96 * (2 * (int)sizeof(Xf) + (int)sizeof(PoseF) + 8 + SPLIT * 12);
   __shared__ __align__(16) unsigned char pbuf[kPfBuf];
@@ -4199,7 +4207,7 @@
   constexpr int kW = NT / 64;
   __shared__ Xf cur_c2w, cur_w2c;
   __shared__ double cur_err;
-  for (int i = tid; i < nl; i += blockDim.x) lmf[i] = lmk.xyzf[i];
+  for (int i = tid; i < nl; i += blockDim.x) lmf[i] = lmk.dxyzf[i];
   if (tid == 0 && !init) {
     cur_c2w = sst[f].cur.c2w;
     cur_w2c = sst[f].cur.w2c;
@@ -4223,11 +4231,12 @@
   const UQueue q{uqe, &uqn, kPfQueue};
   const MaskLds mlds{(lds_cu32*)pf_mask, bits::tiled_rows(H)};
   const MaskBits mglb{fm, bits::tiled_rows(H), W};
-  static_assert(kW % SPLIT == 0 && 64 * kScrUnroll * SPLIT >= 768, "one register trip per slice");
-  WaveLms<kScrUnroll> wl;
+  static_assert(kW % SPLIT == 0 && 64 * kScrUnroll * SPLIT >= 768 && (U == kScrUnroll || U == kScrUnroll - 1),
+                "one register trip per slice: the wide form holds any map, the launch picks the narrow one");
+  WaveLms<U> wl;
   {
     const int h = wave % SPLIT;
-    wl.load(lmf, nl * h / SPLIT, nl * (h + 1) / SPLIT);
+    wl.load(lmf, lmk.dw, nl * h / SPLIT, nl * (h + 1) / SPLIT);
   }
   if (init) {
     static_assert(SPLIT == 2, "the init tasks use landmark halves");
@@ -4280,8 +4289,8 @@
       const int j = task / SPLIT;
       long long sum;
       int cnt;
-      if (LM) wl.sums(Pf[j], fd.scam, W, H, fd.bgr, mlds, q, j, &Pc[j], lmk.xyz, &frames[f].cam, sum, cnt);
-      else wl.sums(Pf[j], fd.scam, W, H, fd.bgr, mglb, q, j, &Pc[j], lmk.xyz, &frames[f].cam, sum, cnt);
+      if (LM) wl.sums(Pf[j], fd.scam, W, H, fd.bgr, mlds, q, j, &Pc[j], lmk.dxyz, &frames[f].cam, sum, cnt);
+      else wl.sums(Pf[j], fd.scam, W, H, fd.bgr, mglb, q, j, &Pc[j], lmk.dxyz, &frames[f].cam, sum, cnt);
       if (lane == 0) {
         Ps[task] = (unsigned long long)sum;
         Pn[task] = cnt;
@@ -4290,12 +4299,12 @@
     __syncthreads();
     MK_PTICK(2);
     const auto pose_of = [&](int t) -> const Xf& { return Pc[t]; };
-    const auto add = [&](int t, int e) {
+    const auto add = [&](int t, int e, int w) {
       atomicAdd(&Ps[t * SPLIT], (unsigned long long)e);
-      atomicAdd(&Pn[t * SPLIT], 1);
+      atomicAdd(&Pn[t * SPLIT], w);
     };
-    if (LM) block_drain(q, lmk.xyz, &frames[f].cam, W, H, fd.bgr, mlds, pose_of, add);
-    else block_drain(q, lmk.xyz, &frames[f].cam, W, H, fd.bgr, mglb, pose_of, add);
+    if (LM) block_drain(q, lmk.dxyz, lmk.dw, &frames[f].cam, W, H, fd.bgr, mlds, pose_of, add);
+    else block_drain(q, lmk.dxyz, lmk.dw, &frames[f].cam, W, H, fd.bgr, mglb, pose_of, add);
     __syncthreads();
     MK_PTICK(3);
     if (wave == 0) {
@@ -4375,8 +4384,8 @@
     const int j = task / SPLIT;
     long long sum;
     int cnt;
-    if (LM) wl.sums(Pf[j], fd.scam, W, H, fd.bgr, mlds, q, j, &Pc[j], lmk.xyz, &frames[f].cam, sum, cnt);
-    else wl.sums(Pf[j], fd.scam, W, H, fd.bgr, mglb, q, j, &Pc[j], lmk.xyz, &frames[f].cam, sum, cnt);
+    if (LM) wl.sums(Pf[j], fd.scam, W, H, fd.bgr, mlds, q, j, &Pc[j], lmk.dxyz, &frames[f].cam, sum, cnt);
+    else wl.sums(Pf[j], fd.scam, W, H, fd.bgr, mglb, q, j, &Pc[j], lmk.dxyz, &frames[f].cam, sum, cnt);
     if (lane == 0) {
       Ps[task] = (unsigned long long)sum;
       Pn[task] = cnt;
@@ -4385,12 +4394,12 @@
   __syncthreads();
   {
     const auto pose_of = [&](int t) -> const Xf& { return Pc[t]; };
-    const auto add = [&](int t, int e) {
+    const auto add = [&](int t, int e, int w) {
       atomicAdd(&Ps[t * SPLIT], (unsigned long long)e);
-      atomicAdd(&Pn[t * SPLIT], 1);
+      atomicAdd(&Pn[t * SPLIT], w);
     };
-    if (LM) block_drain(q, lmk.xyz, &frames[f].cam, W, H, fd.bgr, mlds, pose_of, add);
-    else block_drain(q, lmk.xyz, &frames[f].cam, W, H, fd.bgr, mglb, pose_of, add);
+    if (LM) block_drain(q, lmk.dxyz, lmk.dw, &frames[f].cam, W, H, fd.bgr, mlds, pose_of, add);
+    else block_drain(q, lmk.dxyz, lmk.dw, &frames[f].cam, W, H, fd.bgr, mglb, pose_of, add);
   }
   __syncthreads();
   if (tid < NS) {
@@ -4405,7 +4414,7 @@
   }
 }
 
-template <int NT, int SPLIT>
+template <int NT, int SPLIT, int U>
 __global__ __launch_bounds__(NT) void k_score_pf_part(
     const FrameDesc* __restrict__ frames, const uint32_t* __restrict__ mbits, size_t bstride, Landmarks lmk,
     const FrameState* __restrict__ st, const float* __restrict__ gauss, mantis_cam_result* __restrict__ res,
@@ -4415,7 +4424,7 @@
   if (!st[f].reaches_pf) return;
   const FrameDesc fd = frames[f];
   const int W = fd.w, H = fd.h;
-  const int nl = lmk.nw + lmk.nr + lmk.ng;
+  const int nl = lmk.nd;
   constexpr int kW = NT / 64, kPP = kW / SPLIT > 0 ? kW / SPLIT : 1;
   __shared__ float4 lmf[768];
   __shared__ Xf Pc[kPP];
@@ -4427,7 +4436,7 @@
   ScoreState& S = sst[f];
   const int p0 = b * ppb, np = max(0, min(ppb, particles - p0));
   const float* gs = gauss + st[f].gauss_offset + (size_t)it * particles * 6;
-  for (int i = tid; i < nl; i += NT) lmf[i] = lmk.xyzf[i];
+  for (int i = tid; i < nl; i += NT) lmf[i] = lmk.dxyzf[i];
   if (tid < np) {
     Xf w2c, c2w;
     pf_particle(S.cur.w2c, gs + (size_t)(p0 + tid) * 6, w2c, c2w);
@@ -4440,27 +4449,28 @@
   __syncthreads();
   const UQueue q{uqe, &uqn, kPfQueue};
   const MaskBits mglb{mbits + (size_t)f * bstride, bits::tiled_rows(H), W};
-  static_assert(kW % SPLIT == 0 && 64 * kScrUnroll * SPLIT >= 768, "one register trip per slice");
-  WaveLms<kScrUnroll> wl;
+  static_assert(kW % SPLIT == 0 && 64 * kScrUnroll * SPLIT >= 768 && (U == kScrUnroll || U == kScrUnroll - 1),
+                "one register trip per slice");
+  WaveLms<U> wl;
   {
     const int h = wave % SPLIT;
-    wl.load(lmf, nl * h / SPLIT, nl * (h + 1) / SPLIT);
+    wl.load(lmf, lmk.dw, nl * h / SPLIT, nl * (h + 1) / SPLIT);
   }
   for (int task = __builtin_amdgcn_readfirstlane(wave); task < np * SPLIT; task += kW) {
     const int j = task / SPLIT;
     long long sum;
     int cnt;
-    wl.sums(Pf[j], fd.scam, W, H, fd.bgr, mglb, q, j, &Pc[j], lmk.xyz, &frames[f].cam, sum, cnt);
+    wl.sums(Pf[j], fd.scam, W, H, fd.bgr, mglb, q, j, &Pc[j], lmk.dxyz, &frames[f].cam, sum, cnt);
     if (lane == 0) {
       atomicAdd(&Ps[j], (unsigned long long)sum);
       atomicAdd(&Pn[j], cnt);
     }
   }
   __syncthreads();
-  block_drain(q, lmk.xyz, &frames[f].cam, W, H, fd.bgr, mglb, [&](int t) -> const Xf& { return Pc[t]; },
-              [&](int t, int e) {
+  block_drain(q, lmk.dxyz, lmk.dw, &frames[f].cam, W, H, fd.bgr, mglb, [&](int t) -> const Xf& { return Pc[t]; },
+              [&](int t, int e, int w) {
                 atomicAdd(&Ps[t], (unsigned long long)e);
-                atomicAdd(&Pn[t], 1);
+                atomicAdd(&Pn[t], w);
               });
   __syncthreads();
   if (tid < np) {
@@ -4509,7 +4519,7 @@
   }
 }
 
-template <int NT>
+template <int NT, int U>
 __global__ __launch_bounds__(NT) void k_score_shift_part(
     const FrameDesc* __restrict__ frames, const uint32_t* __restrict__ mbits, size_t bstride, Landmarks lmk,
     const FrameState* __restrict__ st, ScoreState* __restrict__ sst, double grid_spacing, int grid_size, int spb) {
@@ -4519,7 +4529,7 @@
   const FrameDesc fd = frames[f];
   const int W = fd.w, H = fd.h;
   const MaskBits mask{mbits + (size_t)f * bstride, bits::tiled_rows(H), W};
-  const int nl = lmk.nw + lmk.nr + lmk.ng;
+  const int nl = lmk.nd;
   constexpr int NS = 81, kMaxSpb = NT / 128 > 0 ? NT / 128 : 1;
   __shared__ float4 lmf[768];
   __shared__ PoseLds P[kMaxSpb];
@@ -4529,7 +4539,7 @@
   __shared__ uint32_t uqe[kTailQueue];
   __shared__ int32_t uqn;
   const int j0 = b * spb, ns = max(0, min(min(spb, kMaxSpb), NS - j0));
-  for (int i = tid; i < nl; i += NT) lmf[i] = lmk.xyzf[i];
+  for (int i = tid; i < nl; i += NT) lmf[i] = lmk.dxyzf[i];
   if (tid == 0) {
     uqn = 0;
     shift_values(grid_size, grid_spacing, shv);
@@ -4542,24 +4552,25 @@
   }
   __syncthreads();
   const UQueue q{uqe, &uqn, kTailQueue};
-  static_assert((NT / 64) % 2 == 0 && 64 * kScrUnroll * 2 >= 768, "one register trip per half");
-  WaveLms<kScrUnroll> wl;
-  wl.load(lmf, nl * (wave & 1) / 2, nl * ((wave & 1) + 1) / 2);
+  static_assert((NT / 64) % 2 == 0 && 64 * kScrUnroll * 2 >= 768 && (U == kScrUnroll || U == kScrUnroll - 1),
+                "one register trip per half");
+  WaveLms<U> wl;
+  wl.load(lmf, lmk.dw, nl * (wave & 1) / 2, nl * ((wave & 1) + 1) / 2);
   for (int t = __builtin_amdgcn_readfirstlane(wave); t < 2 * ns; t += NT / 64) {
     const int j = t >> 1;
     long long sum;
     int n;
-    wl.sums(posef_from(P[j].c2w), fd.scam, W, H, fd.bgr, mask, q, j, &P[j].c2w, lmk.xyz, &frames[f].cam, sum, n);
+    wl.sums(posef_from(P[j].c2w), fd.scam, W, H, fd.bgr, mask, q, j, &P[j].c2w, lmk.dxyz, &frames[f].cam, sum, n);
     if (lane == 0) {
       atomicAdd(&hs[j], (unsigned long long)sum);
       atomicAdd(&hn[j], n);
     }
   }
   __syncthreads();
-  block_drain(q, lmk.xyz, &frames[f].cam, W, H, fd.bgr, mask, [&](int t) -> const Xf& { return P[t].c2w; },
-              [&](int t, int e) {
+  block_drain(q, lmk.dxyz, lmk.dw, &frames[f].cam, W, H, fd.bgr, mask, [&](int t) -> const Xf& { return P[t].c2w; },
+              [&](int t, int e, int w) {
                 atomicAdd(&hs[t], (unsigned long long)e);
-                atomicAdd(&hn[t], 1);
+                atomicAdd(&hn[t], w);
               });
   __syncthreads();
   if (tid < ns) {
@@ -4581,7 +4592,7 @@
   const MaskBits mask{mbits + (size_t)f * bstride, bits::tiled_rows(H), W};
   mantis_cam_result& R = res[f];
   FrameDebug& D = dbg[f];
-  const int nl = lmk.nw + lmk.nr + lmk.ng;
+  const int nl = lmk.nd;
   __shared__ float4 lmf[768];
   __shared__ PoseLds P[96];
   __shared__ ErrIdx ei[96];
@@ -4603,7 +4614,7 @@
 #else
 #define MK_STICK(k)
 #endif
-  for (int i = tid; i < nl; i += blockDim.x) lmf[i] = lmk.xyzf[i];
+  for (int i = tid; i < nl; i += blockDim.x) lmf[i] = lmk.dxyzf[i];
   if (tid == 0) {
     uqn = 0;
     cur = sst[f].cur;
@@ -4623,12 +4634,12 @@
   if (!pre) {
   static_assert((NT / 64) % 2 == 0 && 64 * kScrUnroll * 2 >= 768, "one register trip per half");
   WaveLms<kScrUnroll> wl;
-  wl.load(lmf, nl * (wave & 1) / 2, nl * ((wave & 1) + 1) / 2);
+  wl.load(lmf, lmk.dw, nl * (wave & 1) / 2, nl * ((wave & 1) + 1) / 2);
   for (int t = __builtin_amdgcn_readfirstlane(wave); t < 2 * NS; t += (NT / 64)) {
     const int j = t >> 1;
     long long sum;
     int n;
-    wl.sums(posef_from(P[j].c2w), fd.scam, W, H, fd.bgr, mask, q, j, &P[j].c2w, lmk.xyz, &frames[f].cam, sum, n);
+    wl.sums(posef_from(P[j].c2w), fd.scam, W, H, fd.bgr, mask, q, j, &P[j].c2w, lmk.dxyz, &frames[f].cam, sum, n);
     if (lane == 0) {
       atomicAdd(&hs[j], (unsigned long long)sum);
       atomicAdd(&hn[j], n);
@@ -4636,10 +4647,10 @@
   }
   __syncthreads();
   MK_STICK(0);
-  block_drain(q, lmk.xyz, &frames[f].cam, W, H, fd.bgr, mask, [&](int t) -> const Xf& { return P[t].c2w; },
-              [&](int t, int e) {
+  block_drain(q, lmk.dxyz, lmk.dw, &frames[f].cam, W, H, fd.bgr, mask, [&](int t) -> const Xf& { return P[t].c2w; },
+              [&](int t, int e, int w) {
                 atomicAdd(&hs[t], (unsigned long long)e);
-                atomicAdd(&hn[t], 1);
+                atomicAdd(&hn[t], w);
               });
   __syncthreads();
   }
@@ -4842,21 +4853,22 @@
 #define MK_DENSE_HYPS 64
 #endif
 constexpr int kApiHyps = 16, kApiQueue = 1024, kDenseHyps = MK_DENSE_HYPS;
-template <int HPB, class MK>
+template <int HPB, int U, class MK>
 __device__ inline void score_api_fast(const FrameDesc& fd, const Cam* cmp, const MK& mask, Landmarks lmk,
                                       const double* c2w, int n, double* err, int32_t* nproj) {
   constexpr int NW = kApiHyps;
-  static_assert(NW % 2 == 0 && 64 * kScrUnroll * 2 >= 768, "one register trip per half");
+  static_assert(NW % 2 == 0 && 64 * kScrUnroll * 2 >= 768 && (U == kScrUnroll || U == kScrUnroll - 1),
+                "one register trip per half");
   const int tid = threadIdx.x, wave = tid >> 6, lane = tid & 63;
   const int h0 = blockIdx.x * HPB, nh = min(HPB, n - h0);
-  const int nl = lmk.nw + lmk.nr + lmk.ng;
+  const int nl = lmk.nd;
   __shared__ float4 lmf[768];
   __shared__ unsigned long long hs[HPB];
   __shared__ int32_t hn[HPB];
   __shared__ uint32_t uqe[kApiQueue];
   __shared__ int32_t uqn;
   __shared__ PoseF pf[HPB];
-  for (int i = tid; i < nl; i += blockDim.x) lmf[i] = lmk.xyzf[i];
+  for (int i = tid; i < nl; i += blockDim.x) lmf[i] = lmk.dxyzf[i];
   for (int i = tid; i < HPB; i += blockDim.x) {
     hs[i] = 0;
     hn[i] = 0;
@@ -4865,25 +4877,25 @@
   if (tid == 0) uqn = 0;
   __syncthreads();
   const UQueue q{uqe, &uqn, kApiQueue};
-  WaveLms<kScrUnroll> wl;
-  wl.load(lmf, nl * (wave & 1) / 2, nl * ((wave & 1) + 1) / 2);
+  WaveLms<U> wl;
+  wl.load(lmf, lmk.dw, nl * (wave & 1) / 2, nl * ((wave & 1) + 1) / 2);
   for (int t = __builtin_amdgcn_readfirstlane(wave); t < 2 * nh; t += NW) {
     const int j = t >> 1;
     const Xf* T = (const Xf*)(c2w + 12 * (size_t)(h0 + j));
     long long s;
     int c;
-    wl.sums(pf[j], fd.scam, fd.w, fd.h, fd.bgr, mask, q, j, T, lmk.xyz, cmp, s, c);
+    wl.sums(pf[j], fd.scam, fd.w, fd.h, fd.bgr, mask, q, j, T, lmk.dxyz, cmp, s, c);
     if (lane == 0) {
       atomicAdd(&hs[j], (unsigned long long)s);
       atomicAdd(&hn[j], c);
     }
   }
   __syncthreads();
-  block_drain(q, lmk.xyz, cmp, fd.w, fd.h, fd.bgr, mask,
+  block_drain(q, lmk.dxyz, lmk.dw, cmp, fd.w, fd.h, fd.bgr, mask,
               [&](int t) -> const Xf& { return *(const Xf*)(c2w + 12 * (size_t)(h0 + t)); },
-              [&](int t, int e) {
+              [&](int t, int e, int w) {
                 atomicAdd(&hs[t], (unsigned long long)e);
-                atomicAdd(&hn[t], 1);
+                atomicAdd(&hn[t], w);
               });
   __syncthreads();
   for (int i = tid; i < nh; i += blockDim.x) {
@@ -4892,14 +4904,15 @@
     nproj[h0 + i] = c;
   }
 }
+template <int U>
 __global__ __launch_bounds__(64 * kApiHyps) void k_score_api(const FrameDesc* __restrict__ frames, const uint8_t* mask,
                                                              Landmarks lmk, const double* __restrict__ c2w, int n,
                                                              int fast, double* __restrict__ err,
                                                              int32_t* __restrict__ nproj) {
   const FrameDesc fd = frames[0];
   if (fast) {
-    if (mask) score_api_fast<kApiHyps>(fd, &frames[0].cam, MaskBytes{mask}, lmk, c2w, n, err, nproj);
-    else score_api_fast<kApiHyps>(fd, &frames[0].cam, MaskNone{}, lmk, c2w, n, err, nproj);
+    if (mask) score_api_fast<kApiHyps, U>(fd, &frames[0].cam, MaskBytes{mask}, lmk, c2w, n, err, nproj);
+    else score_api_fast<kApiHyps, U>(fd, &frames[0].cam, MaskNone{}, lmk, c2w, n, err, nproj);
     return;
   }
   const int wave = threadIdx.x >> 6, lane = threadIdx.x & 63;
diff --git a/mantis_amd/csrc/mk_lmdedupe.h b/mantis_amd/csrc/mk_lmdedupe.h
--- /dev/null
+++ b/mantis_amd/csrc/mk_lmdedupe.h
@@ -0,0 +1,30 @@
+#pragma once
+#include <cstdint>
+#include <cstring>
+
+namespace mk {
+
+inline int lm_dedupe(const double* xyz, int n, bool merge, double* out_xyz, int32_t* out_w, int32_t* out_first) {
+  int nd = 0;
+  for (int i = 0; i < n; i++) {
+    int at = -1;
+    if (merge)
+      for (int j = 0; j < nd && at < 0; j++)
+        if (std::memcmp(out_xyz + 3 * j, xyz + 3 * i, 3 * sizeof(double)) == 0) at = j;
+    if (at >= 0) {
+      out_w[at]++;
+      continue;
+    }
+    std::memcpy(out_xyz + 3 * nd, xyz + 3 * i, 3 * sizeof(double));
+    out_w[nd] = 1;
+    if (out_first) out_first[nd] = i;
+    nd++;
+  }
+  return nd;
+}
+
+inline int lm_trip_slots(int nd, int split, int wide) {
+  return (nd + split - 1) / split <= 64 * (wide - 1) ? wide - 1 : wide;
+}
+
+}
diff --git a/mantis_amd/csrc/track_impl.hip b/mantis_amd/csrc/track_impl.hip
--- a/mantis_amd/csrc/track_impl.hip
+++ b/mantis_amd/csrc/track_impl.hip
@@ -110,7 +110,7 @@
   static_assert(kW % SPLIT == 0 && kPP >= 1 && 64 * kScrUnroll * SPLIT >= 768, "one register trip per slice");
   const FrameDesc fd = frames[f];
   const int W = fd.w, H = fd.h;
-  const int nl = lmk.nw + lmk.nr + lmk.ng;
+  const int nl = lmk.nd;
   __shared__ float4 lmf[768];
   __shared__ Xf Pc[kPP];
   __shared__ PoseF Pf[kPP];
@@ -119,7 +119,7 @@
   __shared__ uint32_t uqe[kPfQueue];
   __shared__ int32_t uqn;
   const int j0 = chunk * kPP, nj = max(0, min(kPP, np - j0));
-  for (int i = tid; i < nl; i += NT) lmf[i] = lmk.xyzf[i];
+  for (int i = tid; i < nl; i += NT) lmf[i] = lmk.dxyzf[i];
   if (tid < nj) {
     const size_t t = t0 + (size_t)(j0 + tid) * C + cam;
     Pc[tid] = c2w[t];
@@ -134,23 +134,23 @@
   WaveLms<kScrUnroll> wl;
   {
     const int h = wave % SPLIT;
-    wl.load(lmf, nl * h / SPLIT, nl * (h + 1) / SPLIT);
+    wl.load(lmf, lmk.dw, nl * h / SPLIT, nl * (h + 1) / SPLIT);
   }
   for (int task = __builtin_amdgcn_readfirstlane(wave); task < nj * SPLIT; task += kW) {
     const int j = task / SPLIT;
     long long sum;
     int cnt;
-    wl.sums(Pf[j], fd.scam, W, H, fd.bgr, mask, q, j, &Pc[j], lmk.xyz, &frames[f].cam, sum, cnt);
+    wl.sums(Pf[j], fd.scam, W, H, fd.bgr, mask, q, j, &Pc[j], lmk.dxyz, &frames[f].cam, sum, cnt);
     if (lane == 0) {
       atomicAdd(&Ps[j], (unsigned long long)sum);
       atomicAdd(&Pn[j], cnt);
     }
   }
   __syncthreads();
-  block_drain(q, lmk.xyz, &frames[f].cam, W, H, fd.bgr, mask, [&](int t) -> const Xf& { return Pc[t]; },
-              [&](int t, int e) {
+  block_drain(q, lmk.dxyz, lmk.dw, &frames[f].cam, W, H, fd.bgr, mask, [&](int t) -> const Xf& { return Pc[t]; },
+              [&](int t, int e, int w) {
                 atomicAdd(&Ps[t], (unsigned long long)e);
-                atomicAdd(&Pn[t], 1);
+                atomicAdd(&Pn[t], w);
               });
   __syncthreads();
   if (tid < nj) {
```

Result: faster. 31170 rig poses/s (median of 3 runs) (+2.2%).
